# lRomul/sensorium

Hardware: AMD Instinct MI355X
Metric: training clips/sec/GPU (DwiseNeuro fwd+bwd, B=32 T=32 36x64) at 1/2/4/8 GPUs (higher is better)
Workload: dtype bf16

## Files before the change

### include/dwn.h

```cpp
#ifndef DWN_H_
#define DWN_H_
#include <stddef.h>
#include <stdint.h>

#ifdef __cplusplus
extern "C" {
#endif

#define DWN_ABI_VERSION 7
#define DWN_F32 0
#define DWN_BF16 1
#define DWN_F32_AUTO 0
#define DWN_F32_NATIVE 1
#define DWN_F32_SPLIT3 2
#define DWN_BN_EVAL 0
#define DWN_BN_TRAIN 1
#define DWN_BN_FROZEN 2
#define DWN_NREP 32

#define DWN_LD_PLAIN 0
#define DWN_LD_PE 1
#define DWN_LD_BNACT 2
#define DWN_LD_AFFINE2 3
#define DWN_LD_DY3 4
// ... 81 lines not shown
typedef struct dwn_dw_spatial_bwd_args {
    dwn_load_desc dy;
    dwn_load_desc y1;
    const float* w;
    void* dh1;
    float* dw;
    int planes, Hin, Win, Hout, Wout, C, stride, ks;
    double* stats;
    int rows_band;
    int impl;
    const void* a0; long long a0_ld; const void* w1; int Cin;
} dwn_dw_spatial_bwd_args;

typedef struct dwn_dw_temporal_fwd_args {
    dwn_load_desc in;
    const float* w;
    void* out;
    int B, T, HW, C, kt;
    double* stats;
    const float* z_scale; const float* z_shift; long long* pooled;
} dwn_dw_temporal_fwd_args;

typedef struct dwn_dw_temporal_bwd_args {
    dwn_load_desc dy; int dy_kind;
    dwn_load_desc y2;
    const float* w;
    void* dh2;
    float* dw;
    int B, T, HW, C, kt;
    double* stats;
} dwn_dw_temporal_bwd_args;

typedef struct dwn_bn {
    const float* gamma; const float* beta;
    float* running_mean; float* running_var; long long* num_batches_tracked;
    float* coef;
    float* dgamma; float* dbeta;
} dwn_bn;

typedef struct dwn_stem_args {
    int dtype, training, B, Cin, C0; long long S;
    float eps, momentum;
    const float* x;
    const float* w;
    dwn_bn bn;
    const float *pe_t, *pe_h, *pe_w;
    int T, H, W;
    void* y0;
    void* out;
    const void* dout;
    float* dw;
    void* ws; size_t ws_bytes;
    double* xmom;
} dwn_stem_args;

typedef struct dwn_stem_input_grad_args {
    int dtype, training, B, Cin, C0; long long S;
    const float* w;
    const float* coef;
    const void* dout;
    float* dx;
} dwn_stem_input_grad_args;

typedef struct dwn_block_args {
    int dtype, training;
    int B, T, Hin, Win, Hout, Wout, Cin, Cmid, Cout, stride, ks, kt, se_r;
    float eps, momentum;
    const void* x; void* out;
    void *y1, *y2, *y3, *y4;
    void* z3;
    int x_has_pe;
    void* a0;
    const float *pe_t, *pe_h, *pe_w;
    const float *out_pe_t, *out_pe_h, *out_pe_w;
    const float *w_pw, *w_dws, *w_dwt, *w_pwl, *se_wr, *se_br, *se_we, *se_be;
    dwn_bn bn1, bn2, bn3, bn4, bnsc;
    const float* drop_scale;
    const int *hsrc, *wsrc, *hinv, *winv;
    float *se_pmean, *se_hidpre, *se_gate;
    const void* dout; void* dx;
    void *buf_a, *buf_b;
    void *dy4, *da0;
    float *dw_pw, *dw_dws, *dw_dwt, *dw_pwl, *dse_wr, *dse_br, *dse_we, *dse_be;
    void* ws; size_t ws_bytes;
    int pwl_bwd;
    int f32_products;
    int y1_mode;
} dwn_block_args;

typedef struct dwn_pool_args {
    int dtype; long long BT; int HW, C;
    const void* x; void* out; const void* dout; void* dx;
} dwn_pool_args;

typedef struct dwn_cortex_args {
    int dtype, training, B, T, Cin, C, groups;
    float eps, momentum;
    const void* x; void* out; void* y;
    const float* w;
    dwn_bn bn, bnsc;
    const float* drop_scale;
    const void* dout; void* dx; float* dw;
    const float* dout_mask; int dout_mask_ld;
    void* ws; size_t ws_bytes;
    int f32_products;
} dwn_cortex_args;

typedef struct dwn_readout_args {
    int dtype, B, T, Cin, groups, n_out;
    float softplus_beta;
    const void* x;
    const float* w; const float* bias;
    const float* drop_mask;
    float* out;
    const float* dout; void* dx; float* dw; float* dbias;
    void* ws; size_t ws_bytes;
    void* wt;
    int f32_products;
    const float* beta_dev; float* dbeta;
} dwn_readout_args;

typedef struct dwn_tensor_entry {
    float* param; const float* grad; float* exp_avg; float* exp_avg_sq; float* ema;
    long long numel; int is_int64; int pad_;
} dwn_tensor_entry;

typedef struct dwn_guarded_entry {
    float* param; const float* grad; float* exp_avg; float* exp_avg_sq; float* ema;
    long long numel; int is_int64; int pad_;
    long long* step;
} dwn_guarded_entry;
typedef struct dwn_step_guard {
    double norm;
    float coef;
    int skip;
    long long nonfinite;
    long long good_steps, skipped_steps;
} dwn_step_guard;
#define DWN_GS_SEG 1024

// ... 11 lines not shown
typedef struct dwn_clip_desc {
    dwn_clip_src src, mix;
    int bbx1, bby1, bbx2, bby2;
    float one_minus_lam, lam;
    int mouse;
    int mix_mode;
} dwn_clip_desc;

enum {
    DWN_FAM_PW_FWD = 0, DWN_FAM_DWS_FWD, DWN_FAM_DWT_FWD, DWN_FAM_SE_POOL, DWN_FAM_PWL_FWD, DWN_FAM_RESID_FWD,
    DWN_FAM_RESID_BWD, DWN_FAM_PWL_DGRAD, DWN_FAM_PWL_WGRAD, DWN_FAM_BN3_REDUCE, DWN_FAM_DWT_BWD, DWN_FAM_DWS_BWD,
    DWN_FAM_PW_DGRAD, DWN_FAM_PW_WGRAD, DWN_FAM_CORTEX_FWD, DWN_FAM_CORTEX_BWD, DWN_FAM_READOUT_FWD, DWN_FAM_READOUT_BWD,
    DWN_FAM_COUNT
};
#define DWN_PROF_ROCTX (1ull << 63)
int dwn_profile_enable(unsigned long long family_mask, int device);
int dwn_profile_collect(int family, double* total_ms, long long* launches);

int dwn_abi_version(void);
const char* dwn_source_hash(void);
int dwn_sizeof(const char* struct_name);
const char* dwn_last_error(void);

int dwn_gemm_nn(const dwn_gemm_nn_args* a, int dtype, int device, void* stream);
int dwn_gemm_tn(const dwn_gemm_tn_args* a, int dtype, int device, void* stream);
int dwn_dw_spatial_fwd(const dwn_dw_spatial_fwd_args* a, int dtype, int device, void* stream);
int dwn_dw_spatial_bwd(const dwn_dw_spatial_bwd_args* a, int dtype, int device, void* stream);
int dwn_dw_spatial_fwd_rc_supported(const dwn_dw_spatial_fwd_args* a, int dtype);
int dwn_dw_spatial_bwd_rc_supported(const dwn_dw_spatial_bwd_args* a, int dtype);
int dwn_dw_temporal_fwd(const dwn_dw_temporal_fwd_args* a, int dtype, int device, void* stream);
int dwn_dw_temporal_bwd(const dwn_dw_temporal_bwd_args* a, int dtype, int device, void* stream);
int dwn_dw_temporal_wide_fwd(const dwn_dw_temporal_fwd_args* a, int dtype, int device, void* stream);
int dwn_dw_temporal_wide_bwd(const dwn_dw_temporal_bwd_args* a, int dtype, int device, void* stream);
int dwn_bn_finalize(const double* stats, int stat_c, double count, const dwn_bn* bn, int C, int training,
                    float momentum, float eps, int device, void* stream);
int dwn_bn_bwd_finalize(const double* stats, double count, const dwn_bn* bn, float* abc, int C, int device,
                        void* stream);
int dwn_pack_weight(const float* src, void* dst, int groups, int R, int C, int transpose, int Rd, int Cd,
                    int dtype, int device, void* stream);
size_t dwn_conv_pw_bn_stats_workspace_bytes(int Cin);
int dwn_conv_pw_bn_stats(const void* a0, long long a0_ld, long long M, const float* w_pw, int E, int Cin, const dwn_bn* bn,
                         float momentum, float eps, double* sc_stats, void* ws, size_t ws_bytes, int dtype, int device,
                         void* stream);

size_t dwn_stem_workspace_bytes(const dwn_stem_args* a);
int dwn_stem_forward(const dwn_stem_args* a, int device, void* stream);
int dwn_stem_backward(const dwn_stem_args* a, int device, void* stream);
int dwn_stem_input_grad(const dwn_stem_input_grad_args* a, int device, void* stream);
int dwn_stem_backward_input(const dwn_stem_args* a, float* dx, int device, void* stream);
size_t dwn_block_workspace_bytes(const dwn_block_args* a, int backward);
int dwn_block_forward(const dwn_block_args* a, int device, void* stream);
int dwn_block_backward(const dwn_block_args* a, int device, void* stream);
int dwn_block_forward_writes(const dwn_block_args* a);
int dwn_pool_forward(const dwn_pool_args* a, int device, void* stream);
int dwn_pool_backward(const dwn_pool_args* a, int device, void* stream);
size_t dwn_cortex_workspace_bytes(const dwn_cortex_args* a, int backward);
int dwn_cortex_forward(const dwn_cortex_args* a, int device, void* stream);
int dwn_cortex_backward(const dwn_cortex_args* a, int device, void* stream);
size_t dwn_readout_workspace_bytes(const dwn_readout_args* a, int backward);
size_t dwn_readout_wt_bytes(const dwn_readout_args* a);
int dwn_readout_forward(const dwn_readout_args* a, int device, void* stream);
int dwn_readout_backward(const dwn_readout_args* a, int device, void* stream);

int dwn_poisson_loss_forward(const float* pred, const float* target, const float* w, long long per_sample,
                             long long total, float eps, double* loss_acc, int device, void* stream);
int dwn_poisson_loss_backward(const float* pred, const float* target, const float* w, const float* gscale,
                              long long per_sample, long long total, float eps, float* dpred, int device,
                              void* stream);
int dwn_f64_to_f32(const double* src, float* dst, int n, int device, void* stream);

int dwn_adamw_ema_multi(const dwn_tensor_entry* list, int ntensors, int max_blocks, double lr, double beta1,
                        double beta2, double eps, double weight_decay, long long step, double ema_decay,
                        double grad_scale, int device, void* stream);
int dwn_ema_lerp_multi(const dwn_tensor_entry* list, int ntensors, int max_blocks, double decay, int device,
                       void* stream);

size_t dwn_grad_guard_workspace_bytes(int ntensors, int max_blocks);
int dwn_grad_sumsq_multi(const dwn_guarded_entry* list, int ntensors, int max_blocks, double grad_scale, void* ws,
                         size_t ws_bytes, double* pair, int device, void* stream);
int dwn_step_guard_finalize(const double* pair_a, const double* pair_b, double max_norm, int skip_nonfinite,
                            const dwn_guarded_entry* list, int ntensors, dwn_step_guard* guard, int device, void* stream);
int dwn_adamw_ema_multi_guarded(const dwn_guarded_entry* list, int ntensors, int max_blocks, double lr, double beta1,
                                double beta2, double eps, double weight_decay, double ema_decay, double grad_scale,
                                const dwn_step_guard* guard, int device, void* stream);


typedef struct dwn_pw_bwd_args {
    const void* dh1; const void* a0; const float* w_pw; const float* abc;
    void* da0; float* dw;
    long long M; int E; int Cin;
    void* ws; size_t ws_bytes;
    const void* res; const float* res_abc; int res_C;
    const int* res_hinv; const int* res_winv; int res_Hin, res_Win, res_Hout, res_Wout;
} dwn_pw_bwd_args;
int dwn_pw_bwd_fused_supported(int dtype, long long M, int E, int Cin);
size_t dwn_pw_backward_workspace_bytes(int E, int Cin, int dtype);
int dwn_pw_backward(const dwn_pw_bwd_args* a, int dtype, int device, void* stream);

typedef struct dwn_dw_spatial_rc_fwd_args {
    const void* a0; long long a0_ld;
    const void* blob;
    void* out;
    int planes, Hin, Win, Hout, Wout, Cin, E, stride;
    double* stats;
    int rows_band;
    int round_y1;
// ... 238 lines not shown
```

### sensorium_amd/_lib.py

```python
from __future__ import annotations

import ctypes as C
import os
from pathlib import Path

import torch

_HERE = Path(__file__).resolve().parent
DETERMINISTIC = os.environ.get("DWN_DETERMINISTIC", "0") == "1"
_LIB_NAME = "libdwiseneuro_hip_det.so" if DETERMINISTIC else "libdwiseneuro_hip.so"
LIB_PATH = Path(os.environ["DWN_LIB_PATH"]) if os.environ.get("DWN_LIB_PATH") else _HERE / "csrc" / _LIB_NAME

c_p = C.c_void_p
c_i = C.c_int
c_ll = C.c_longlong
c_f = C.c_float
c_d = C.c_double
c_sz = C.c_size_t

DWN_F32, DWN_BF16 = 0, 1
DWN_NREP = 32
LD_PLAIN, LD_PE, LD_BNACT, LD_AFFINE2, LD_DY3, LD_GATE, LD_CAT1 = 0, 1, 2, 3, 4, 5, 6
EPI_STORE, EPI_READOUT, EPI_DG, EPI_STORE_CAT, EPI_DH3 = 0, 1, 2, 3, 4
NN_AUTO, NN_XL128, NN_XL256, NN_TILE128, NN_KD = 0, 1, 2, 3, 4
# ... 12 lines not shown


class GemmNNArgs(C.Structure):
    _fields_ = [("a", LoadDesc), ("a_kind", c_i), ("b", c_p), ("ldb", c_ll), ("c", c_p), ("ldc", c_ll),
                ("M", c_i), ("N", c_i), ("K", c_i), ("groups", c_i), ("stats", c_p),
                ("f32_split", c_i), ("stat_nchan", c_i), ("epi", c_i), ("bias", c_p),
                ("sp_beta", c_f), ("out_nct", c_p), ("Tn", c_i), ("n_valid", c_i), ("y3", c_p), ("ldy3", c_ll),
                ("s3", c_p), ("t3", c_p), ("dg", c_p), ("dg_ld", c_i), ("rows_per_sample", c_i),
                ("a2", c_p), ("a2_ld", c_ll), ("K1", c_i), ("b_sample_stride", c_ll), ("b_rows_per_sample", c_i),
                ("gate3", c_p), ("dps3", c_p), ("coef3", c_p), ("coef3_ld", c_i), ("variant", c_i), ("sp_beta_dev", c_p)]


class GemmTNArgs(C.Structure):
    _fields_ = [("p", LoadDesc), ("p_kind", c_i), ("q", LoadDesc), ("q_kind", c_i), ("M", c_i), ("R", c_i),
                ("Cc", c_i), ("dw", c_p), ("lddw", c_ll), ("groups", c_i), ("rows_per_split", c_i),
                ("nsplit", c_i), ("R_load", c_i), ("rows_per_sample", c_i), ("splits_per_sample", c_i),
                ("dw_sample_stride", c_ll), ("overwrite", c_i), ("dw_f64", c_i)]


class DwSpatialFwdArgs(C.Structure):
    _fields_ = [("inp", LoadDesc), ("w", c_p), ("out", c_p), ("planes", c_i), ("Hin", c_i), ("Win", c_i),
                ("Hout", c_i), ("Wout", c_i), ("C", c_i), ("stride", c_i), ("ks", c_i), ("stats", c_p),
                ("rows_band", c_i), ("impl", c_i),
                ("a0", c_p), ("a0_ld", c_ll), ("w1", c_p), ("Cin", c_i)]


class DwSpatialBwdArgs(C.Structure):
    _fields_ = [("dy", LoadDesc), ("y1", LoadDesc), ("w", c_p), ("dh1", c_p), ("dw", c_p), ("planes", c_i),
                ("Hin", c_i), ("Win", c_i), ("Hout", c_i), ("Wout", c_i), ("C", c_i), ("stride", c_i),
                ("ks", c_i), ("stats", c_p), ("rows_band", c_i), ("impl", c_i),
                ("a0", c_p), ("a0_ld", c_ll), ("w1", c_p), ("Cin", c_i)]


class DwTemporalFwdArgs(C.Structure):
    _fields_ = [("inp", LoadDesc), ("w", c_p), ("out", c_p), ("B", c_i), ("T", c_i), ("HW", c_i), ("C", c_i),
                ("kt", c_i), ("stats", c_p), ("z_scale", c_p), ("z_shift", c_p), ("pooled", c_p)]


class DwTemporalBwdArgs(C.Structure):
    _fields_ = [("dy", LoadDesc), ("dy_kind", c_i), ("y2", LoadDesc), ("w", c_p), ("dh2", c_p), ("dw", c_p),
                ("B", c_i), ("T", c_i), ("HW", c_i), ("C", c_i), ("kt", c_i), ("stats", c_p)]


class BN(C.Structure):
    _fields_ = [("gamma", c_p), ("beta", c_p), ("running_mean", c_p), ("running_var", c_p),
                ("num_batches_tracked", c_p), ("coef", c_p), ("dgamma", c_p), ("dbeta", c_p)]


class StemArgs(C.Structure):
    _fields_ = [("dtype", c_i), ("training", c_i), ("B", c_i), ("Cin", c_i), ("C0", c_i), ("S", c_ll),
                ("eps", c_f), ("momentum", c_f), ("x", c_p), ("w", c_p), ("bn", BN),
                ("pe_t", c_p), ("pe_h", c_p), ("pe_w", c_p), ("T", c_i), ("H", c_i), ("W", c_i),
                ("y0", c_p), ("out", c_p),
                ("dout", c_p), ("dw", c_p), ("ws", c_p), ("ws_bytes", c_sz), ("xmom", c_p)]


class StemInputGradArgs(C.Structure):
    _fields_ = [("dtype", c_i), ("training", c_i), ("B", c_i), ("Cin", c_i), ("C0", c_i), ("S", c_ll),
                ("w", c_p), ("coef", c_p), ("dout", c_p), ("dx", c_p)]


class BlockArgs(C.Structure):
    _fields_ = [("dtype", c_i), ("training", c_i),
                ("B", c_i), ("T", c_i), ("Hin", c_i), ("Win", c_i), ("Hout", c_i), ("Wout", c_i), ("Cin", c_i),
                ("Cmid", c_i), ("Cout", c_i), ("stride", c_i), ("ks", c_i), ("kt", c_i), ("se_r", c_i),
                ("eps", c_f), ("momentum", c_f),
                ("x", c_p), ("out", c_p), ("y1", c_p), ("y2", c_p), ("y3", c_p), ("y4", c_p),
                ("z3", c_p), ("x_has_pe", c_i), ("a0", c_p),
                ("pe_t", c_p), ("pe_h", c_p), ("pe_w", c_p),
                ("out_pe_t", c_p), ("out_pe_h", c_p), ("out_pe_w", c_p),
                ("w_pw", c_p), ("w_dws", c_p), ("w_dwt", c_p), ("w_pwl", c_p), ("se_wr", c_p), ("se_br", c_p),
                ("se_we", c_p), ("se_be", c_p),
                ("bn1", BN), ("bn2", BN), ("bn3", BN), ("bn4", BN), ("bnsc", BN),
                ("drop_scale", c_p), ("hsrc", c_p), ("wsrc", c_p), ("hinv", c_p), ("winv", c_p),
                ("se_pmean", c_p), ("se_hidpre", c_p), ("se_gate", c_p),
                ("dout", c_p), ("dx", c_p), ("buf_a", c_p), ("buf_b", c_p), ("dy4", c_p), ("da0", c_p),
                ("dw_pw", c_p), ("dw_dws", c_p), ("dw_dwt", c_p), ("dw_pwl", c_p), ("dse_wr", c_p),
                ("dse_br", c_p), ("dse_we", c_p), ("dse_be", c_p),
                ("ws", c_p), ("ws_bytes", c_sz), ("pwl_bwd", c_i), ("f32_products", c_i), ("y1_mode", c_i)]


class PoolArgs(C.Structure):
    _fields_ = [("dtype", c_i), ("BT", c_ll), ("HW", c_i), ("C", c_i), ("x", c_p), ("out", c_p), ("dout", c_p),
                ("dx", c_p)]


class CortexArgs(C.Structure):
    _fields_ = [("dtype", c_i), ("training", c_i), ("B", c_i), ("T", c_i), ("Cin", c_i), ("C", c_i),
                ("groups", c_i), ("eps", c_f), ("momentum", c_f), ("x", c_p), ("out", c_p), ("y", c_p),
                ("w", c_p), ("bn", BN), ("bnsc", BN), ("drop_scale", c_p), ("dout", c_p), ("dx", c_p),
                ("dw", c_p), ("dout_mask", c_p), ("dout_mask_ld", c_i), ("ws", c_p), ("ws_bytes", c_sz), ("f32_products", c_i)]


class ReadoutArgs(C.Structure):
    _fields_ = [("dtype", c_i), ("B", c_i), ("T", c_i), ("Cin", c_i), ("groups", c_i), ("n_out", c_i),
                ("softplus_beta", c_f), ("x", c_p), ("w", c_p), ("bias", c_p), ("drop_mask", c_p), ("out", c_p),
                ("dout", c_p), ("dx", c_p), ("dw", c_p), ("dbias", c_p), ("ws", c_p), ("ws_bytes", c_sz), ("wt", c_p),
                ("f32_products", c_i), ("beta_dev", c_p), ("dbeta", c_p)]


class TensorEntry(C.Structure):
    _fields_ = [("param", c_p), ("grad", c_p), ("exp_avg", c_p), ("exp_avg_sq", c_p), ("ema", c_p),
                ("numel", c_ll), ("is_int64", c_i), ("pad_", c_i)]


class GuardedEntry(C.Structure):
    _fields_ = [("param", c_p), ("grad", c_p), ("exp_avg", c_p), ("exp_avg_sq", c_p), ("ema", c_p),
                ("numel", c_ll), ("is_int64", c_i), ("pad_", c_i), ("step", c_p)]


class StepGuard(C.Structure):
    _fields_ = [("norm", c_d), ("coef", c_f), ("skip", c_i), ("nonfinite", c_ll), ("good_steps", c_ll),
                ("skipped_steps", c_ll)]


class ClipSrc(C.Structure):
    _fields_ = [("video", c_p), ("behavior", c_p), ("pupil_center", c_p), ("responses", c_p), ("length", c_ll),
                ("video_dtype", c_i), ("frame_start", c_i), ("frame_step", c_i), ("valid", c_i)]


class ClipDesc(C.Structure):
    _fields_ = [("src", ClipSrc), ("mix", ClipSrc), ("bbx1", c_i), ("bby1", c_i), ("bbx2", c_i), ("bby2", c_i),
                ("one_minus_lam", c_f), ("lam", c_f), ("mouse", c_i), ("mix_mode", c_i)]


class PwBwdArgs(C.Structure):
    _fields_ = [("dh1", c_p), ("a0", c_p), ("w_pw", c_p), ("abc", c_p), ("da0", c_p), ("dw", c_p),
                ("M", c_ll), ("E", c_i), ("Cin", c_i), ("ws", c_p), ("ws_bytes", c_sz), ("res", c_p), ("res_abc", c_p),
                ("res_C", c_i), ("res_hinv", c_p), ("res_winv", c_p), ("res_Hin", c_i), ("res_Win", c_i), ("res_Hout", c_i),
                ("res_Wout", c_i)]


# ... 99 lines not shown
TRIAL_STATE_ROWS, TRIAL_SCORE_ROWS, TRIAL_SUMMARY, TRIAL_TILE = 17, 5, 8, 4
NOISE_BINARY, NOISE_SPARSE = 0, 1
STA_SUMMARY = 8
GAUSS_PARAMS, GAUSS_TABLE = 7, 16
MIX_BOX, MIX_BLEND = 0, 1
VID_U8, VID_F32 = 0, 1

_STRUCTS = {
    "dwn_load_desc": LoadDesc, "dwn_gemm_nn_args": GemmNNArgs, "dwn_gemm_tn_args": GemmTNArgs,
    "dwn_dw_spatial_fwd_args": DwSpatialFwdArgs, "dwn_dw_spatial_bwd_args": DwSpatialBwdArgs,
    "dwn_dw_temporal_fwd_args": DwTemporalFwdArgs, "dwn_dw_temporal_bwd_args": DwTemporalBwdArgs,
    "dwn_bn": BN, "dwn_stem_args": StemArgs, "dwn_block_args": BlockArgs, "dwn_pool_args": PoolArgs,
    "dwn_cortex_args": CortexArgs, "dwn_readout_args": ReadoutArgs, "dwn_tensor_entry": TensorEntry,
    "dwn_clip_src": ClipSrc, "dwn_clip_desc": ClipDesc, "dwn_pw_bwd_args": PwBwdArgs,
    "dwn_dw_spatial_rc_fwd_args": DwSpatialRcFwdArgs, "dwn_stem_input_grad_args": StemInputGradArgs,
    "dwn_guarded_entry": GuardedEntry, "dwn_step_guard": StepGuard, "dwn_gaze_args": GazeArgs,
    "dwn_corr_args": CorrArgs, "dwn_gabor_args": GaborArgs, "dwn_modulator_args": ModulatorArgs,
    "dwn_blur3d_args": Blur3dArgs, "dwn_clip_moments_args": ClipMomentsArgs, "dwn_mei_update_args": MeiUpdateArgs,
    "dwn_trial_desc": TrialDesc, "dwn_trial_group": TrialGroup, "dwn_trial_score_args": TrialScoreArgs,
    "dwn_spatial_gain_args": SpatialGainArgs, "dwn_noise_args": NoiseArgs, "dwn_sta_args": StaArgs,
    "dwn_gauss2d_args": Gauss2dArgs, "dwn_gauss2d_profile_args": Gauss2dProfileArgs,
}

_P = C.POINTER
SYMBOLS = {
    "dwn_abi_version": (c_i, []),
    "dwn_source_hash": (C.c_char_p, []),
    "dwn_sizeof": (c_i, [C.c_char_p]),
    "dwn_last_error": (C.c_char_p, []),
    "dwn_profile_enable": (c_i, [C.c_ulonglong, c_i]),
    "dwn_profile_collect": (c_i, [c_i, _P(c_d), _P(c_ll)]),
    "dwn_gemm_nn": (c_i, [_P(GemmNNArgs), c_i, c_i, c_p]),
    "dwn_gemm_tn": (c_i, [_P(GemmTNArgs), c_i, c_i, c_p]),
    "dwn_dw_spatial_fwd": (c_i, [_P(DwSpatialFwdArgs), c_i, c_i, c_p]),
    "dwn_dw_spatial_bwd": (c_i, [_P(DwSpatialBwdArgs), c_i, c_i, c_p]),
    "dwn_dw_spatial_bwd_rc_supported": (c_i, [_P(DwSpatialBwdArgs), c_i]),
    "dwn_dw_spatial_fwd_rc_supported": (c_i, [_P(DwSpatialFwdArgs), c_i]),
    "dwn_dw_temporal_fwd": (c_i, [_P(DwTemporalFwdArgs), c_i, c_i, c_p]),
    "dwn_dw_temporal_bwd": (c_i, [_P(DwTemporalBwdArgs), c_i, c_i, c_p]),
    "dwn_dw_temporal_wide_fwd": (c_i, [_P(DwTemporalFwdArgs), c_i, c_i, c_p]),
    "dwn_dw_temporal_wide_bwd": (c_i, [_P(DwTemporalBwdArgs), c_i, c_i, c_p]),
    "dwn_bn_finalize": (c_i, [c_p, c_i, c_d, _P(BN), c_i, c_i, c_f, c_f, c_i, c_p]),
    "dwn_bn_bwd_finalize": (c_i, [c_p, c_d, _P(BN), c_p, c_i, c_i, c_p]),
    "dwn_pack_weight": (c_i, [c_p, c_p, c_i, c_i, c_i, c_i, c_i, c_i, c_i, c_i, c_p]),
    "dwn_stem_workspace_bytes": (c_sz, [_P(StemArgs)]),
    "dwn_stem_forward": (c_i, [_P(StemArgs), c_i, c_p]),
    "dwn_stem_backward": (c_i, [_P(StemArgs), c_i, c_p]),
    "dwn_stem_input_grad": (c_i, [_P(StemInputGradArgs), c_i, c_p]),
    "dwn_stem_backward_input": (c_i, [_P(StemArgs), c_p, c_i, c_p]),
    "dwn_block_workspace_bytes": (c_sz, [_P(BlockArgs), c_i]),
    "dwn_block_forward": (c_i, [_P(BlockArgs), c_i, c_p]),
    "dwn_block_backward": (c_i, [_P(BlockArgs), c_i, c_p]),
    "dwn_block_forward_writes": (c_i, [_P(BlockArgs)]),
    "dwn_pool_forward": (c_i, [_P(PoolArgs), c_i, c_p]),
    "dwn_pool_backward": (c_i, [_P(PoolArgs), c_i, c_p]),
    "dwn_cortex_workspace_bytes": (c_sz, [_P(CortexArgs), c_i]),
    "dwn_cortex_forward": (c_i, [_P(CortexArgs), c_i, c_p]),
    "dwn_cortex_backward": (c_i, [_P(CortexArgs), c_i, c_p]),
    "dwn_readout_workspace_bytes": (c_sz, [_P(ReadoutArgs), c_i]),
    "dwn_readout_wt_bytes": (c_sz, [_P(ReadoutArgs)]),
    "dwn_readout_forward": (c_i, [_P(ReadoutArgs), c_i, c_p]),
    "dwn_readout_backward": (c_i, [_P(ReadoutArgs), c_i, c_p]),
    "dwn_poisson_loss_forward": (c_i, [c_p, c_p, c_p, c_ll, c_ll, c_f, c_p, c_i, c_p]),
    "dwn_poisson_loss_backward": (c_i, [c_p, c_p, c_p, c_p, c_ll, c_ll, c_f, c_p, c_i, c_p]),
    "dwn_f64_to_f32": (c_i, [c_p, c_p, c_i, c_i, c_p]),
    "dwn_adamw_ema_multi": (c_i, [c_p, c_i, c_i, c_d, c_d, c_d, c_d, c_d, c_ll, c_d, c_d, c_i, c_p]),
    "dwn_ema_lerp_multi": (c_i, [c_p, c_i, c_i, c_d, c_i, c_p]),
    "dwn_grad_guard_workspace_bytes": (c_sz, [c_i, c_i]),
    "dwn_grad_sumsq_multi": (c_i, [c_p, c_i, c_i, c_d, c_p, c_sz, c_p, c_i, c_p]),
    "dwn_step_guard_finalize": (c_i, [c_p, c_p, c_d, c_i, c_p, c_i, c_p, c_i, c_p]),
    "dwn_adamw_ema_multi_guarded": (c_i, [c_p, c_i, c_i, c_d, c_d, c_d, c_d, c_d, c_d, c_d, c_p, c_i, c_p]),
    "dwn_conv_pw_bn_stats_workspace_bytes": (c_sz, [c_i]),
    "dwn_conv_pw_bn_stats": (c_i, [c_p, c_ll, c_ll, c_p, c_i, c_i, _P(BN), c_f, c_f, c_p, c_p, c_sz, c_i, c_i, c_p]),
    "dwn_pw_bwd_fused_supported": (c_i, [c_i, c_ll, c_i, c_i]),
    "dwn_pw_backward_workspace_bytes": (c_sz, [c_i, c_i, c_i]),
    "dwn_pw_backward": (c_i, [_P(PwBwdArgs), c_i, c_i, c_p]),
    "dwn_dw_spatial_rc_blob_bytes": (c_sz, [c_i, c_i]),
    "dwn_dw_spatial_rc_prep": (c_i, [c_p, c_p, c_p, c_i, c_i, c_p, c_i, c_p]),
    "dwn_dw_spatial_rc_supported": (c_i, [c_i, c_i, c_i, c_i, c_i, c_i, c_i]),
    "dwn_dw_spatial_fwd_rc": (c_i, [_P(DwSpatialRcFwdArgs), c_i, c_p]),
    "dwn_assemble_inputs": (c_i, [c_p, c_i, c_i, c_i, c_i, c_i, c_i, c_f, c_p, c_i, c_p]),
    "dwn_assemble_targets": (c_i, [c_p, c_i, c_i, c_p, c_p, c_i, c_i, c_p, c_i, c_p]),
    "dwn_gaze_shift_forward": (c_i, [_P(GazeArgs), c_i, c_p]),
    "dwn_gaze_shift_backward": (c_i, [_P(GazeArgs), c_i, c_p]),
    "dwn_plane_mean": (c_i, [c_p, c_i, c_i, c_i, c_i, c_i, c_i, c_i, c_p, c_i, c_p]),
    "dwn_corr_ws_bytes": (c_sz, [_P(CorrArgs)]),
    "dwn_corr_moments": (c_i, [_P(CorrArgs), c_i, c_p]),
    "dwn_corr_loss_finalize": (c_i, [_P(CorrArgs), c_i, c_p]),
    "dwn_corr_loss_backward": (c_i, [_P(CorrArgs), c_i, c_p]),
    "dwn_gabor_workspace_bytes": (c_sz, [_P(GaborArgs)]),
    "dwn_gabor_forward": (c_i, [_P(GaborArgs), c_i, c_p]),
    "dwn_gabor_backward": (c_i, [_P(GaborArgs), c_i, c_p]),
    "dwn_modulator_ws_bytes": (c_sz, [_P(ModulatorArgs)]),
    "dwn_modulator_forward": (c_i, [_P(ModulatorArgs), c_i, c_p]),
    "dwn_modulator_backward": (c_i, [_P(ModulatorArgs), c_i, c_p]),
    "dwn_blur3d_ws_bytes": (c_sz, [_P(Blur3dArgs)]),
    "dwn_clip_moments_ws_bytes": (c_sz, [_P(ClipMomentsArgs)]),
    "dwn_blur3d": (c_i, [_P(Blur3dArgs), c_i, c_p]),
    "dwn_clip_moments": (c_i, [_P(ClipMomentsArgs), c_i, c_p]),
    "dwn_mei_update": (c_i, [_P(MeiUpdateArgs), c_i, c_p]),
    "dwn_trial_score_ws_bytes": (c_sz, [_P(TrialScoreArgs)]),
    "dwn_trial_moments": (c_i, [_P(TrialScoreArgs), c_i, c_p]),
    "dwn_trial_score_finalize": (c_i, [_P(TrialScoreArgs), c_i, c_p]),
    "dwn_spatial_gain_ws_bytes": (c_sz, [_P(SpatialGainArgs)]),
    "dwn_spatial_gain_forward": (c_i, [_P(SpatialGainArgs), c_i, c_p]),
    "dwn_spatial_gain_backward": (c_i, [_P(SpatialGainArgs), c_i, c_p]),
    "dwn_gauss2d_ws_bytes": (c_sz, [_P(Gauss2dArgs)]),
    "dwn_gauss2d_fit": (c_i, [_P(Gauss2dArgs), c_i, c_p]),
    "dwn_gauss2d_profile": (c_i, [_P(Gauss2dProfileArgs), c_i, c_p]),
    "dwn_noise_forward": (c_i, [_P(NoiseArgs), c_i, c_p]),
    "dwn_sta_state_bytes": (c_sz, [_P(StaArgs)]),
    "dwn_sta_ws_bytes": (c_sz, [_P(StaArgs)]),
    "dwn_sta_accumulate": (c_i, [_P(StaArgs), c_i, c_p]),
    "dwn_sta_finalize": (c_i, [_P(StaArgs), c_i, c_p]),
}


class DwnError(RuntimeError):
    pass


HASH_SRCS = ("dwn_api.hip", "dwn_gemm.hip", "dwn_gemm_nn_1.hip", "dwn_gemm_nn_2.hip", "dwn_gemm_nn_3.hip", "dwn_gemm_nn_4.hip", "dwn_gemm_nn_5.hip",
             "dwn_gemm_nn_6.hip", "dwn_gemm_tn.hip", "dwn_pw_bwd.hip", "dwn_gemm_xl.hip", "dwn_gemm_kd.hip", "dwn_dwconv.hip", "dwn_dwrc.hip",
             "dwn_dwbwd.hip", "dwn_dwfwd.hip", "dwn_elementwise.hip", "dwn_data.hip", "dwn_gaze.hip", "dwn_modulator.hip", "dwn_spatial.hip", "dwn_mei.hip", "dwn_rf_fit.hip", "dwn_trial_score.hip", "dwn_rf.hip", "dwn_corr.hip", "dwn_stim.hip", "dwn_common.h", "dwn_internal.h",
             "dwn_kernels.h", "dwn_launch.h", "dwn_gemm_nn.h", "dwn_gain.h",
             "../../include/dwn.h")


def source_hash() -> str:
    import hashlib
    h = hashlib.sha256()
    for name in HASH_SRCS:
        h.update((_HERE / "csrc" / name).read_bytes())
    return h.hexdigest()[:16]


def _load():
    if not LIB_PATH.exists():
        raise ImportError(
            f"{LIB_PATH} is missing: build it with `python -c 'import __graft_entry__ as g; g.build()'` "
            f"(or `make -C {LIB_PATH.parent}`).  sensorium_amd has no fallback path.")
    lib = C.CDLL(str(LIB_PATH), mode=getattr(os, "RTLD_NOW", 2))
    ab = bool(os.environ.get("DWN_LIB_PATH"))
    for name, (restype, argtypes) in SYMBOLS.items():
        if ab and name in ("dwn_stem_input_grad", "dwn_stem_backward_input", "dwn_grad_guard_workspace_bytes", "dwn_grad_sumsq_multi",
                           "dwn_step_guard_finalize", "dwn_adamw_ema_multi_guarded", "dwn_dw_temporal_wide_fwd",
                           "dwn_dw_temporal_wide_bwd", "dwn_gaze_shift_forward", "dwn_gaze_shift_backward",
                           "dwn_plane_mean", "dwn_corr_ws_bytes", "dwn_corr_moments", "dwn_corr_loss_finalize",
                           "dwn_corr_loss_backward", "dwn_gabor_workspace_bytes", "dwn_gabor_forward",
                           "dwn_gabor_backward", "dwn_modulator_ws_bytes", "dwn_modulator_forward",
                           "dwn_modulator_backward", "dwn_blur3d_ws_bytes", "dwn_clip_moments_ws_bytes", "dwn_blur3d",
                           "dwn_clip_moments", "dwn_mei_update", "dwn_trial_score_ws_bytes", "dwn_trial_moments",
                           "dwn_trial_score_finalize", "dwn_spatial_gain_ws_bytes", "dwn_spatial_gain_forward",
                           "dwn_spatial_gain_backward", "dwn_noise_forward", "dwn_sta_state_bytes", "dwn_sta_ws_bytes",
                           "dwn_sta_accumulate", "dwn_sta_finalize", "dwn_gauss2d_ws_bytes", "dwn_gauss2d_fit",
                           "dwn_gauss2d_profile") and not hasattr(lib, name):
            continue
        fn = getattr(lib, name)
        fn.restype = restype
        fn.argtypes = argtypes
    if lib.dwn_abi_version() != 7 and not (ab and lib.dwn_abi_version() == 6):
        raise ImportError("libdwiseneuro_hip.so ABI version mismatch")
    built, have = lib.dwn_source_hash().decode(), source_hash()
    if built != have and not os.environ.get("DWN_LIB_PATH"):
        raise ImportError(f"{LIB_PATH.name} was built from other sources (binary {built}, tree {have}): rebuild it with "
                          f"`make -C {LIB_PATH.parent}` — binaries are not in git, so what runs must be what is committed")
    for cname, struct in _STRUCTS.items():
        n = lib.dwn_sizeof(cname.encode())
        if n != C.sizeof(struct) and not (ab and (0 < n < C.sizeof(struct) or cname in ("dwn_stem_input_grad_args", "dwn_guarded_entry", "dwn_step_guard", "dwn_gaze_args", "dwn_corr_args", "dwn_gabor_args", "dwn_modulator_args", "dwn_blur3d_args", "dwn_clip_moments_args", "dwn_mei_update_args", "dwn_trial_desc", "dwn_trial_group", "dwn_trial_score_args", "dwn_spatial_gain_args", "dwn_noise_args", "dwn_sta_args", "dwn_gauss2d_args", "dwn_gauss2d_profile_args"))):
            raise ImportError(f"struct layout mismatch for {cname}: C {n} bytes vs ctypes {C.sizeof(struct)}")
    return lib


lib = _load()


def check(rc: int, what: str = ""):
    if rc != 0:
        msg = lib.dwn_last_error()
        raise DwnError(f"{what} failed (rc={rc}): {msg.decode() if msg else ''}")
```

### sensorium_amd/csrc/dwn_api.hip

```cpp
#include "dwn_internal.h"
#include "dwn_kernels.h"
#include <string.h>
#include <math.h>

static thread_local char g_err[512] = "";
#ifndef DWN_EVAL_CHAIN
#define DWN_EVAL_CHAIN 1
#endif

extern "C" size_t dwn_dw_spatial_rc_blob_bytes(int E, int Cin);
extern "C" int dwn_dw_spatial_rc_supported(int dtype, int Cin, int E, int ks, int stride, int Hin, int Win);
extern "C" int dwn_dw_spatial_rc_prep(const float* w_pw, const float* w_dws, const float* bn1_coef, int E, int Cin, void* blob,
                                      int device, void* stream);
extern "C" int dwn_dw_spatial_fwd_rc(const dwn_dw_spatial_rc_fwd_args* a, int device, void* stream);
bool dw_spatial_bwd_rc_supported(const DwSpatialBwd& a, int dtype);
bool dw_spatial_fwd_rc_walk_supported(const DwSpatialFwd& a, int dtype);

int dwn_set_error(int code, const char* msg) {
    snprintf(g_err, sizeof(g_err), "dwn error %d: %s", code, msg ? msg : "");
    return code;
}

#define TRY(x) do { int rc__ = (x); if (rc__ != 0) return rc__; } while (0)

// ... 325 lines not shown
int dwn_dw_temporal_wide_bwd(const dwn_dw_temporal_bwd_args* a, int dtype, int device, void* stream) {
    g_err[0] = 0;
    if (int rc = dw_temporal_wide_check(a->kt, a->C, a->dy_kind)) return rc;
    ENTER(device);
    return launch_dw_temporal_wide_bwd(*a, dtype, (hipStream_t)stream);
}
int dwn_bn_finalize(const double* stats, int stat_c, double count, const dwn_bn* bn, int C, int training,
                    float momentum, float eps, int device, void* stream) {
    ENTER(device);
    return bn_finalize(stats, stat_c, count, *bn, C, training, momentum, eps, (hipStream_t)stream);
}
int dwn_bn_bwd_finalize(const double* stats, double count, const dwn_bn* bn, float* abc, int C, int device,
                        void* stream) {
    ENTER(device);
    return k_bn_bwd_finalize(bwd_job(stats, count, *bn, abc, C, false), BnBwdJob{}, (hipStream_t)stream);
}
size_t dwn_conv_pw_bn_stats_workspace_bytes(int Cin) { return (size_t)(Cin + 8) * Cin * sizeof(double) + 256; }
int dwn_conv_pw_bn_stats(const void* a0, long long a0_ld, long long M, const float* w_pw, int E, int Cin, const dwn_bn* bn,
                         float momentum, float eps, double* sc_stats, void* ws, size_t ws_bytes, int dtype, int device, void* stream) {
    ENTER(device);
    hipStream_t s = (hipStream_t)stream;
    if (!a0 || !w_pw || !bn || !bn->coef || !ws) return dwn_set_error(-1, "conv_pw_bn_stats: null pointer");
    if (Cin % 8 || E <= 0 || M <= 0 || M >= (1ll << 31)) return dwn_set_error(-2, "conv_pw_bn_stats: Cin % 8 == 0, 0 < M < 2^31");
    if (ws_bytes < dwn_conv_pw_bn_stats_workspace_bytes(Cin)) return dwn_set_error(-6, "conv_pw_bn_stats: workspace too small");
    double* gram = reinterpret_cast<double*>(((size_t)ws + 255) & ~(size_t)255);
    TRY(k_zero(gram, (size_t)(Cin + 8) * Cin * sizeof(double), s));
    LoadDesc cat = ld_plain(a0, a0_ld);
    cat.cat_c1 = Cin; cat.cat_c2 = 0;
    GemmTN g = tn_base(cat, LD_CAT1, ld_plain(a0, a0_ld), LD_PLAIN, (int)M, Cin + 8, Cin, reinterpret_cast<float*>(gram), Cin, 1);
    g.dw_f64 = 1;
    TRY(launch_gemm_tn(g, dtype, s));
    return k_bn1_gram_finalize(gram, w_pw, E, Cin, (double)M, bn->gamma, bn->beta, bn->running_mean, bn->running_var,
                               bn->num_batches_tracked, momentum, eps, bn->coef, sc_stats, dtype, s);
}
int dwn_pack_weight(const float* src, void* dst, int groups, int R, int C, int transpose, int Rd, int Cd, int dtype,
                    int device, void* stream) {
    ENTER(device);
    return k_pack_weight(src, dst, groups, R, C, transpose, Rd, Cd, dtype, (hipStream_t)stream);
}

size_t dwn_stem_workspace_bytes(const dwn_stem_args* a) {
    return ((size_t)DWN_NREP * stem_moment_count() * sizeof(double) + 256 +
            (size_t)DWN_NREP * a->C0 * stem_acc_stride() * sizeof(double) + 1024);
}
int dwn_stem_forward(const dwn_stem_args* a, int device, void* stream) {
    ENTER(device);
    hipStream_t s = (hipStream_t)stream;
    if (a->C0 % 8) return dwn_set_error(-2, "stem: C0 must be a multiple of 8");
    if (a->pe_t && (i64)a->T * a->H * a->W != a->S) return dwn_set_error(-2, "stem: T*H*W != S");
    Carver c(a->ws, a->ws_bytes);
    double* mom = c.take<double>((size_t)DWN_NREP * stem_moment_count());
    if (!c.ok()) return dwn_set_error(-6, "stem: workspace too small");
    const i64 M = (i64)a->B * a->S;
    if (a->training == DWN_BN_TRAIN) {
        if (!a->xmom) return dwn_set_error(-1, "stem_forward: xmom buffer required in training mode");
        TRY(k_zero(mom, (size_t)DWN_NREP * stem_moment_count() * sizeof(double), s));
        TRY(k_stem_xmom(a->x, a->B, a->Cin, a->S, mom, s));
        TRY(k_stem_bn_finalize(mom, (double)M, a->w, a->bn.gamma, a->bn.beta, a->bn.running_mean, a->bn.running_var,
                               a->bn.num_batches_tracked, a->momentum, a->eps, a->bn.coef, a->xmom, a->C0, a->Cin, s));
    } else {
        TRY(bn_finalize(nullptr, a->C0, (double)M, a->bn, a->C0, 0, a->momentum, a->eps, s));
    }
    return k_stem_out(a->x, a->w, a->bn.coef, a->pe_t, a->pe_h, a->pe_w, a->T, a->H, a->W, a->B, a->Cin, a->S, a->C0, a->out,
                      a->dtype, s);
}
int dwn_stem_backward(const dwn_stem_args* a, int device, void* stream) {
    ENTER(device);
    hipStream_t s = (hipStream_t)stream;
    const bool frozen = a->training == DWN_BN_FROZEN;
    if (!frozen && !a->xmom) return dwn_set_error(-1, "stem_backward: xmom (saved by the forward) required");
    Carver c(a->ws, a->ws_bytes);
    double* mom = c.take<double>((size_t)DWN_NREP * stem_moment_count());
    double* acc = c.take<double>((size_t)DWN_NREP * a->C0 * stem_acc_stride());
    if (!c.ok()) return dwn_set_error(-6, "stem: workspace too small");
    const i64 M = (i64)a->B * a->S;
    if (frozen) {
        TRY(k_zero(mom, (size_t)((char*)(acc + (size_t)DWN_NREP * a->C0 * stem_acc_stride()) - (char*)mom), s));
        TRY(k_stem_bwd_acc(a->dout, a->x, mom, (double)M, a->B, a->Cin, a->S, a->C0, acc, a->dtype, s));
        return k_stem_bwd_finalize_frozen(acc, a->w, a->bn.coef, a->bn.dgamma, a->bn.dbeta, a->dw, a->C0, a->Cin, s);
    }
    TRY(k_zero(acc, (size_t)DWN_NREP * a->C0 * stem_acc_stride() * sizeof(double), s));
    TRY(k_stem_bwd_acc(a->dout, a->x, a->xmom, (double)M, a->B, a->Cin, a->S, a->C0, acc, a->dtype, s));
    return k_stem_bwd_finalize(acc, a->xmom, a->w, a->bn.coef, (double)M, a->bn.dgamma, a->bn.dbeta, a->dw, a->C0, a->Cin, s);
}

int dwn_stem_backward_input(const dwn_stem_args* a, float* dx, int device, void* stream) {
    g_err[0] = 0;
    if (!a || !dx) return dwn_set_error(-1, "stem_backward_input: null pointer (args, dx)");
    if (a->training != DWN_BN_TRAIN)
        return dwn_set_error(-7, "stem_backward_input: built for batch statistics (DWN_BN_TRAIN) only; the frozen-statistics input "
                                 "gradient is dwn_stem_backward + dwn_stem_input_grad");
    if (!a->x || !a->w || !a->bn.coef || !a->dout || !a->dw || !a->xmom || !a->ws)
        return dwn_set_error(-1, "stem_backward_input: null pointer (x, w, bn.coef, dout, dw, xmom, ws)");
    if (a->C0 <= 0 || a->C0 % 8 || a->Cin <= 0 || a->B <= 0 || a->S <= 0)
        return dwn_set_error(-2, "stem_backward_input: C0 must be a positive multiple of 8; B, Cin, S positive");
    if (a->dtype != DWN_F32 && a->dtype != DWN_BF16) return dwn_set_error(-2, "stem_backward_input: dtype");
    if (a->C0 > (a->dtype == DWN_BF16 ? 128 : 64) || a->Cin > 8)
        return dwn_set_error(-4, "stem_backward_input: more than 128 (bf16) / 64 (fp32) stem channels or 8 input channels not built");
    ENTER(device);
    hipStream_t s = (hipStream_t)stream;
    Carver c(a->ws, a->ws_bytes);
    double* mom = c.take<double>((size_t)DWN_NREP * stem_moment_count());
    double* acc = c.take<double>((size_t)DWN_NREP * a->C0 * stem_acc_stride());
    if (!c.ok()) return dwn_set_error(-6, "stem: workspace too small");
    float* qx = reinterpret_cast<float*>(mom);
    const i64 M = (i64)a->B * a->S;
    TRY(k_zero(acc, (size_t)DWN_NREP * a->C0 * stem_acc_stride() * sizeof(double), s));
    TRY(k_stem_bwd_acc(a->dout, a->x, a->xmom, (double)M, a->B, a->Cin, a->S, a->C0, acc, a->dtype, s));
    TRY(k_stem_bwd_finalize(acc, a->xmom, a->w, a->bn.coef, (double)M, a->bn.dgamma, a->bn.dbeta, a->dw, a->C0, a->Cin, s));
    TRY(k_stem_bwd_finalize_dx(acc, a->xmom, a->w, a->bn.coef, (double)M, qx, a->C0, a->Cin, s));
    return k_stem_input_grad_train(a->dout, a->w, a->bn.coef, a->x, qx, a->B, a->Cin, a->S, a->C0, dx, a->dtype, s);
}

int dwn_stem_input_grad(const dwn_stem_input_grad_args* a, int device, void* stream) {
    g_err[0] = 0;
    if (!a || !a->w || !a->coef || !a->dout || !a->dx) return dwn_set_error(-1, "stem_input_grad: null pointer");
    if (a->C0 <= 0 || a->C0 % 8 || a->Cin <= 0 || a->B <= 0 || a->S <= 0)
        return dwn_set_error(-2, "stem_input_grad: C0 must be a positive multiple of 8; B, Cin, S positive");
    if (a->dtype != DWN_F32 && a->dtype != DWN_BF16) return dwn_set_error(-2, "stem_input_grad: dtype");
    if (a->training != DWN_BN_FROZEN)
        return dwn_set_error(-7, "stem_input_grad: this entry is the frozen-statistics (DWN_BN_FROZEN) input gradient; through batch "
                                 "statistics (DWN_BN_TRAIN) it is dwn_stem_backward_input");
    ENTER(device);
    return k_stem_input_grad(a->dout, a->w, a->coef, a->B, a->Cin, a->S, a->C0, a->dx, a->dtype, (hipStream_t)stream);
}

size_t dwn_block_workspace_bytes(const dwn_block_args* a, int backward) {
    return carve_block(*a, backward, nullptr, 0).bytes;
}

int dwn_block_forward(const dwn_block_args* ap, int device, void* stream) {
    ENTER(device);
    const dwn_block_args& a = *ap;
    hipStream_t s = (hipStream_t)stream;
    TRY(check_block(a));
    BlockWs w = carve_block(a, 0, a.ws, a.ws_bytes);
    if (w.bytes > a.ws_bytes) return dwn_set_error(-6, "block_forward: workspace too small");
    const int dt = a.dtype, tr = a.training != DWN_BN_EVAL;
    const bool bs = a.training == DWN_BN_TRAIN;
    const i64 Min = (i64)a.B * a.T * a.Hin * a.Win, Mout = (i64)a.B * a.T * a.Hout * a.Wout;
    const int S_out = a.T * a.Hout * a.Wout;
    {
        PrepArgs pa;
        bool ok = pa.zero(w.zero_beg, ((size_t)(w.zero_end - w.zero_beg) + 15) & ~(size_t)15);
        ok = ok && pa.packw(a.w_pw, w.wpw, 1, a.Cmid, a.Cin, 0, a.Cmid, a.Cin);
        ok = ok && pa.packw(a.w_pwl, w.wpwl, 1, a.Cout, a.Cmid, 0, a.Cout, a.Cmid);
        ok = ok && pa.packdw(a.w_dws, w.wdws, a.Cmid, a.ks * a.ks);
        ok = ok && pa.packdw(a.w_dwt, w.wdwt, a.Cmid, a.kt);
        if (!bs) {
            ok = ok && pa.bneval(a.bn1, a.Cmid, a.eps) && pa.bneval(a.bn2, a.Cmid, a.eps) && pa.bneval(a.bn3, a.Cmid, a.eps);
            ok = ok && pa.bneval(a.bn4, a.Cout, a.eps) && pa.bneval(a.bnsc, a.Cout, a.eps);
        }
        if (!ok) return dwn_set_error(-2, "block_forward: workspace arena must be 16-byte aligned");
        TRY(k_prep(pa, dt, s));
    }

    const void* a0 = a.x;
    if (!a.x_has_pe) {
        if (!a.a0) return dwn_set_error(-2, "block_forward: a0 buffer required when x_has_pe == 0");
        TRY(k_ew_apply(ld_pe(a.x, a.Cin, a.pe_t, a.pe_h, a.pe_w, a.T, a.Hin, a.Win), LD_PE, a.a0, a.Cin, Min, a.Cin, dt, s));
        a0 = a.a0;
    }
    LoadDesc xin = ld_plain(a0, a.Cin);
    const bool identity_sc = a.stride == 1 && a.Hin == a.Hout && a.Win == a.Wout;
    const bool y1_free = tr && block_y1_free(a);
    bool eval_chain = false;
    if (DWN_EVAL_CHAIN && !tr && dt == DWN_BF16) {
        DwSpatialFwd f; memset(&f, 0, sizeof(f));
        f.planes = a.B * a.T; f.Hin = a.Hin; f.Win = a.Win; f.Hout = a.Hout; f.Wout = a.Wout; f.C = a.Cmid; f.stride = a.stride; f.ks = a.ks;
        f.in.ld = a.Cmid; f.a0_ld = a.Cin; f.Cin = a.Cin;
        eval_chain = dw_spatial_fwd_rc_walk_supported(f, dt);
    }
    if (eval_chain) {
        DwSpatialFwd d; memset(&d, 0, sizeof(d));
        d.in = ld_bnact(nullptr, a.Cmid, a.bn1.coef, a.Cmid, 1, nullptr, 0, 1);
        d.a0 = a0; d.a0_ld = a.Cin; d.w1 = w.wpw; d.Cin = a.Cin;
        d.w = w.wdws; d.out = a.y2; d.planes = a.B * a.T; d.Hin = a.Hin; d.Win = a.Win; d.Hout = a.Hout;
        d.Wout = a.Wout; d.C = a.Cmid; d.stride = a.stride; d.ks = a.ks; d.stats = nullptr;
        PROF(DWN_FAM_DWS_FWD, launch_dw_spatial_fwd(d, dt, s));
    } else if (y1_free) {
        LoadDesc cat = ld_plain(a0, a.Cin);
        cat.cat_c1 = a.Cin; cat.cat_c2 = 0;
        if (bs) {
        GemmTN g = tn_base(cat, LD_CAT1, ld_plain(a0, a.Cin), LD_PLAIN, (int)Min, a.Cin + 8, a.Cin, reinterpret_cast<float*>(w.gram), a.Cin, 1);
        g.dw_f64 = 1;
        PROF(DWN_FAM_PW_FWD, launch_gemm_tn(g, dt, s));
        PROF(DWN_FAM_PW_FWD, k_bn1_gram_finalize(w.gram, a.w_pw, a.Cmid, a.Cin, (double)Min, a.bn1.gamma, a.bn1.beta, a.bn1.running_mean,
                                                 a.bn1.running_var, a.bn1.num_batches_tracked, a.momentum, a.eps, a.bn1.coef,
                                                 identity_sc ? w.stsc : nullptr, dt, s));
        }
        DwSpatialFwd d; memset(&d, 0, sizeof(d));
        d.in = ld_bnact(nullptr, a.Cmid, a.bn1.coef, a.Cmid, 1, nullptr, 0, 1);
        d.a0 = a0; d.a0_ld = a.Cin; d.w1 = w.wpw; d.Cin = a.Cin;
        d.w = w.wdws; d.out = a.y2; d.planes = a.B * a.T; d.Hin = a.Hin; d.Win = a.Win; d.Hout = a.Hout;
        d.Wout = a.Wout; d.C = a.Cmid; d.stride = a.stride; d.ks = a.ks; d.stats = w.st2;
        PROF(DWN_FAM_DWS_FWD, launch_dw_spatial_fwd(d, dt, s));
    } else if (block_fwd_rc(a)) {
        TRY(dwn_dw_spatial_rc_prep(a.w_pw, w.wdws, a.bn1.coef, a.Cmid, a.Cin, w.rcblob, device, stream));
        dwn_dw_spatial_rc_fwd_args r; memset(&r, 0, sizeof(r));
        r.a0 = a0; r.a0_ld = a.Cin; r.blob = w.rcblob; r.out = a.y2; r.planes = a.B * a.T; r.Hin = a.Hin; r.Win = a.Win;
        r.Hout = a.Hout; r.Wout = a.Wout; r.Cin = a.Cin; r.E = a.Cmid; r.stride = a.stride; r.stats = nullptr;
        r.rows_band = 0; r.round_y1 = 1;
        PROF(DWN_FAM_DWS_FWD, dwn_dw_spatial_fwd_rc(&r, device, stream));
    } else {
    {
        GemmNN g = nn_base(xin, LD_PLAIN, w.wpw, a.Cin, a.y1, a.Cmid, (int)Min, a.Cmid, a.Cin, 1);
        g.f32_split = f32_split_of(a.f32_products, !tr);
        g.stats = tr ? w.st1 : nullptr; g.stat_nchan = a.Cmid;
        PROF(DWN_FAM_PW_FWD, launch_gemm_nn(g, dt, s));
    }
    if (bs) TRY(bn_finalize(w.st1, a.Cmid, (double)Min, a.bn1, a.Cmid, 1, a.momentum, a.eps, s));
    {
        DwSpatialFwd d; memset(&d, 0, sizeof(d));
        d.in = ld_bnact(a.y1, a.Cmid, a.bn1.coef, a.Cmid, 1, nullptr, 0, 1);
        d.w = w.wdws; d.out = a.y2; d.planes = a.B * a.T; d.Hin = a.Hin; d.Win = a.Win; d.Hout = a.Hout;
        d.Wout = a.Wout; d.C = a.Cmid; d.stride = a.stride; d.ks = a.ks; d.stats = tr ? w.st2 : nullptr;
        PROF(DWN_FAM_DWS_FWD, launch_dw_spatial_fwd(d, dt, s));
    }
    }
    if (bs) TRY(bn_finalize(w.st2, a.Cmid, (double)Mout, a.bn2, a.Cmid, 1, a.momentum, a.eps, s));
    const bool eval_z3 = !tr;
    {
        DwTemporalFwd d; memset(&d, 0, sizeof(d));
        d.in = ld_bnact(a.y2, a.Cmid, a.bn2.coef, a.Cmid, 1, nullptr, 0, 1);
        d.w = w.wdwt; d.out = a.y3; d.B = a.B; d.T = a.T; d.HW = a.Hout * a.Wout; d.C = a.Cmid; d.kt = a.kt;
        d.stats = tr ? w.st3 : nullptr;
        if (eval_z3) {
            d.out = a.z3; d.z_scale = a.bn3.coef; d.z_shift = a.bn3.coef + a.Cmid; d.pooled = w.pooled;
        }
        PROF(DWN_FAM_DWT_FWD, launch_dw_temporal_fwd(d, dt, s));
    }
    if (bs) TRY(bn_finalize(w.st3, a.Cmid, (double)Mout, a.bn3, a.Cmid, 1, a.momentum, a.eps, s));
    if (!eval_z3) {
        LoadDesc z3 = ld_bnact(a.y3, a.Cmid, a.bn3.coef, a.Cmid, 1, nullptr, 0, S_out);
        PROF(DWN_FAM_SE_POOL, k_se_pool(z3, a.B, a.Cmid, S_out, w.pooled, a.z3, dt, s));
    }
    int gate_folded = 0;
    TRY(k_se_mlp_fwd(w.pooled, 1.0f / (float)S_out, a.se_wr, a.se_br, a.se_we, a.se_be, a.B, a.Cmid, a.se_r,
                     a.se_pmean, a.se_hidpre, a.se_gate, pwl_gated_weights(a) ? a.w_pwl : nullptr, w.wgated, a.Cout, dt, &gate_folded, s));
    if (pwl_gated_weights(a)) {
        if (!gate_folded) TRY(k_gate_weights(a.w_pwl, a.se_gate, w.wgated, a.B, a.Cout, a.Cmid, dt, s));
        GemmNN g = nn_base(ld_plain(a.z3, a.Cmid), LD_PLAIN, w.wgated, a.Cmid, a.y4, a.Cout, (int)Mout, a.Cout, a.Cmid, 1);
        g.b_sample_stride = (i64)a.Cout * a.Cmid; g.b_rows_per_sample = S_out;
        g.stats = tr ? w.st4 : nullptr; g.stat_nchan = a.Cout; g.f32_split = f32_split_of(a.f32_products, !tr);
        PROF(DWN_FAM_PWL_FWD, launch_gemm_nn(g, dt, s));
    } else {
        LoadDesc u = ld_plain(a.z3, a.Cmid);
        u.gate = a.se_gate; u.gate_ld = a.Cmid; u.rows_per_sample = S_out;
        GemmNN g = nn_base(u, LD_GATE, w.wpwl, a.Cmid, a.y4, a.Cout, (int)Mout, a.Cout, a.Cmid, 1);
        g.stats = tr ? w.st4 : nullptr; g.stat_nchan = a.Cout; g.f32_split = f32_split_of(a.f32_products, !tr);
        PROF(DWN_FAM_PWL_FWD, launch_gemm_nn(g, dt, s));
    }
    ResGeom gm = geom_of(a);
    if (bs) {
        if (!(y1_free && identity_sc)) PROF(DWN_FAM_RESID_FWD, k_shortcut_stats(xin, gm, w.stsc, dt, s));
        TRY(k_bn_finalize_train(fin_job(w.st4, a.Cout, (double)Mout, a.bn4, a.Cout),
                                 fin_job(w.stsc, a.Cin, (double)Mout, a.bnsc, a.Cout), a.momentum, a.eps, s));
    }
    PROF(DWN_FAM_RESID_FWD, k_residual_fwd(xin, a.y4, a.bn4.coef, a.bnsc.coef, a.drop_scale, gm, a.out_pe_t, a.out_pe_h,
                                           a.out_pe_w, a.out, dt, s));
    return 0;
}

static int pw_backward(int dt, const void* dh1, const void* a0, const float* w_pw, const float* abc, int E, int Cin, i64 M,
                       void* bp, float* gacc, float* r3, float* tacc, void* da0, float* dw, const void* res,
                       const float* res_abc, int res_C, const ResGeom* rg, hipStream_t s) {
    const int res_n = res ? res_C / Cin : 0;
    const bool gathered = res && rg && rg->hinv;
    if (res && (!res_abc || res_C % Cin || res_n < 1 || res_n > 2))
        return dwn_set_error(-2, "pw_backward: the shortcut term needs res_abc and res_C in {Cin, 2 Cin}");
    if (res && !pw_bwd_fused_supported(dt, M, E, Cin))
        return dwn_set_error(-3, "pw_backward: the shortcut term is built into the one-pass kernel only (dwn_pw_bwd_fused_supported)");
    TRY(k_pw_bwd_prep(w_pw, abc, E, Cin, bp, gacc, r3, dt, (res && !gathered) ? res_abc : nullptr, res_C, s));
    if (pw_bwd_fused_supported(dt, M, E, Cin)) {
        PROF(DWN_FAM_PW_DGRAD, launch_pw_bwd_fused(dh1, a0, bp, r3, da0, tacc, M, E, Cin, dt, res, res_abc, res_n,
                                                   gathered ? rg->hinv : nullptr, gathered ? rg->winv : nullptr, gathered ? rg->Hin : 0,
                                                   gathered ? rg->Win : 0, gathered ? rg->Hout : 0, gathered ? rg->Wout : 0, s));
    } else {
        {
            GemmNN g = nn_base(ld_plain(dh1, E), LD_PLAIN, bp, (i64)E + Cin, da0, Cin, (int)M, Cin, E + Cin, 1);
            g.epi = EPI_STORE_CAT; g.a2 = a0; g.a2_ld = Cin; g.K1 = E; g.bias = r3;
            PROF(DWN_FAM_PW_DGRAD, launch_gemm_nn(g, dt, s));
        }
        {
            LoadDesc cat = ld_plain(dh1, E);
            cat.q = a0; cat.ld2 = Cin; cat.cat_c1 = E; cat.cat_c2 = Cin;
            GemmTN g = tn_base(cat, LD_CAT1, ld_plain(a0, Cin), LD_PLAIN, (int)M, E + Cin + 8, Cin, tacc, Cin, 1);
            PROF(DWN_FAM_PW_WGRAD, launch_gemm_tn(g, dt, s));
        }
    }
    return k_pw_wgrad_fold(tacc, abc, w_pw, E, Cin, dw, dt, s);
}

int dwn_block_backward(const dwn_block_args* ap, int device, void* stream) {
    const dwn_block_args& a = *ap;
    hipStream_t s = (hipStream_t)stream;
    g_err[0] = 0;
    TRY(check_block(a));
    if (a.training == DWN_BN_EVAL)
        return dwn_set_error(-7, "block_backward: only training-mode (batch-statistics) and frozen-statistics backward are built");
    ENTER(device);
    const bool frozen = a.training == DWN_BN_FROZEN;
    BlockWs w = carve_block(a, 1, a.ws, a.ws_bytes);
    if (w.bytes > a.ws_bytes) return dwn_set_error(-6, "block_backward: workspace too small");
    const int dt = a.dtype;
    const i64 Min = (i64)a.B * a.T * a.Hin * a.Win, Mout = (i64)a.B * a.T * a.Hout * a.Wout;
    const int S_out = a.T * a.Hout * a.Wout;
    float* dg = reinterpret_cast<float*>(w.pooled);
    const bool y1_free = block_y1_free(a);
    {
        PrepArgs pa;
        bool ok = pa.zero(w.zero_beg, ((size_t)(w.zero_end - w.zero_beg) + 15) & ~(size_t)15);
        ok = ok && pa.packw(a.w_pwl, w.wpwl, 1, a.Cout, a.Cmid, 1, a.Cmid, a.Cout);
// ... 49 lines not shown
    }
    TRY(k_se_mlp_bwd(dg, a.se_gate, a.se_hidpre, a.se_pmean, a.se_wr, a.se_we, a.B, a.Cmid, a.se_r,
                     1.0f / (float)S_out, w.dgp, w.dhp, w.dps, a.dse_wr, a.dse_br, a.dse_we, a.dse_be, s));
    LoadDesc d3; memset(&d3, 0, sizeof(d3));
    d3.p = du; d3.q = a.y3; d3.ld = a.Cmid; d3.v1 = w.ident3; d3.v2 = w.ident3 + a.Cmid; d3.v3 = w.ident3 + 2 * a.Cmid;
    d3.v4 = a.bn3.coef; d3.v5 = a.bn3.coef + a.Cmid; d3.gate = a.se_gate; d3.gate2 = w.dps; d3.gate_ld = a.Cmid;
    d3.rows_per_sample = S_out;
    PROF(DWN_FAM_BN3_REDUCE, k_bn3_bwd_reduce(d3, a.bn3.coef, Mout, a.Cmid, w.st3, du, dt, s));
    }
    TRY(k_bn_bwd_finalize(bwd_job(w.st3, (double)Mout, a.bn3, w.abc3, a.Cmid, frozen), BnBwdJob{}, s));
    {
        DwTemporalBwd d; memset(&d, 0, sizeof(d));
        d.dy = ld_affine2(du, a.y3, a.Cmid, w.abc3, a.Cmid);
        d.dy_kind = LD_PLAIN;
        d.y2 = ld_ycoef(a.y2, a.Cmid, a.bn2.coef, a.Cmid);
        d.w = w.wdwt; d.dh2 = a.buf_b; d.dw = a.dw_dwt; d.B = a.B; d.T = a.T; d.HW = a.Hout * a.Wout; d.C = a.Cmid;
        d.kt = a.kt; d.stats = w.st2;
        PROF(DWN_FAM_DWT_BWD, launch_dw_temporal_bwd(d, dt, s));
    }
    TRY(k_bn_bwd_finalize(bwd_job(w.st2, (double)Mout, a.bn2, w.abc2, a.Cmid, frozen), BnBwdJob{}, s));
    void* dh1 = a.buf_a;
    {
        DwSpatialBwd d; memset(&d, 0, sizeof(d));
        d.dy = ld_affine2(a.buf_b, a.y2, a.Cmid, w.abc2, a.Cmid);
        d.y1 = ld_ycoef(y1_free ? nullptr : a.y1, a.Cmid, a.bn1.coef, a.Cmid);
        if (y1_free) { d.a0 = xin.p; d.a0_ld = a.Cin; d.w1 = w.wpw; d.Cin = a.Cin; }
        d.w = w.wdws; d.dh1 = dh1; d.dw = a.dw_dws; d.planes = a.B * a.T; d.Hin = a.Hin; d.Win = a.Win;
        d.Hout = a.Hout; d.Wout = a.Wout; d.C = a.Cmid; d.stride = a.stride; d.ks = a.ks; d.stats = w.st1;
        PROF(DWN_FAM_DWS_BWD, launch_dw_spatial_bwd(d, dt, s));
    }
    TRY(k_bn_bwd_finalize(bwd_job(w.st1, (double)Min, a.bn1, w.abc1, a.Cmid, frozen), BnBwdJob{}, s));
    const bool identity_sc = a.stride == 1 && a.Hin == a.Hout && a.Win == a.Wout;
    const bool dx_folded = a.Cout % a.Cin == 0 && a.Cout / a.Cin <= 2 && dwn_pw_bwd_fused_supported(dt, Min, a.Cmid, a.Cin) &&
                           (identity_sc || (gm.hinv && gm.winv && a.Hin + a.Win <= 512));
    TRY(pw_backward(dt, dh1, xin.p, a.w_pw, w.abc1, a.Cmid, a.Cin, Min, w.bp, w.gacc, w.r3, w.tacc, dx_folded ? a.dx : a.da0, a.dw_pw,
                    dx_folded ? a.dout : nullptr, w.abcsc, a.Cout, (dx_folded && !identity_sc) ? &gm : nullptr, s));
    if (dx_folded) return 0;
    PROF(DWN_FAM_RESID_BWD, k_residual_bwd_dx(xin, a.da0, a.dout, w.abcsc, gm, a.dx, dt, s));
    return 0;
}

int dwn_block_forward_writes(const dwn_block_args* ap) {
    const dwn_block_args& a = *ap;
    if (a.training) return block_y1_free(a) ? 2 : 3;
    if (block_fwd_rc(a)) return 0;
    if (DWN_EVAL_CHAIN && a.dtype == DWN_BF16) {
        DwSpatialFwd f; memset(&f, 0, sizeof(f));
        f.planes = a.B * a.T; f.Hin = a.Hin; f.Win = a.Win; f.Hout = a.Hout; f.Wout = a.Wout; f.C = a.Cmid; f.stride = a.stride; f.ks = a.ks;
        f.in.ld = a.Cmid; f.a0_ld = a.Cin; f.Cin = a.Cin;
        if (dw_spatial_fwd_rc_walk_supported(f, a.dtype)) return 0;
    }
    return 1;
}

int dwn_pool_forward(const dwn_pool_args* a, int device, void* stream) {
    ENTER(device);
    if (a->C % 8) return dwn_set_error(-2, "pool: C must be a multiple of 8");
    return k_pool_fwd(a->x, a->out, a->BT, a->HW, a->C, a->dtype, (hipStream_t)stream);
}
int dwn_pool_backward(const dwn_pool_args* a, int device, void* stream) {
    ENTER(device);
    if (a->C % 8) return dwn_set_error(-2, "pool: C must be a multiple of 8");
    return k_pool_bwd(a->dout, a->dx, a->BT, a->HW, a->C, a->dtype, (hipStream_t)stream);
}

namespace {
struct CortexWs { void* wp; double *st, *stsc; float *abc, *abcsc; void *dy, *dxmain; char *zb, *ze; size_t bytes; };
CortexWs carve_cortex(const dwn_cortex_args& a, int backward, void* base, size_t cap) {
    CortexWs w; memset(&w, 0, sizeof(w));
    Carver c(base, cap);
    const size_t ts = tsize(a.dtype);
    const i64 M = (i64)a.B * a.T;
    w.wp = c.take<char>((size_t)a.C * (a.Cin / a.groups) * ts);
    c.take<char>(0);
    size_t z0 = (c.off + 255) & ~(size_t)255;
    w.st = c.take<double>(nstat(a.C));
    w.stsc = c.take<double>(nstat(backward ? a.C : a.Cin));
    size_t z1 = c.off;
    if (backward) {
        w.abc = c.take<float>(3 * (size_t)a.C);
        w.abcsc = c.take<float>(3 * (size_t)a.C);
        w.dy = c.take<char>((size_t)M * a.C * ts);
        w.dxmain = c.take<char>((size_t)M * a.Cin * ts);
    }
    w.bytes = c.off + 256;
    if (base) { w.zb = (char*)base + z0; w.ze = (char*)base + z1; }
    return w;
}
}

size_t dwn_cortex_workspace_bytes(const dwn_cortex_args* a, int backward) {
    return carve_cortex(*a, backward, nullptr, 0).bytes;
}
int dwn_cortex_forward(const dwn_cortex_args* ap, int device, void* stream) {
    ENTER(device);
    const dwn_cortex_args& a = *ap;
    hipStream_t s = (hipStream_t)stream;
    if (a.Cin % (8 * a.groups) || a.C % (8 * a.groups)) return dwn_set_error(-2, "cortex: channels per group must be multiples of 8");
    CortexWs w = carve_cortex(a, 0, a.ws, a.ws_bytes);
    if (w.bytes > a.ws_bytes) return dwn_set_error(-6, "cortex_forward: workspace too small");
    const int M = a.B * a.T, Kg = a.Cin / a.groups, Ng = a.C / a.groups, dt = a.dtype, tr = a.training != DWN_BN_EVAL;
    const bool bs = a.training == DWN_BN_TRAIN;
    {
        PrepArgs pa;
        bool ok = pa.zero(w.zb, ((size_t)(w.ze - w.zb) + 15) & ~(size_t)15);
        ok = ok && pa.packw(a.w, w.wp, 1, a.C, Kg, 0, a.C, Kg);
// ... 661 lines not shown
```

### sensorium_amd/csrc/dwn_elementwise.hip

```cpp
#include "dwn_internal.h"
#include "dwn_kernels.h"
#include "dwn_launch.h"

#define NCV 8
#define DISPATCH_T(dtype, CALL_BF, CALL_F) do { if ((dtype) == DWN_BF16) { CALL_BF; } else { CALL_F; } } while (0)

#define SLICE_SETUP(Cval)                                   \
    constexpr int KC = TT<T>::KC;                           \
    const int tid = threadIdx.x;                            \
    const int cv = tid % NCV, pl = tid / NCV;               \
    const int c0 = blockIdx.y * NCV * KC;                   \
    const int chan = c0 + cv * KC;                          \
    const bool chan_ok = chan < (Cval);                     \
    (void)pl; (void)chan_ok;

template <int KC>
__device__ __forceinline__ void slice_stats_flush(float* lstat, const float* s0, const float* s1, int cv,
                                                 int c0, int C, double* stats, int rep) {
    static_assert(NCV == 8, "wave pre-reduction below assumes 8 channel vectors per slice");
    const int tid = threadIdx.x;
    DET_WAVES_BEGIN
#pragma unroll
    for (int i = 0; i < KC; ++i) {
        float a = s0[i], b = s1[i];
#pragma unroll
        for (int o = 8; o < 64; o <<= 1) { a += __shfl_xor(a, o); b += __shfl_xor(b, o); }
        if ((tid & 63) < NCV) {
            atomicAdd(&lstat[cv * KC + i], a);
            atomicAdd(&lstat[NCV * KC + cv * KC + i], b);
        }
    }
    DET_WAVES_END
    __syncthreads();
    DET_ENTER();
    if (tid < 2 * NCV * KC) {
        int which = tid / (NCV * KC), c = c0 + tid % (NCV * KC);
        if (c < C) stat_add(stats, rep, C, which, c, lstat[tid]);
    }
}

template <typename K>
static dim3 resident_slice_grid(K kernel, i64 rows, int C, int KC, int max_bpc = 1 << 20) {
    int slices = (C + NCV * KC - 1) / (NCV * KC);
    int bpc = resident_bpc(kernel, 256, 0, 4);
    if (bpc > max_bpc) bpc = max_bpc;
    return dim3((unsigned)resident_grid_x(bpc, slices, (rows + 31) / 32), (unsigned)slices);
}

static inline dim3 slice_grid(i64 rows, int C, int KC, int cap = 2048) {
    int slices = (C + NCV * KC - 1) / (NCV * KC);
    i64 bx = (rows + 31) / 32;
    int capx = (cap + slices - 1) / slices;
    if (bx > capx) bx = capx;
    if (bx < 1) bx = 1;
    return dim3((unsigned)bx, (unsigned)slices);
}

static inline dim3 fat_slice_grid(i64 rows, int C, int KC) {
    int slices = (C + NCV * KC - 1) / (NCV * KC);
    i64 bx = 256 / slices;
    i64 need = (rows + (1024 / NCV) - 1) / (1024 / NCV);
    if (bx > need) bx = need;
    if (bx < 1) bx = 1;
    return dim3((unsigned)bx, (unsigned)slices);
}

static_assert(DWN_NREP == 32, "replica reduce below assumes 32 replicas");
__device__ __forceinline__ void rep_reduce(const double* stats, int stat_c, int sc, int r, bool ok, double& s, double& ss) {
    s = ok ? stats[((i64)r * 2 + 0) * stat_c + sc] : 0.0;
    ss = ok ? stats[((i64)r * 2 + 1) * stat_c + sc] : 0.0;
#pragma unroll
    for (int o = 16; o > 0; o >>= 1) { s += __shfl_xor(s, o); ss += __shfl_xor(ss, o); }
}

__device__ __forceinline__ void bn_finalize_train_body(const int blk, const double* stats, int stat_c, double count,
                                                       const float* gamma, const float* beta, float* running_mean,
                                                       float* running_var, long long* nbt, float momentum, float eps,
                                                       float* coef, int C) {
    const int r = threadIdx.x & 31;
    const int c = blk * 8 + (threadIdx.x >> 5);
    if (c == 0 && r == 0 && nbt) *nbt += 1;
    const bool ok = c < C;
    const int sc = ok ? c % stat_c : 0;
    double s, ss;
    rep_reduce(stats, stat_c, sc, r, ok, s, ss);
    if (!ok || r != 0) return;
    double mean = s / count;
    double var = ss / count - mean * mean;
    if (var < 0) var = 0;
    float invstd = (float)(1.0 / sqrt(var + (double)eps));
    float scale = gamma[c] * invstd;
    coef[c] = scale;
    coef[C + c] = beta[c] - (float)mean * scale;
    coef[2 * C + c] = (float)mean;
    coef[3 * C + c] = invstd;
    if (running_mean) {
        double unbiased = count > 1 ? var * count / (count - 1) : var;
        running_mean[c] = (1.f - momentum) * running_mean[c] + momentum * (float)mean;
        running_var[c] = (1.f - momentum) * running_var[c] + momentum * (float)unbiased;
    }
}
__global__ __launch_bounds__(256) void bn_finalize_train_kernel(BnFinJob j0, BnFinJob j1, float momentum, float eps) {
    const bool first = (int)blockIdx.x < j0.nblocks;
    const BnFinJob& j = first ? j0 : j1;
    bn_finalize_train_body(first ? blockIdx.x : blockIdx.x - j0.nblocks, j.stats, j.stat_c, j.count, j.gamma, j.beta,
                           j.running_mean, j.running_var, j.nbt, momentum, eps, j.coef, j.C);
}

__global__ void bn_finalize_eval_kernel(const float* gamma, const float* beta, const float* running_mean,
                                        const float* running_var, float eps, float* coef, int C) {
    int c = blockIdx.x * blockDim.x + threadIdx.x;
    if (c >= C) return;
    float invstd = 1.0f / sqrtf(running_var[c] + eps);
    float scale = gamma[c] * invstd;
    coef[c] = scale;
    coef[C + c] = beta[c] - running_mean[c] * scale;
    coef[2 * C + c] = running_mean[c];
    coef[3 * C + c] = invstd;
// ... 184 lines not shown
    DET_WAVES_END
    __syncthreads();
    DET_ENTER();
    if (tid < STEM_NM) {
        const double v = lsum[tid];
        if (v != 0.0) atomicAdd(mom + (i64)(blockIdx.x % DWN_NREP) * STEM_NM + tid, v);
    }
    DET_EXIT();
}

__global__ __launch_bounds__(256) void stem_bn_finalize_kernel(const double* mom, double count, const float* w, const float* gamma,
                                                               const float* beta, float* running_mean, float* running_var,
                                                               long long* nbt, float momentum, float eps, float* coef,
                                                               double* xmom, int C0, int Cin) {
    __shared__ double lm[STEM_NM];
    const int tid = threadIdx.x;
    if (tid < STEM_NM) {
        double v = 0.0;
        for (int r = 0; r < DWN_NREP; ++r) v += mom[(i64)r * STEM_NM + tid];
        lm[tid] = v;
    }
    __syncthreads();
    if (tid < STEM_NM) {
        const int a_ = tid < STEM_MAXCIN ? 0 : (tid - STEM_MAXCIN) / STEM_MAXCIN, b_ = tid < STEM_MAXCIN ? 0 : (tid - STEM_MAXCIN) % STEM_MAXCIN;
        double v = lm[tid];
        if (tid >= STEM_MAXCIN && b_ < a_) v = lm[STEM_MAXCIN + b_ * STEM_MAXCIN + a_];
        xmom[tid] = v;
    }
    if (tid == 0 && nbt) *nbt += 1;
    for (int c = tid; c < C0; c += blockDim.x) {
        double mean = 0.0, var = 0.0;
        for (int a_ = 0; a_ < Cin; ++a_) mean += (double)w[c * Cin + a_] * (lm[a_] / count);
        for (int a_ = 0; a_ < Cin; ++a_)
            for (int b_ = 0; b_ < Cin; ++b_) {
                const double sxx = a_ <= b_ ? lm[STEM_MAXCIN + a_ * STEM_MAXCIN + b_] : lm[STEM_MAXCIN + b_ * STEM_MAXCIN + a_];
                const double cov = sxx / count - (lm[a_] / count) * (lm[b_] / count);
                var += (double)w[c * Cin + a_] * (double)w[c * Cin + b_] * cov;
            }
        if (var < 0) var = 0;
        const float invstd = (float)(1.0 / sqrt(var + (double)eps));
        const float scale = gamma[c] * invstd;
        coef[c] = scale;
        coef[C0 + c] = beta[c] - (float)mean * scale;
        coef[2 * C0 + c] = (float)mean;
        coef[3 * C0 + c] = invstd;
        if (running_mean) {
            const double unbiased = count > 1 ? var * count / (count - 1) : var;
            running_mean[c] = (1.f - momentum) * running_mean[c] + momentum * (float)mean;
            running_var[c] = (1.f - momentum) * running_var[c] + momentum * (float)unbiased;
        }
    }
}

template <typename T, int CINT>
__global__ __launch_bounds__(256) void stem_out_kernel(const float* x, const float* w, const float* coef, const float* pe_t,
                                                       const float* pe_h, const float* pe_w, int Tn, int H, int W, int B,
                                                       int Cin, i64 S, int C0, T* out) {
    SLICE_SETUP(C0)
    constexpr int STEM_MAXCIN = CINT;
    const int chs_ = chan_ok ? chan : 0;
    float wr[STEM_MAXCIN][KC], sc[KC], sh[KC];
#pragma unroll
    for (int c = 0; c < STEM_MAXCIN; ++c)
#pragma unroll
        for (int i = 0; i < KC; ++i) wr[c][i] = (c < Cin && chan_ok) ? w[(chan + i) * Cin + c] : 0.f;
    ld_coef<KC>(coef + chs_, sc);
    ld_coef<KC>(coef + C0 + chs_, sh);
    const RasterIdx ro(H, W);
    const UDiv32 dT((unsigned)Tn), dS((unsigned)S);
    constexpr int RU = 2;
    const unsigned nrows = (unsigned)((i64)B * S), stride = gridDim.x * 32u;
    for (unsigned row0 = blockIdx.x * 32u + pl; row0 < nrows; row0 += RU * stride) {
        float xm[RU], xv[RU][STEM_MAXCIN];
#pragma unroll
        for (int u = 0; u < RU; ++u) {
            const unsigned row = row0 + u * stride < nrows ? row0 + u * stride : row0;
            const unsigned b = dS.div(row), sp = row - b * (unsigned)S;
            xm[u] = cv < Cin ? x[((i64)b * Cin + cv) * S + sp] : 0.f;
        }
#pragma unroll
        for (int u = 0; u < RU; ++u)
#pragma unroll
            for (int c = 0; c < STEM_MAXCIN; ++c) xv[u][c] = __shfl(xm[u], (tid & 56) | c);
#pragma unroll
        for (int u = 0; u < RU; ++u) {
            const unsigned row = row0 + u * stride;
            if (row >= nrows || !chan_ok) break;
            float v[KC];
#pragma unroll
            for (int i = 0; i < KC; ++i) v[i] = 0.f;
#pragma unroll
            for (int c = 0; c < STEM_MAXCIN; ++c)
#pragma unroll
                for (int i = 0; i < KC; ++i) v[i] = fmaf(wr[c][i], xv[u][c], v[i]);
#pragma unroll
            for (int i = 0; i < KC; ++i) v[i] = fmaf(v[i], sc[i], sh[i]);
            if (pe_t) {
                unsigned f; int h, wq;
                ro.decode(row, f, h, wq);
                const unsigned t = f - dT.div(f) * (unsigned)Tn;
                float pa[KC], pb[KC], pc[KC];
                ld_coef<KC>(pe_t + (i64)t * C0 + chan, pa);
                ld_coef<KC>(pe_h + (i64)h * C0 + chan, pb);
                ld_coef<KC>(pe_w + (i64)wq * C0 + chan, pc);
#pragma unroll
                for (int i = 0; i < KC; ++i) v[i] = round_t<T>(v[i]) + ((pa[i] + pb[i]) + pc[i]);
            }
            st_vec<T>(out + (i64)row * C0 + chan, v);
        }
    }
}

template <typename T, int CINT>
__global__ __launch_bounds__(256) void stem_bwd_acc_kernel(const T* dout, const float* x, const double* xmom, double count,
                                                           int B, int Cin, i64 S, int C0, double* acc) {
    SLICE_SETUP(C0)
    constexpr int NVG = ::STEM_MAXCIN + 1;
    constexpr int STEM_MAXCIN = CINT;
    constexpr int NV = STEM_MAXCIN + 1;
    __shared__ float lacc[NV * NCV * KC];
    for (int i = tid; i < NV * NCV * KC; i += 256) lacc[i] = 0.f;
    __syncthreads();
    float a_[NV][KC];
#pragma unroll
    for (int c = 0; c < NV; ++c)
#pragma unroll
        for (int i = 0; i < KC; ++i) a_[c][i] = 0.f;
    const float xbar_mine = cv < Cin ? (float)(xmom[cv] / count) : 0.f;
    const unsigned rows = (unsigned)((i64)B * S);
    const UDiv32 dS((unsigned)S);
    const int chs_ = chan_ok ? chan : 0;
    {
        constexpr int RU = 4;
        const unsigned stride = gridDim.x * 32u;
        for (unsigned row0 = blockIdx.x * 32u + pl; row0 < rows; row0 += RU * stride) {
            float g[RU][KC], xm[RU], xv[RU][STEM_MAXCIN];
#pragma unroll
            for (int u = 0; u < RU; ++u) {
                const unsigned row = row0 + u * stride < rows ? row0 + u * stride : row0;
                const unsigned b = dS.div(row), sp = row - b * (unsigned)S;
                ld_vec<T>(dout + (i64)row * C0 + chs_, g[u]);
                xm[u] = cv < Cin ? x[((i64)b * Cin + cv) * S + sp] - xbar_mine : 0.f;
            }
#pragma unroll
            for (int u = 0; u < RU; ++u)
#pragma unroll
                for (int c = 0; c < STEM_MAXCIN; ++c) xv[u][c] = __shfl(xm[u], (tid & 56) | c);
#pragma unroll
            for (int u = 0; u < RU; ++u) {
                if (row0 + u * stride >= rows || !chan_ok) break;
#pragma unroll
                for (int c = 0; c < STEM_MAXCIN; ++c)
#pragma unroll
                    for (int i = 0; i < KC; ++i) a_[c][i] = fmaf(g[u][i], xv[u][c], a_[c][i]);
#pragma unroll
                for (int i = 0; i < KC; ++i) a_[STEM_MAXCIN][i] += g[u][i];
            }
        }
    }
    DET_WAVES_BEGIN
#pragma unroll
    for (int c = 0; c < NV; ++c) {
        if (c < STEM_MAXCIN && c >= Cin) continue;
// ... 23 lines not shown
    const int part = threadIdx.x & 3;
    for (int cb = 0; cb < C0; cb += blockDim.x / 4) {
        const int c = cb + (threadIdx.x >> 2);
        const bool ok = c < C0;
        double dx[STEM_MAXCIN], s1 = 0.0;
        for (int k = 0; k < STEM_MAXCIN; ++k) dx[k] = 0.0;
        for (int r = part * (DWN_NREP / 4); r < (part + 1) * (DWN_NREP / 4); ++r) {
            const double* p = acc + ((i64)r * C0 + (ok ? c : 0)) * NV;
            for (int k = 0; k < Cin; ++k) dx[k] += p[k];
            s1 += p[STEM_MAXCIN];
        }
        for (int o = 1; o < 4; o <<= 1) {
            for (int k = 0; k < STEM_MAXCIN; ++k) dx[k] += __shfl_xor(dx[k], o);
            s1 += __shfl_xor(s1, o);
        }
        if (!ok || part != 0) continue;
        const double scale = coef[c], invstd = coef[3 * C0 + c];
        double dyc = 0.0;
        for (int k = 0; k < Cin; ++k) dyc += (double)w[c * Cin + k] * dx[k];
        const double s2 = invstd * dyc;
        if (dgamma) dgamma[c] = (float)s2;
        if (dbeta) dbeta[c] = (float)s1;
        const double a2 = -scale * invstd * (s2 / count);
        for (int k = 0; k < Cin; ++k) {
            double cw = 0.0;
            for (int l = 0; l < Cin; ++l)
                cw += (double)w[c * Cin + l] * (xmom[STEM_MAXCIN + l * STEM_MAXCIN + k] - xmom[l] * xmom[k] / count);
            dw[c * Cin + k] = (float)(scale * dx[k] + a2 * cw);
        }
    }
}

int k_stem_xmom(const float* x, int B, int Cin, i64 S, double* mom, hipStream_t s) {
    if (Cin > STEM_MAXCIN) return dwn_set_error(-4, "stem: in_channels > 8 not built");
    i64 bx = ((i64)B * S + 255) / 256;
    if (bx > 1024) bx = 1024;
    hipLaunchKernelGGL(stem_xmom_kernel, dim3((unsigned)bx), dim3(256), 0, s, x, B, Cin, S, mom);
    DWN_CHECK_LAUNCH();
    return 0;
}
int k_stem_bn_finalize(const double* mom, double count, const float* w, const float* gamma, const float* beta, float* rm,
                       float* rv, long long* nbt, float momentum, float eps, float* coef, double* xmom, int C0, int Cin,
                       hipStream_t s) {
    hipLaunchKernelGGL(stem_bn_finalize_kernel, dim3(1), dim3(256), 0, s, mom, count, w, gamma, beta, rm, rv, nbt, momentum, eps,
                       coef, xmom, C0, Cin);
    DWN_CHECK_LAUNCH();
    return 0;
}
template <typename T, int CINT>
static void stem_out_launch(const float* x, const float* w, const float* coef, const float* pe_t, const float* pe_h, const float* pe_w,
                            int Tn, int H, int W, int B, int Cin, i64 S, int C0, void* out, hipStream_t s) {
    auto kern = stem_out_kernel<T, CINT>;
    hipLaunchKernelGGL(kern, resident_slice_grid(kern, (i64)B * S, C0, TT<T>::KC), dim3(256), 0, s, x, w, coef, pe_t, pe_h, pe_w, Tn, H, W,
                       B, Cin, S, C0, (T*)out);
}
int k_stem_out(const float* x, const float* w, const float* coef, const float* pe_t, const float* pe_h, const float* pe_w,
               int Tn, int H, int W, int B, int Cin, i64 S, int C0, void* out, int dtype, hipStream_t s) {
    if (Cin > STEM_MAXCIN) return dwn_set_error(-4, "stem: in_channels > 8 not built");
    if ((i64)B * S >= (1ll << 31)) return dwn_set_error(-4, "stem: more than 2^31 rows");
    if (Cin <= 5) {
        DISPATCH_T(dtype, (stem_out_launch<bf16_t, 5>(x, w, coef, pe_t, pe_h, pe_w, Tn, H, W, B, Cin, S, C0, out, s)),
                   (stem_out_launch<float, 5>(x, w, coef, pe_t, pe_h, pe_w, Tn, H, W, B, Cin, S, C0, out, s)));
    } else {
        DISPATCH_T(dtype, (stem_out_launch<bf16_t, 8>(x, w, coef, pe_t, pe_h, pe_w, Tn, H, W, B, Cin, S, C0, out, s)),
                   (stem_out_launch<float, 8>(x, w, coef, pe_t, pe_h, pe_w, Tn, H, W, B, Cin, S, C0, out, s)));
    }
    DWN_CHECK_LAUNCH();
    return 0;
}
template <typename T, int CINT>
static void stem_bwd_acc_launch(const void* dout, const float* x, const double* xmom, double count, int B, int Cin, i64 S, int C0,
                                double* acc, hipStream_t s) {
    auto kern = stem_bwd_acc_kernel<T, CINT>;
    hipLaunchKernelGGL(kern, resident_slice_grid(kern, (i64)B * S, C0, TT<T>::KC), dim3(256), 0, s, (const T*)dout, x, xmom, count, B, Cin,
                       S, C0, acc);
}
int k_stem_bwd_acc(const void* dout, const float* x, const double* xmom, double count, int B, int Cin, i64 S, int C0,
                   double* acc, int dtype, hipStream_t s) {
    if (Cin > STEM_MAXCIN) return dwn_set_error(-4, "stem: in_channels > 8 not built");
    if ((i64)B * S >= (1ll << 31)) return dwn_set_error(-4, "stem: more than 2^31 rows");
    if (Cin <= 5) {
        DISPATCH_T(dtype, (stem_bwd_acc_launch<bf16_t, 5>(dout, x, xmom, count, B, Cin, S, C0, acc, s)),
                   (stem_bwd_acc_launch<float, 5>(dout, x, xmom, count, B, Cin, S, C0, acc, s)));
    } else {
        DISPATCH_T(dtype, (stem_bwd_acc_launch<bf16_t, 8>(dout, x, xmom, count, B, Cin, S, C0, acc, s)),
                   (stem_bwd_acc_launch<float, 8>(dout, x, xmom, count, B, Cin, S, C0, acc, s)));
    }
    DWN_CHECK_LAUNCH();
    return 0;
}
int k_stem_bwd_finalize(const double* acc, const double* xmom, const float* w, const float* coef, double count, float* dgamma,
                        float* dbeta, float* dw, int C0, int Cin, hipStream_t s) {
    hipLaunchKernelGGL(stem_bwd_finalize_kernel, dim3(1), dim3(256), 0, s, acc, xmom, w, coef, count, dgamma, dbeta, dw, C0, Cin);
    DWN_CHECK_LAUNCH();
    return 0;
}
constexpr int STEM_DX_MAXC0 = 128;
__global__ __launch_bounds__(256) void stem_bwd_finalize_dx_kernel(const double* acc, const double* xmom, const float* w,
                                                                   const float* coef, double count, float* qx, int C0, int Cin) {
    constexpr int NV = STEM_MAXCIN + 1;
    __shared__ double la2[STEM_DX_MAXC0], lb[STEM_DX_MAXC0];
    const int part = threadIdx.x & 3;
    for (int cb = 0; cb < C0; cb += blockDim.x / 4) {
        const int c = cb + (threadIdx.x >> 2);
        const bool ok = c < C0;
        double dx[STEM_MAXCIN], s1 = 0.0;
        for (int k = 0; k < STEM_MAXCIN; ++k) dx[k] = 0.0;
        for (int r = part * (DWN_NREP / 4); r < (part + 1) * (DWN_NREP / 4); ++r) {
            const double* p = acc + ((i64)r * C0 + (ok ? c : 0)) * NV;
            for (int k = 0; k < Cin; ++k) dx[k] += p[k];
            s1 += p[STEM_MAXCIN];
        }
// ... 226 lines not shown
#define RES_RU 2
#define RES_TAB 256
#define RES_STAGE_TABLES(hptr, hn, wptr, wn)                                             \
    __shared__ int s_ht[RES_TAB], s_wt[RES_TAB];                                         \
    const bool tab_lds = (hn) <= RES_TAB && (wn) <= RES_TAB;                             \
    if (tab_lds) {                                                                       \
        for (int i_ = threadIdx.x; i_ < (hn); i_ += blockDim.x) s_ht[i_] = (hptr)[i_];          \
        for (int i_ = threadIdx.x; i_ < (wn); i_ += blockDim.x) s_wt[i_] = (wptr)[i_];          \
    }                                                                                    \
    __syncthreads();                                                                     \
    const int* const ht_ = tab_lds ? s_ht : (hptr);                                      \
    const int* const wt_ = tab_lds ? s_wt : (wptr);
#define SC_RU 4
#define STAT_NT 1024
template <typename T>
__global__ __launch_bounds__(STAT_NT) void shortcut_stats_kernel(LoadDesc xin, ResGeom gm, double* stats) {
    SLICE_SETUP(gm.Cin)
    __shared__ float lstat[2 * NCV * KC];
    if (tid < 2 * NCV * KC) lstat[tid] = 0.f;
    __syncthreads();
    float s0[KC], s1[KC];
#pragma unroll
    for (int i = 0; i < KC; ++i) { s0[i] = 0.f; s1[i] = 0.f; }
    const unsigned rows = (unsigned)gm.BT * gm.Hout * gm.Wout;
    const RasterIdx ro(gm.Hout, gm.Wout);
    const T* xp = reinterpret_cast<const T*>(xin.p);
    RES_STAGE_TABLES(gm.hsrc, gm.Hout, gm.wsrc, gm.Wout)
    if (chan_ok) {
        const unsigned stride = gridDim.x * (unsigned)(STAT_NT / NCV);
        for (unsigned row0 = blockIdx.x * (unsigned)(STAT_NT / NCV) + pl; row0 < rows; row0 += SC_RU * stride) {
            uint4 raw[SC_RU];
#pragma unroll
            for (int u = 0; u < SC_RU; ++u) {
                const unsigned row = row0 + u * stride < rows ? row0 + u * stride : row0;
                unsigned bt; int ho, wo;
                ro.decode(row, bt, ho, wo);
                const i64 rin = ((i64)bt * gm.Hin + ht_[ho]) * gm.Win + wt_[wo];
                raw[u] = *reinterpret_cast<const uint4*>(xp + rin * xin.ld + chan);
            }
#pragma unroll
            for (int u = 0; u < SC_RU; ++u) {
                if (row0 + u * stride >= rows) break;
                float v[KC];
                unpack16<T>(raw[u], v);
#pragma unroll
                for (int i = 0; i < KC; ++i) { s0[i] += v[i]; s1[i] += v[i] * v[i]; }
            }
        }
    }
    slice_stats_flush<KC>(lstat, s0, s1, cv, c0, gm.Cin, stats, blockIdx.x % DWN_NREP);
    DET_EXIT();
}

template <typename T>
__global__ __launch_bounds__(256) void residual_fwd_kernel(LoadDesc xin, const T* y4, const float* coef4,
                                                           const float* coefsc, const float* dscale, ResGeom gm,
                                                           const float* ope_t, const float* ope_h, const float* ope_w,
                                                           T* out) {
    SLICE_SETUP(gm.Cout)
    RES_STAGE_TABLES(gm.hsrc, gm.Hout, gm.wsrc, gm.Wout)
    if (!chan_ok) return;
    float s4[KC], t4[KC], ss[KC], ts[KC];
    ld_coef<KC>(coef4 + chan, s4); ld_coef<KC>(coef4 + gm.Cout + chan, t4);
    ld_coef<KC>(coefsc + chan, ss); ld_coef<KC>(coefsc + gm.Cout + chan, ts);
    const int csrc = chan % gm.Cin;
    const unsigned rows = (unsigned)gm.BT * gm.Hout * gm.Wout;
    const RasterIdx ro(gm.Hout, gm.Wout);
    const UDiv32 dT((unsigned)gm.T);
    const T* xp = reinterpret_cast<const T*>(xin.p);
    const unsigned stride = gridDim.x * 32u;
    for (unsigned row0 = blockIdx.x * 32u + pl; row0 < rows; row0 += RES_RU * stride) {
        uint4 rs[RES_RU], ry[RES_RU];
        unsigned btv[RES_RU]; int hov[RES_RU], wov[RES_RU];
#pragma unroll
        for (int u = 0; u < RES_RU; ++u) {
            const unsigned row = row0 + u * stride < rows ? row0 + u * stride : row0;
            ro.decode(row, btv[u], hov[u], wov[u]);
            const i64 rin = ((i64)btv[u] * gm.Hin + ht_[hov[u]]) * gm.Win + wt_[wov[u]];
            rs[u] = *reinterpret_cast<const uint4*>(xp + rin * xin.ld + csrc);
            ry[u] = *reinterpret_cast<const uint4*>(y4 + (i64)row * gm.Cout + chan);
        }
#pragma unroll
        for (int u = 0; u < RES_RU; ++u) {
            const unsigned row = row0 + u * stride;
            if (row >= rows) break;
            float sv[KC], yv[KC], o[KC];
            unpack16<T>(rs[u], sv);
            unpack16<T>(ry[u], yv);
            const unsigned b = dT.div(btv[u]);
            const float d = dscale ? dscale[b] : 1.0f;
#pragma unroll
            for (int i = 0; i < KC; ++i) o[i] = d * fmaf(yv[i], s4[i], t4[i]) + fmaf(sv[i], ss[i], ts[i]);
            if (ope_t) {
                float pa[KC], pb[KC], pc[KC];
                ld_coef<KC>(ope_t + (i64)(btv[u] - b * (unsigned)gm.T) * gm.Cout + chan, pa);
                ld_coef<KC>(ope_h + (i64)hov[u] * gm.Cout + chan, pb);
                ld_coef<KC>(ope_w + (i64)wov[u] * gm.Cout + chan, pc);
#pragma unroll
                for (int i = 0; i < KC; ++i) o[i] = round_t<T>(o[i]) + ((pa[i] + pb[i]) + pc[i]);
            }
            st_vec<T>(out + (i64)row * gm.Cout + chan, o);
        }
    }
}

#define RR_RU 2
template <typename T>
__global__ __launch_bounds__(STAT_NT) void residual_bwd_reduce_kernel(LoadDesc xin, const T* y4, const T* dout,
                                                                  const float* coef4, const float* coefsc,
                                                                  const float* dscale, ResGeom gm, double* stats4,
                                                                  double* statssc) {
    SLICE_SETUP(gm.Cout)
    __shared__ float lstat[2 * NCV * KC];
    __shared__ float lstat2[2 * NCV * KC];
    if (tid < 2 * NCV * KC) { lstat[tid] = 0.f; lstat2[tid] = 0.f; }
    RES_STAGE_TABLES(gm.hsrc, gm.Hout, gm.wsrc, gm.Wout)
    float a0[KC], a1[KC], b0[KC], b1[KC];
#pragma unroll
    for (int i = 0; i < KC; ++i) { a0[i] = a1[i] = b0[i] = b1[i] = 0.f; }
    if (chan_ok) {
        float m4[KC], i4[KC], ms[KC], is[KC];
        ld_coef<KC>(coef4 + 2 * gm.Cout + chan, m4); ld_coef<KC>(coef4 + 3 * gm.Cout + chan, i4);
        ld_coef<KC>(coefsc + 2 * gm.Cout + chan, ms); ld_coef<KC>(coefsc + 3 * gm.Cout + chan, is);
        const int csrc = chan % gm.Cin;
        const unsigned rows = (unsigned)gm.BT * gm.Hout * gm.Wout;
        const RasterIdx ro(gm.Hout, gm.Wout);
        const UDiv32 dT((unsigned)gm.T);
        const T* xp = reinterpret_cast<const T*>(xin.p);
        const unsigned stride = gridDim.x * (unsigned)(STAT_NT / NCV);
        for (unsigned row0 = blockIdx.x * (unsigned)(STAT_NT / NCV) + pl; row0 < rows; row0 += RR_RU * stride) {
            uint4 rs[RR_RU], ry[RR_RU], rg[RR_RU];
            unsigned btv[RR_RU];
#pragma unroll
            for (int u = 0; u < RR_RU; ++u) {
                const unsigned row = row0 + u * stride < rows ? row0 + u * stride : row0;
                int ho, wo;
                ro.decode(row, btv[u], ho, wo);
                const i64 rin = ((i64)btv[u] * gm.Hin + ht_[ho]) * gm.Win + wt_[wo];
                rs[u] = *reinterpret_cast<const uint4*>(xp + rin * xin.ld + csrc);
                ry[u] = *reinterpret_cast<const uint4*>(y4 + (i64)row * gm.Cout + chan);
                rg[u] = *reinterpret_cast<const uint4*>(dout + (i64)row * gm.Cout + chan);
            }
#pragma unroll
            for (int u = 0; u < RR_RU; ++u) {
                if (row0 + u * stride >= rows) break;
                float sv[KC], yv[KC], g[KC];
                unpack16<T>(rs[u], sv);
                unpack16<T>(ry[u], yv);
                unpack16<T>(rg[u], g);
                const float d = dscale ? dscale[dT.div(btv[u])] : 1.0f;
#pragma unroll
                for (int i = 0; i < KC; ++i) {
                    float gd = g[i] * d;
                    a0[i] += gd;
                    a1[i] += gd * (yv[i] - m4[i]) * i4[i];
                    b0[i] += g[i];
// ... 49 lines not shown
    if (!chan_ok) return;
    const unsigned rows = (unsigned)gm.BT * gm.Hin * gm.Win;
    const RasterIdx ri(gm.Hin, gm.Win);
    const T* xp = reinterpret_cast<const T*>(xin.p);
    const unsigned stride = gridDim.x * 32u;
    for (unsigned row0 = blockIdx.x * 32u + pl; row0 < rows; row0 += RES_RU * stride) {
        uint4 ra[RES_RU], rx[RES_RU];
        i64 routv[RES_RU];
#pragma unroll
        for (int u = 0; u < RES_RU; ++u) {
            const unsigned row = row0 + u * stride < rows ? row0 + u * stride : row0;
            unsigned bt; int hi, wi;
            ri.decode(row, bt, hi, wi);
            const int ho = ht_[hi], wo = wt_[wi];
            routv[u] = (ho >= 0 && wo >= 0) ? ((i64)bt * gm.Hout + ho) * gm.Wout + wo : -1;
            ra[u] = *reinterpret_cast<const uint4*>(da0 + (i64)row * gm.Cin + chan);
            rx[u] = make_uint4(0, 0, 0, 0);
            if (routv[u] >= 0) rx[u] = *reinterpret_cast<const uint4*>(xp + (i64)row * xin.ld + chan);
        }
#pragma unroll
        for (int u = 0; u < RES_RU; ++u) {
            const unsigned row = row0 + u * stride;
            if (row >= rows) break;
            float o[KC];
            unpack16<T>(ra[u], o);
            if (routv[u] >= 0) {
                float sv[KC];
                unpack16<T>(rx[u], sv);
                for (int cc = chan; cc < gm.Cout; cc += gm.Cin) {
                    float g[KC], a1[KC], a2[KC], a3[KC];
                    ld_vec<T>(dout + routv[u] * gm.Cout + cc, g);
                    ld_coef<KC>(abcsc + cc, a1); ld_coef<KC>(abcsc + gm.Cout + cc, a2);
                    ld_coef<KC>(abcsc + 2 * gm.Cout + cc, a3);
#pragma unroll
                    for (int i = 0; i < KC; ++i) o[i] += fmaf(a1[i], g[i], fmaf(a2[i], sv[i], a3[i]));
                }
            }
            st_vec<T>(dx + (i64)row * gm.Cin + chan, o);
        }
    }
}


int k_shortcut_stats(const LoadDesc& xin, const ResGeom& gm, double* stats, int dtype, hipStream_t s) {
    i64 rows = (i64)gm.BT * gm.Hout * gm.Wout;
    DISPATCH_T(dtype,
        hipLaunchKernelGGL((shortcut_stats_kernel<bf16_t>), fat_slice_grid(rows, gm.Cin, 8), dim3(STAT_NT), 0, s, xin, gm, stats),
        hipLaunchKernelGGL((shortcut_stats_kernel<float>), fat_slice_grid(rows, gm.Cin, 4), dim3(STAT_NT), 0, s, xin, gm, stats));
    DWN_CHECK_LAUNCH();
    return 0;
}
int k_residual_fwd(const LoadDesc& xin, const void* y4, const float* coef4, const float* coefsc, const float* dscale,
                   const ResGeom& gm, const float* ope_t, const float* ope_h, const float* ope_w, void* out, int dtype,
                   hipStream_t s) {
    i64 rows = (i64)gm.BT * gm.Hout * gm.Wout;
    DISPATCH_T(dtype,
        hipLaunchKernelGGL((residual_fwd_kernel<bf16_t>), slice_grid(rows, gm.Cout, 8), dim3(256), 0, s, xin, (const bf16_t*)y4, coef4, coefsc, dscale, gm, ope_t, ope_h, ope_w, (bf16_t*)out),
        hipLaunchKernelGGL((residual_fwd_kernel<float>), slice_grid(rows, gm.Cout, 4), dim3(256), 0, s, xin, (const float*)y4, coef4, coefsc, dscale, gm, ope_t, ope_h, ope_w, (float*)out));
    DWN_CHECK_LAUNCH();
    return 0;
}
int k_residual_bwd_reduce(const LoadDesc& xin, const void* y4, const void* dout, const float* coef4,
                          const float* coefsc, const float* dscale, const ResGeom& gm, double* stats4,
                          double* statssc, int dtype, hipStream_t s) {
    i64 rows = (i64)gm.BT * gm.Hout * gm.Wout;
    DISPATCH_T(dtype,
        hipLaunchKernelGGL((residual_bwd_reduce_kernel<bf16_t>), fat_slice_grid(rows, gm.Cout, 8), dim3(STAT_NT), 0, s, xin, (const bf16_t*)y4, (const bf16_t*)dout, coef4, coefsc, dscale, gm, stats4, statssc),
        hipLaunchKernelGGL((residual_bwd_reduce_kernel<float>), fat_slice_grid(rows, gm.Cout, 4), dim3(STAT_NT), 0, s, xin, (const float*)y4, (const float*)dout, coef4, coefsc, dscale, gm, stats4, statssc));
    DWN_CHECK_LAUNCH();
    return 0;
}
int k_residual_bwd_dy4(const void* y4, const void* dout, const float* abc4, const float* dscale, const ResGeom& gm,
                       void* dy4, int dtype, hipStream_t s) {
    i64 rows = (i64)gm.BT * gm.Hout * gm.Wout;
    DISPATCH_T(dtype,
        hipLaunchKernelGGL((residual_bwd_dy4_kernel<bf16_t>), slice_grid(rows, gm.Cout, 8), dim3(256), 0, s, (const bf16_t*)y4, (const bf16_t*)dout, abc4, dscale, gm, (bf16_t*)dy4),
        hipLaunchKernelGGL((residual_bwd_dy4_kernel<float>), slice_grid(rows, gm.Cout, 4), dim3(256), 0, s, (const float*)y4, (const float*)dout, abc4, dscale, gm, (float*)dy4));
    DWN_CHECK_LAUNCH();
    return 0;
}
int k_residual_bwd_dx(const LoadDesc& xin, const void* da0, const void* dout, const float* abcsc, const ResGeom& gm,
                      void* dx, int dtype, hipStream_t s) {
    i64 rows = (i64)gm.BT * gm.Hin * gm.Win;
    DISPATCH_T(dtype,
        hipLaunchKernelGGL((residual_bwd_dx_kernel<bf16_t>), slice_grid(rows, gm.Cin, 8), dim3(256), 0, s, xin, (const bf16_t*)da0, (const bf16_t*)dout, abcsc, gm, (bf16_t*)dx),
        hipLaunchKernelGGL((residual_bwd_dx_kernel<float>), slice_grid(rows, gm.Cin, 4), dim3(256), 0, s, xin, (const float*)da0, (const float*)dout, abcsc, gm, (float*)dx));
    DWN_CHECK_LAUNCH();
    return 0;
}

template <typename T>
__global__ __launch_bounds__(256) void se_pool_kernel(LoadDesc z3, int C, int rows_per_sample, int chunks,
                                                      long long* pooled, T* z3out) {
    SLICE_SETUP(C)
    __shared__ unsigned long long lacc[NCV * KC];
    if (tid < NCV * KC) lacc[tid] = 0ull;
    __syncthreads();
    const int b = blockIdx.x / chunks, chunk = blockIdx.x % chunks;
    const int per = (rows_per_sample + chunks - 1) / chunks;
    const int r_beg = chunk * per;
    const int r_end = (r_beg + per < rows_per_sample) ? r_beg + per : rows_per_sample;
    float acc[KC];
#pragma unroll
    for (int i = 0; i < KC; ++i) acc[i] = 0.f;
    if (chan_ok) {
        float sc[KC], sh[KC];
        ld_coef<KC>(z3.v1 + chan, sc);
        ld_coef<KC>(z3.v2 + chan, sh);
        const T* yp = reinterpret_cast<const T*>(z3.p);
        for (int r0 = r_beg + pl; r0 < r_end; r0 += 4 * 32) {
            uint4 raw[4];
// ... 1551 lines not shown
```

### sensorium_amd/csrc/dwn_kernels.h

```cpp
#pragma once
#include "dwn_internal.h"

struct ResGeom {
    int BT, T, Hin, Win, Hout, Wout, Cin, Cout;
    const int* hsrc; const int* wsrc;
    const int* hinv; const int* winv;
};

typedef dwn_tensor_entry TensorListEntry;

struct BnFinJob {
    const double* stats; int stat_c; double count; const float* gamma; const float* beta;
    float* running_mean; float* running_var; long long* nbt; float* coef; int C; int nblocks;
};
struct BnBwdJob { const double* stats; double count; const float* coef; float* dgamma; float* dbeta; float* abc; int C; int nblocks; int frozen; };
int k_bn_finalize_train(BnFinJob j0, BnFinJob j1, float momentum, float eps, hipStream_t s);
int k_bn_bwd_finalize(BnBwdJob j0, BnBwdJob j1, hipStream_t s);
int k_bn_finalize_eval(const float* gamma, const float* beta, const float* rm, const float* rv, float eps,
                       float* coef, int C, hipStream_t s);
int k_bn1_gram_finalize(const double* gram, const float* w1, int E, int Cin, double count, const float* gamma, const float* beta,
                        float* rm, float* rv, long long* nbt, float momentum, float eps, float* coef, double* sc_stats, int dtype,
                        hipStream_t s);
int k_ew_apply(const LoadDesc& d, int kind, void* out, i64 ldo, i64 rows, int C, int dtype, hipStream_t s);
int k_stem_xmom(const float* x, int B, int Cin, i64 S, double* mom, hipStream_t s);
int k_stem_bn_finalize(const double* mom, double count, const float* w, const float* gamma, const float* beta, float* rm,
                       float* rv, long long* nbt, float momentum, float eps, float* coef, double* xmom, int C0, int Cin,
                       hipStream_t s);
int k_stem_out(const float* x, const float* w, const float* coef, const float* pe_t, const float* pe_h, const float* pe_w,
               int Tn, int H, int W, int B, int Cin, i64 S, int C0, void* out, int dtype, hipStream_t s);
int k_stem_bwd_acc(const void* dout, const float* x, const double* xmom, double count, int B, int Cin, i64 S, int C0,
                   double* acc, int dtype, hipStream_t s);
int k_stem_bwd_finalize(const double* acc, const double* xmom, const float* w, const float* coef, double count, float* dgamma,
                        float* dbeta, float* dw, int C0, int Cin, hipStream_t s);
int k_stem_bwd_finalize_frozen(const double* acc, const float* w, const float* coef, float* dgamma, float* dbeta, float* dw,
                               int C0, int Cin, hipStream_t s);
int k_stem_input_grad(const void* dout, const float* w, const float* coef, int B, int Cin, i64 S, int C0, float* dx, int dtype,
                      hipStream_t s);
int k_stem_bwd_finalize_dx(const double* acc, const double* xmom, const float* w, const float* coef, double count, float* qx,
                           int C0, int Cin, hipStream_t s);
int k_stem_input_grad_train(const void* dout, const float* w, const float* coef, const float* x, const float* qx, int B, int Cin,
                            i64 S, int C0, float* dx, int dtype, hipStream_t s);
int stem_moment_count();
int stem_acc_stride();
int k_shortcut_stats(const LoadDesc& xin, const ResGeom& gm, double* stats, int dtype, hipStream_t s);
int k_residual_fwd(const LoadDesc& xin, const void* y4, const float* coef4, const float* coefsc, const float* dscale,
                   const ResGeom& gm, const float* ope_t, const float* ope_h, const float* ope_w, void* out, int dtype,
                   hipStream_t s);
int k_residual_bwd_reduce(const LoadDesc& xin, const void* y4, const void* dout, const float* coef4,
                          const float* coefsc, const float* dscale, const ResGeom& gm, double* stats4,
                          double* statssc, int dtype, hipStream_t s);
int k_residual_bwd_dy4(const void* y4, const void* dout, const float* abc4, const float* dscale, const ResGeom& gm,
                       void* dy4, int dtype, hipStream_t s);
int k_residual_bwd_dx(const LoadDesc& xin, const void* da0, const void* dout, const float* abcsc, const ResGeom& gm,
                      void* dx, int dtype, hipStream_t s);
int k_se_pool(const LoadDesc& z3, int B, int C, int rows_per_sample, long long* pooled, void* z3out, int dtype, hipStream_t s);
int k_se_mlp_fwd(const long long* pooled_sum, float inv_s, const float* wr, const float* br, const float* we,
                 const float* be, int B, int C, int R, float* pmean, float* hid_pre, float* gate, const float* w2, void* wg, int N2,
                 int dtype, int* folded, hipStream_t s);
int k_se_mlp_bwd(const float* dg, const float* gate, const float* hid_pre, const float* pmean, const float* wr,
                 const float* we, int B, int C, int R, float inv_s, float* dgp, float* dhp, float* dps, float* dwr,
                 float* dbr, float* dwe, float* dbe, hipStream_t s);
int k_bn3_bwd_reduce(const LoadDesc& d, const float* coef3, i64 rows, int C, double* stats, void* dh_out, int dtype, hipStream_t s);
int k_pool_fwd(const void* x, void* out, i64 BT, int HW, int C, int dtype, hipStream_t s);
int k_pool_bwd(const void* dpool, void* dx, i64 BT, int HW, int C, int dtype, hipStream_t s);
int k_cortex_residual_fwd(const void* y, const void* x, const float* coef, const float* coefsc, const float* dscale,
                          int M, int Tn, int Cin, int C, int groups, void* out, int dtype, hipStream_t s);
int k_cortex_stats(const void* y, const void* x, int M, int Cin, int C, double* stats, double* statssc, int dtype, hipStream_t s);
int k_cortex_bwd_reduce(const void* y, const void* x, const void* dout, const float* gmask, int gmask_ld,
                        const float* coef, const float* coefsc, const float* dscale, int M, int Tn, int Cin, int C,
                        int groups, double* stats, double* statssc, int dtype, hipStream_t s);
int k_cortex_bwd_dy(const void* y, const void* dout, const float* gmask, int gmask_ld, const float* coef,
                    const float* abc, const float* dscale, int M, int Tn, int C, int groups, void* dy, int dtype,
                    hipStream_t s);
int k_cortex_bwd_dx(const void* dxmain, const void* x, const void* dout, const float* gmask, int gmask_ld,
                    const float* abcsc, int M, int Tn, int Cin, int C, void* dx, int dtype, hipStream_t s);
int k_pack_weight(const float* src, void* dst, int groups, int R, int C, int transpose, int Rd, int Cd, int dtype,
                  hipStream_t s);
int k_gate_weights(const float* w, const float* gate, void* dst, int B, int N, int K, int dtype, hipStream_t s);
size_t k_readout_dbeta_parts(int B, int Rp, int groups);
int k_readout_dz(const float* dout, const float* out, float beta, const float* beta_dev, double* part, float* dbeta, int B, int Tn, int n_valid, int Rg, int Rp,
                 int groups, void* dz, float* db, int dtype, hipStream_t s);
int k_poisson_fwd(const float* pred, const float* target, const float* w, i64 per_sample, i64 total, float eps,
                  double* loss, hipStream_t s);
int k_poisson_bwd(const float* pred, const float* target, const float* w, const float* gscale, i64 per_sample,
                  i64 total, float eps, float* dpred, hipStream_t s);
int k_f64_to_f32(const double* src, float* dst, int n, hipStream_t s);
int k_adamw_ema(const TensorListEntry* list, int ntensors, int max_blocks, float decay_w, float omb1, float beta2,
                float omb2, float eps, float step_size, float bc2_sqrt, float ema_decay, float ema_omd,
                float grad_scale, hipStream_t s);
int k_ema_lerp(const TensorListEntry* list, int ntensors, int max_blocks, float decay, float omd, hipStream_t s);
int k_grad_sumsq(const dwn_guarded_entry* list, int ntensors, int max_blocks, double grad_scale, void* ws, double* pair,
                 hipStream_t s);
int k_step_guard_finalize(const double* pair_a, const double* pair_b, double max_norm, int skip_nonfinite,
                          const dwn_guarded_entry* list, int ntensors, dwn_step_guard* guard, hipStream_t s);
int k_adamw_ema_guarded(const dwn_guarded_entry* list, int ntensors, int max_blocks, double lr, double beta1, double beta2,
                        double eps, double weight_decay, double ema_decay, double grad_scale, const dwn_step_guard* guard,
                        hipStream_t s);
int k_fill_f32(float* p, float v, int n, hipStream_t s);
int k_pack_weight_dual(const float* src, void* plain, void* tr, int groups, int R, int C, int Rp, int ldp, int ldt, int dtype,
                       hipStream_t s);
// ... 94 lines not shown
```

### sensorium_amd/dwiseneuro.py

```python
from __future__ import annotations

import math
from typing import Optional, Sequence

import torch
from torch import nn

from . import ops


def _select_dtype(explicit: Optional[torch.dtype]) -> torch.dtype:
    if explicit is not None:
        return explicit
    if torch.is_autocast_enabled():
        return torch.bfloat16
    return torch.float32


class BatchNormAct(nn.Module):

    def __init__(self, num_features: int, bn_layer=nn.BatchNorm3d, apply_act: bool = True):
        super().__init__()
        self.bn = bn_layer(num_features)
        self.apply_act = apply_act
# ... 71 lines not shown
        self.temp_covn_dw = nn.Sequential(
            nn.Conv3d(mid, mid, (temporal_kernel, 1, 1), stride=(1, 1, 1), padding=(tp, 0, 0), groups=mid,
                      bias=False),
            BatchNormAct(mid))
        self.se = SqueezeExcite3d(mid, reduce_ratio=se_reduce_ratio)
        self.conv_pwl = nn.Sequential(nn.Conv3d(mid, out_features, (1, 1, 1), bias=False),
                                      BatchNormAct(out_features, apply_act=False))
        self.drop_path = DropPath(drop_prob=drop_path_rate)
        self.bn_sc = BatchNormAct(out_features, apply_act=False)
        self._geom_cache: dict = {}

    def __deepcopy__(self, memo):
        cache, self._geom_cache = self._geom_cache, {}
        try:
            cls = self.__class__
            new = cls.__new__(cls)
            memo[id(self)] = new
            import copy
            for k, v in self.__dict__.items():
                setattr(new, k, copy.deepcopy(v, memo))
            return new
        finally:
            self._geom_cache = cache

    def bn_modules(self):
        return [self.conv_pw[1].bn, self.spat_covn_dw[1].bn, self.temp_covn_dw[1].bn, self.conv_pwl[1].bn,
                self.bn_sc.bn]

    def parameters_in_kernel_order(self):
        bn = self.bn_modules()
        return (self.conv_pw[0].weight, bn[0].weight, bn[0].bias,
                self.spat_covn_dw[0].weight, bn[1].weight, bn[1].bias,
                self.temp_covn_dw[0].weight, bn[2].weight, bn[2].bias,
                self.se.conv_reduce.weight, self.se.conv_reduce.bias,
                self.se.conv_expand.weight, self.se.conv_expand.bias,
                self.conv_pwl[0].weight, bn[3].weight, bn[3].bias, bn[4].weight, bn[4].bias)

    def geometry(self, pe: PositionalEncoding3d, t: int, h: int, w: int, device):
        key = (t, h, w, str(device))
        geom = self._geom_cache.get(key)
        if geom is None:
            pt, ph, pw = ops.pe_axis_tables(self.in_features, pe.inv_freq, t, h, w)
            s = self.spatial_stride
            ho, wo = (h - 1) // s + 1, (w - 1) // s + 1
            hsrc = ops.nearest_src_index(ho, h)
            wsrc = ops.nearest_src_index(wo, w)
            to = lambda a: torch.as_tensor(a).to(device)
            geom = (pt.to(device), ph.to(device), pw.to(device), to(hsrc), to(wsrc),
                    to(ops.inverse_index(hsrc, h)), to(ops.inverse_index(wsrc, w)))
            self._geom_cache = {key: geom}
        return geom

    def forward(self, x: torch.Tensor, pe: PositionalEncoding3d, dtype: torch.dtype, x_has_pe: bool = False,
                out_pe=None) -> torch.Tensor:
        b, t, h, w, _ = x.shape
        geom = self.geometry(pe, t, h, w, x.device)
        drop = self.drop_path.sample(b, x.device)
        mode = ops.bn_mode(self.conv_pw[1].bn.training, x)
        return ops.BlockFn.apply(x, drop, self, geom, dtype, x_has_pe, out_pe, mode, *self.parameters_in_kernel_order())


class ShuffleLayer(nn.Module):

    def __init__(self, in_features: int, out_features: int, groups: int = 1, drop_path_rate: float = 0.0):
        super().__init__()
        self.in_features = in_features
        self.out_features = out_features
        self.groups = groups
        self.conv = nn.Conv1d(in_features, out_features, (1,), groups=groups, bias=False)
        self.bn = BatchNormAct(out_features, bn_layer=nn.BatchNorm1d)
        self.drop_path = DropPath(drop_prob=drop_path_rate)
        self.bn_sc = BatchNormAct(out_features, bn_layer=nn.BatchNorm1d, apply_act=False)

    def forward(self, x: torch.Tensor, dtype: torch.dtype) -> torch.Tensor:
        drop = self.drop_path.sample(x.shape[0], x.device)
        mode = ops.bn_mode(self.bn.bn.training, x)
        return ops.CortexFn.apply(x, drop, self, dtype, mode, self.conv.weight, self.bn.bn.weight, self.bn.bn.bias,
                                  self.bn_sc.bn.weight, self.bn_sc.bn.bias)


class Cortex(nn.Module):

    def __init__(self, in_features: int, features: Sequence[int], groups: int = 1, drop_path_rate: float = 0.0):
        super().__init__()
        self.layers = nn.Sequential()
        prev = in_features
        for num_features in features:
            self.layers.append(ShuffleLayer(prev, num_features, groups=groups, drop_path_rate=drop_path_rate))
            prev = num_features

    def forward(self, x: torch.Tensor, dtype: torch.dtype) -> torch.Tensor:
        for layer in self.layers:
            x = layer(x, dtype)
        return x


class SoftplusGate(nn.Module):

    def __init__(self, softplus_beta: float, param: str = "beta"):
        super().__init__()
        if param not in ("beta", "log"):
            raise ValueError("softplus_param: 'beta' or 'log'")
        if not float(softplus_beta) > 0.0:
            raise ValueError("a learnable Softplus beta must start positive")
        self.param = param
        if param == "beta":
            self.beta = nn.Parameter(torch.tensor(float(softplus_beta), dtype=torch.float32))
        else:
            self.log_beta = nn.Parameter(torch.tensor(math.log(float(softplus_beta)), dtype=torch.float32))

    def value(self) -> torch.Tensor:
        return self.beta if self.param == "beta" else self.log_beta.float().exp()
# ... 22 lines not shown

    def beta(self) -> torch.Tensor:
        if self.learnable_softplus:
            return self.gate.value().detach()
        return torch.tensor(self.softplus_beta, dtype=torch.float32, device=self.layer[1].weight.device)

    def forward(self, x: torch.Tensor) -> torch.Tensor:
        mask = None
        if self.training and self.drop_rate > 0.0:
            keep = 1.0 - self.drop_rate
            mask = torch.empty(x.shape[0], x.shape[2], dtype=torch.float32, device=x.device).bernoulli_(keep)
            mask.div_(keep)
        conv = self.layer[1]
        if self.learnable_softplus:
            return ops.ReadoutFn.apply(x, mask, self, conv.weight, conv.bias, self.gate.value())
        return ops.ReadoutFn.apply(x, mask, self, conv.weight, conv.bias)


class DepthwiseCore(nn.Module):

    def __init__(self, in_channels: int = 1, features: Sequence[int] = (64, 128, 256, 512),
                 spatial_strides: Sequence[int] = (2, 2, 2, 2), spatial_kernel: int = 3, temporal_kernel: int = 3,
                 expansion_ratio: int = 3, se_reduce_ratio: int = 16, drop_path_rate: float = 0.0):
        super().__init__()
        num_blocks = len(features)
        assert num_blocks and num_blocks == len(spatial_strides)
        self.stem = nn.Sequential(nn.Conv3d(in_channels, features[0], (1, 1, 1), bias=False),
                                  BatchNormAct(features[0], apply_act=False))
        blocks = []
        nxt = features[0]
        for i in range(num_blocks):
            if i < num_blocks - 1:
                nxt = features[i + 1]
            blocks += [
                PositionalEncoding3d(features[i]),
                InvertedResidual3d(features[i], nxt, spatial_kernel=spatial_kernel, temporal_kernel=temporal_kernel,
                                   spatial_stride=spatial_strides[i], expansion_ratio=expansion_ratio,
                                   se_reduce_ratio=se_reduce_ratio,
                                   drop_path_rate=drop_path_rate * i / num_blocks, bias=False),
            ]
        self.blocks = nn.Sequential(*blocks)

    def forward(self, x: torch.Tensor, dtype: torch.dtype) -> torch.Tensor:
        bn = self.stem[1].bn
        mods = list(self.blocks)
        pes, blks = mods[0::2], mods[1::2]
        _, _, t, h, w = x.shape
        sizes = []
        for blk in blks:
            sizes.append((h, w))
            s = blk.spatial_stride
            h, w = (h - 1) // s + 1, (w - 1) // s + 1
        tables = [blk.geometry(pe, t, hw[0], hw[1], x.device)[:3] for pe, blk, hw in zip(pes, blks, sizes)]
        x = ops.StemFn.apply(x, self.stem[0].weight, bn.weight, bn.bias, self, dtype, tables[0], ops.bn_mode(bn.training, x))
        for i, (pe, blk) in enumerate(zip(pes, blks)):
            x = blk(x, pe, dtype, True, tables[i + 1] if i + 1 < len(blks) else None)
        return x


class DwiseNeuro(nn.Module):

    def __init__(self,
                 readout_outputs: Sequence[int],
                 in_channels: int = 5,
                 core_features: Sequence[int] = (64, 64, 64, 64, 128, 128, 128, 256, 256),
                 spatial_strides: Sequence[int] = (2, 1, 1, 1, 2, 1, 1, 2, 1),
                 spatial_kernel: int = 3,
                 temporal_kernel: int = 5,
                 expansion_ratio: int = 6,
                 se_reduce_ratio: int = 32,
                 cortex_features: Sequence[int] = (1024, 2048, 4096),
                 groups: int = 2,
                 softplus_beta: float = 0.07,
                 drop_rate: float = 0.4,
                 drop_path_rate: float = 0.1,
                 compute_dtype: Optional[torch.dtype] = None,
                 learnable_softplus: bool = False,
                 softplus_param: str = "beta"):
        super().__init__()
        self.compute_dtype = compute_dtype
        self.fp32_eval_products = "bf16x3"
        self.bn_frozen_finetune = False
        self.core = DepthwiseCore(in_channels=in_channels, features=core_features, spatial_strides=spatial_strides,
                                  spatial_kernel=spatial_kernel, temporal_kernel=temporal_kernel,
                                  expansion_ratio=expansion_ratio, se_reduce_ratio=se_reduce_ratio,
                                  drop_path_rate=drop_path_rate)
        self.pool = nn.AdaptiveAvgPool3d((None, 1, 1))
        self.cortex = Cortex(in_features=core_features[-1], features=cortex_features, groups=groups,
                             drop_path_rate=drop_path_rate)
        self.readouts = nn.ModuleList()
        for n in readout_outputs:
            self.readouts.append(Readout(in_features=cortex_features[-1], out_features=n, groups=groups,
                                         softplus_beta=softplus_beta, drop_rate=drop_rate,
                                         learnable_softplus=learnable_softplus, softplus_param=softplus_param))

    def softplus_parameters(self):
        return [p for r in self.readouts if r.learnable_softplus for p in r.gate.parameters()]

    def set_fp32_eval_products(self, mode: str = "bf16x3") -> "DwiseNeuro":
        if mode not in ("bf16x3", "native"):
            raise ValueError("fp32 eval products: 'bf16x3' or 'native'")
        self.fp32_eval_products = mode
        for m in self.modules():
            if isinstance(m, (InvertedResidual3d, ShuffleLayer, Readout)):
                m._dwn_fp32_native = mode == "native"
        return self

    def freeze_batchnorm(self, flag: bool = True) -> "DwiseNeuro":
        self.bn_frozen_finetune = bool(flag)
# ... 44 lines not shown
```

### sensorium_amd/ops.py

```python
from __future__ import annotations

import ctypes as C
import math
import os
import threading
from typing import Optional

import numpy as np
import torch
from torch.autograd.function import once_differentiable

from . import _lib as L

_DT = {torch.float32: L.DWN_F32, torch.bfloat16: L.DWN_BF16}


def _ptr(t: Optional[torch.Tensor]):
    return None if t is None else t.data_ptr()


def _stream(device: torch.device):
    return torch.cuda.current_stream(device).cuda_stream


# ... 33 lines not shown

class _BnModeState(threading.local):
    override: Optional[int] = None


_BN_MODE = _BnModeState()


class bn_mode_scope:

    def __init__(self, mode: Optional[int]):
        self.mode = mode

    def __enter__(self):
        self.prev, _BN_MODE.override = _BN_MODE.override, self.mode
        return self

    def __exit__(self, *exc):
        _BN_MODE.override = self.prev
        return False


def wants_frozen(x: torch.Tensor, switch: bool = False) -> bool:
    return torch.is_grad_enabled() and (bool(x.requires_grad) or switch)


def bn_mode(training: bool, x: torch.Tensor) -> int:
    if training:
        return L.BN_TRAIN
    if _BN_MODE.override is not None:
        return _BN_MODE.override
    return L.BN_FROZEN if wants_frozen(x) else L.BN_EVAL


def _ddp_flush() -> None:
    from . import ddp
    if ddp._LIVE:
        ddp.flush_ready_all()


def _ws(nbytes: int, device) -> torch.Tensor:
    return torch.empty(int(nbytes), dtype=torch.uint8, device=device)


def _env_choice(name: str, table: dict) -> int:
    v = os.environ.get(name, "")
    if v not in table:
        raise ValueError(f"{name}={v!r}: expected one of {sorted(k for k in table if k)} (or unset)")
    return table[v]


_PWL_BWD = _env_choice("DWN_PWL_BWD", {"": 0, "new": 1, "old": 2})
_Y1_MODE = _env_choice("DWN_Y1", {"": 0, "free": 0, "materialise": 1, "all": 2})


def grad_out(param: torch.Tensor, zero: bool = False) -> torch.Tensor:
    slot = getattr(param, "_dwn_grad_slot", None)
    if slot is not None and param.grad is None and not getattr(param, "_dwn_slot_out", False):
        param._dwn_slot_out = True
        flat, off = slot
        g = flat[off:off + param.numel()].view(param.shape)
        return g.zero_() if zero else g
    if zero:
        return torch.zeros_like(param, dtype=torch.float32)
    return torch.empty_like(param, dtype=torch.float32)


def nearest_src_index(out_size: int, in_size: int) -> np.ndarray:
    scale = np.float32(in_size) / np.float32(out_size)
    src = np.floor(np.arange(out_size, dtype=np.float32) * scale).astype(np.int64)
    return np.minimum(src, in_size - 1).astype(np.int32)


def inverse_index(src: np.ndarray, in_size: int) -> np.ndarray:
    inv = np.full(in_size, -1, dtype=np.int32)
    inv[src] = np.arange(len(src), dtype=np.int32)
    if len(np.unique(src)) != len(src):
        raise RuntimeError("nearest-neighbour shortcut map is not injective (stride < 1?)")
    return inv


def pe_axis_tables(channels: int, inv_freq: torch.Tensor, t: int, h: int, w: int):
    ch = int(math.ceil(channels / 6) * 2)
    if ch % 2:
        ch += 1
    inv = inv_freq.detach().float().cpu()
    tabs = []
    for axis, size in enumerate((t, h, w)):
        arg = inv[:, None] * torch.arange(size).float()[None, :]
        emb = torch.cat([arg.sin(), arg.cos()], dim=0)
        tab = torch.zeros(size, channels, dtype=torch.float32)
        lo = axis * ch
        n = max(0, min(ch, channels - lo))
        if n > 0:
            tab[:, lo:lo + n] = emb[:n].t()
        tabs.append(tab.contiguous())
    return tabs


class StemFn(torch.autograd.Function):

    @staticmethod
    def forward(ctx, x, weight, gamma, beta, mod, dtype, pe=None, mode=None):
        _require_gpu(x, "StemFn")
        conv, bn = mod.stem[0], mod.stem[1].bn
        _check_bn(bn)
        if mode is None:
            mode = int(bn.training)
        x = x.contiguous().float()
        B, Cin, T, H, W = x.shape
        C0 = weight.shape[0]
        dev = x.device
        out = torch.empty(B, T, H, W, C0, dtype=dtype, device=dev)
        coef = torch.empty(4 * C0, dtype=torch.float32, device=dev)
        xmom = torch.empty(72, dtype=torch.float64, device=dev)
        a = L.StemArgs()
        a.dtype = _DT[dtype]; a.training = mode; a.B = B; a.Cin = Cin; a.C0 = C0; a.S = T * H * W
        a.eps = bn.eps; a.momentum = bn.momentum
        a.x = x.data_ptr(); a.w = weight.data_ptr(); a.bn = _bn_struct(bn, coef)
        a.out = out.data_ptr(); a.xmom = xmom.data_ptr()
        if pe is not None:
            a.pe_t, a.pe_h, a.pe_w = (t.data_ptr() for t in pe)
        a.T, a.H, a.W = T, H, W
        ws = _ws(L.lib.dwn_stem_workspace_bytes(C.byref(a)), dev)
        a.ws = ws.data_ptr(); a.ws_bytes = ws.numel()
        L.check(L.lib.dwn_stem_forward(C.byref(a), dev.index, _stream(dev)), "dwn_stem_forward")
        ctx.mod = mod; ctx.dtype = dtype; ctx.mode = mode
        ctx.save_for_backward(x, weight, xmom, coef)
        return out

    @staticmethod
    def backward(ctx, dout):
        x, weight, xmom, coef = ctx.saved_tensors
        if ctx.mode == L.BN_EVAL:
            raise RuntimeError(_EVAL_BACKWARD_ERROR)
        bn = ctx.mod.stem[1].bn
        dev = x.device
        B, Cin, T, H, W = x.shape
        C0 = weight.shape[0]
        dout = dout.contiguous()
        dx = None
        if ctx.needs_input_grad[0] and ctx.mode == L.BN_FROZEN:
            dx = torch.empty_like(x)
            g = L.StemInputGradArgs()
            g.dtype = _DT[ctx.dtype]; g.training = ctx.mode; g.B = B; g.Cin = Cin; g.C0 = C0; g.S = T * H * W
            g.w = weight.data_ptr(); g.coef = coef.data_ptr(); g.dout = dout.data_ptr(); g.dx = dx.data_ptr()
            L.check(L.lib.dwn_stem_input_grad(C.byref(g), dev.index, _stream(dev)), "dwn_stem_input_grad")
            if not any(ctx.needs_input_grad[1:4]):
                return dx, None, None, None, None, None, None, None
        dw = grad_out(ctx.mod.stem[0].weight)
        dgamma = grad_out(bn.weight)
        dbeta = grad_out(bn.bias)
        a = L.StemArgs()
        a.dtype = _DT[ctx.dtype]; a.training = ctx.mode; a.B = B; a.Cin = Cin; a.C0 = C0; a.S = T * H * W
        a.eps = bn.eps; a.momentum = bn.momentum
        a.x = x.data_ptr(); a.w = weight.data_ptr(); a.bn = _bn_struct(bn, coef, dgamma, dbeta)
        a.xmom = xmom.data_ptr(); a.dout = dout.data_ptr(); a.dw = dw.data_ptr()
        ws = _ws(L.lib.dwn_stem_workspace_bytes(C.byref(a)), dev)
        a.ws = ws.data_ptr(); a.ws_bytes = ws.numel()
        if ctx.needs_input_grad[0] and ctx.mode == L.BN_TRAIN:
            dx = torch.empty_like(x)
            L.check(L.lib.dwn_stem_backward_input(C.byref(a), dx.data_ptr(), dev.index, _stream(dev)), "dwn_stem_backward_input")
        else:
            L.check(L.lib.dwn_stem_backward(C.byref(a), dev.index, _stream(dev)), "dwn_stem_backward")
        return dx, dw, dgamma, dbeta, None, None, None, None


_BLOCK_PARAMS = ("w_pw", "g1", "b1", "w_dws", "g2", "b2", "w_dwt", "g3", "b3", "se_wr", "se_br", "se_we", "se_be",
                 "w_pwl", "g4", "b4", "gsc", "bsc")


def _block_args(blk, geom, x, dtype, training, coefs, saved, drop_scale, x_has_pe, a0):
    B, T, Hin, Win, Cin = x.shape
    a = L.BlockArgs()
    a.dtype = _DT[dtype]; a.training = int(training)
    a.B = B; a.T = T; a.Hin = Hin; a.Win = Win
    a.Hout = (Hin - 1) // blk.spatial_stride + 1
    a.Wout = (Win - 1) // blk.spatial_stride + 1
    a.Cin = Cin; a.Cmid = blk.mid_features; a.Cout = blk.out_features
    a.stride = blk.spatial_stride; a.ks = blk.spatial_kernel; a.kt = blk.temporal_kernel
    a.se_r = blk.se.conv_reduce.out_channels
    bn1 = blk.conv_pw[1].bn
    a.eps = bn1.eps; a.momentum = bn1.momentum
    a.x = x.data_ptr()
    a.x_has_pe = int(x_has_pe)
    a.a0 = _ptr(a0)
    pe_t, pe_h, pe_w, hsrc, wsrc, hinv, winv = geom
    a.pe_t = pe_t.data_ptr(); a.pe_h = pe_h.data_ptr(); a.pe_w = pe_w.data_ptr()
    a.hsrc = hsrc.data_ptr(); a.wsrc = wsrc.data_ptr(); a.hinv = hinv.data_ptr(); a.winv = winv.data_ptr()
    a.w_pw = blk.conv_pw[0].weight.data_ptr()
    a.w_dws = blk.spat_covn_dw[0].weight.data_ptr()
    a.w_dwt = blk.temp_covn_dw[0].weight.data_ptr()
    a.w_pwl = blk.conv_pwl[0].weight.data_ptr()
    a.se_wr = blk.se.conv_reduce.weight.data_ptr(); a.se_br = blk.se.conv_reduce.bias.data_ptr()
    a.se_we = blk.se.conv_expand.weight.data_ptr(); a.se_be = blk.se.conv_expand.bias.data_ptr()
    a.drop_scale = _ptr(drop_scale)
    a.se_pmean = saved["pmean"].data_ptr(); a.se_hidpre = saved["hidpre"].data_ptr()
    a.se_gate = saved["gate"].data_ptr()
    a.f32_products = _f32_products(blk)
    a.y1_mode = getattr(blk, "_dwn_y1_mode", _Y1_MODE)
    return a


class BlockFn(torch.autograd.Function):

    @staticmethod
    def forward(ctx, x, drop_scale, blk, geom, dtype, x_has_pe, out_pe, mode, *params):
        _require_gpu(x, "BlockFn")
        x = x.contiguous()
        dev = x.device
        B, T, Hin, Win, Cin = x.shape
        s = blk.spatial_stride
        Hout, Wout = (Hin - 1) // s + 1, (Win - 1) // s + 1
        Cmid, Cout = blk.mid_features, blk.out_features
        bns = blk.bn_modules()
        for bn in bns:
            _check_bn(bn)
        training = mode
        f32 = dict(dtype=torch.float32, device=dev)
        y2 = torch.empty(B, T, Hout, Wout, Cmid, dtype=dtype, device=dev)
        z3 = torch.empty_like(y2)
        a0 = None if x_has_pe else torch.empty_like(x)
        y4 = torch.empty(B, T, Hout, Wout, Cout, dtype=dtype, device=dev)
        out = torch.empty_like(y4)
        coefs = [torch.empty(4 * c, **f32) for c in (Cmid, Cmid, Cmid, Cout, Cout)]
        R = blk.se.conv_reduce.out_channels
        saved = dict(pmean=torch.empty(B, Cmid, **f32), hidpre=torch.empty(B, R, **f32),
                     gate=torch.empty(B, Cmid, **f32))
        a = _block_args(blk, geom, x, dtype, training, coefs, saved, drop_scale, x_has_pe, a0)
        a.out = out.data_ptr()
        writes = L.lib.dwn_block_forward_writes(C.byref(a))
        y1 = torch.empty(B, T, Hin, Win, Cmid, dtype=dtype, device=dev) if writes & 1 else None
        y3 = torch.empty_like(y2) if writes & 2 else None
        a.y1 = _ptr(y1); a.y2 = y2.data_ptr(); a.y3 = _ptr(y3); a.y4 = y4.data_ptr()
        a.z3 = z3.data_ptr()
        if out_pe is not None:
            a.out_pe_t, a.out_pe_h, a.out_pe_w = (t.data_ptr() for t in out_pe)
        a.bn1, a.bn2, a.bn3, a.bn4, a.bnsc = (_bn_struct(bn, cf) for bn, cf in zip(bns, coefs))
        ws = _ws(L.lib.dwn_block_workspace_bytes(C.byref(a), 0), dev)
        a.ws = ws.data_ptr(); a.ws_bytes = ws.numel()
        L.check(L.lib.dwn_block_forward(C.byref(a), dev.index, _stream(dev)), "dwn_block_forward")
        ctx.blk = blk; ctx.geom = geom; ctx.dtype = dtype; ctx.mode = mode
        if getattr(blk, "_capture", False):
            blk._captured = dict(y1=y1, y2=y2, y3=y3, y4=y4, z3=z3, coefs=coefs, **saved)
        ctx.has_drop = drop_scale is not None
        if mode == L.BN_EVAL:
            return out
        tensors = [x if x_has_pe else a0, y1, y2, y3, y4, *coefs, saved["pmean"], saved["hidpre"], saved["gate"], z3]
        if drop_scale is not None:
            tensors.append(drop_scale)
        ctx.save_for_backward(*tensors)
        return out

    @staticmethod
    def backward(ctx, dout):
        if ctx.mode == L.BN_EVAL:
            raise RuntimeError(_EVAL_BACKWARD_ERROR)
        blk, dtype = ctx.blk, ctx.dtype
        t = ctx.saved_tensors
        x, y1, y2, y3, y4 = t[:5]
        coefs = list(t[5:10])
        saved = dict(pmean=t[10], hidpre=t[11], gate=t[12])
        z3 = t[13]
        drop_scale = t[14] if ctx.has_drop else None
        dev = x.device
        dout = dout.contiguous()
        B, T, Hin, Win, Cin = x.shape
        Hout, Wout = y2.shape[2], y2.shape[3]
        Cmid, Cout = blk.mid_features, blk.out_features
        f32 = dict(dtype=torch.float32, device=dev)
        a = _block_args(blk, ctx.geom, x, dtype, ctx.mode, coefs, saved, drop_scale, True, None)
        a.y1 = _ptr(y1); a.y2 = y2.data_ptr(); a.y3 = y3.data_ptr(); a.y4 = y4.data_ptr()
        a.z3 = z3.data_ptr()
        bns = blk.bn_modules()
        dg = [grad_out(bn.weight) for bn in bns]
        db = [grad_out(bn.bias) for bn in bns]
        a.bn1, a.bn2, a.bn3, a.bn4, a.bnsc = (_bn_struct(bn, cf, g_, b_) for bn, cf, g_, b_ in zip(bns, coefs, dg, db))
        m_in, m_out = B * T * Hin * Win, B * T * Hout * Wout
        buf_a = torch.empty(max(m_in, m_out) * Cmid, dtype=dtype, device=dev)
        buf_b = torch.empty(m_out * Cmid, dtype=dtype, device=dev)
        dy4 = torch.empty(m_out * Cout, dtype=dtype, device=dev)
        da0 = torch.empty(m_in * Cin, dtype=dtype, device=dev)
        dx = torch.empty_like(x)
        R = blk.se.conv_reduce.out_channels
        dw_pw = grad_out(blk.conv_pw[0].weight)
        dw_dws = grad_out(blk.spat_covn_dw[0].weight)
        dw_dwt = grad_out(blk.temp_covn_dw[0].weight)
        dw_pwl = grad_out(blk.conv_pwl[0].weight)
        dse_wr = grad_out(blk.se.conv_reduce.weight); dse_br = grad_out(blk.se.conv_reduce.bias)
        dse_we = grad_out(blk.se.conv_expand.weight); dse_be = grad_out(blk.se.conv_expand.bias)
        a.dout = dout.data_ptr(); a.dx = dx.data_ptr()
        a.buf_a = buf_a.data_ptr(); a.buf_b = buf_b.data_ptr(); a.dy4 = dy4.data_ptr(); a.da0 = da0.data_ptr()
        a.dw_pw = dw_pw.data_ptr(); a.dw_dws = dw_dws.data_ptr(); a.dw_dwt = dw_dwt.data_ptr()
        a.dw_pwl = dw_pwl.data_ptr()
        a.dse_wr = dse_wr.data_ptr(); a.dse_br = dse_br.data_ptr(); a.dse_we = dse_we.data_ptr()
        a.dse_be = dse_be.data_ptr()
        a.pwl_bwd = _PWL_BWD
        ws = _ws(L.lib.dwn_block_workspace_bytes(C.byref(a), 1), dev)
        a.ws = ws.data_ptr(); a.ws_bytes = ws.numel()
        L.check(L.lib.dwn_block_backward(C.byref(a), dev.index, _stream(dev)), "dwn_block_backward")
        _ddp_flush()
        grads = (dw_pw, dg[0], db[0], dw_dws, dg[1], db[1], dw_dwt, dg[2], db[2], dse_wr, dse_br, dse_we, dse_be,
                 dw_pwl, dg[3], db[3], dg[4], db[4])
        return (dx, None, None, None, None, None, None, None) + grads


class PoolFn(torch.autograd.Function):

    @staticmethod
    def forward(ctx, x):
        _require_gpu(x, "PoolFn")
        x = x.contiguous()
        B, T, H, W, Cc = x.shape
        out = torch.empty(B, T, Cc, dtype=x.dtype, device=x.device)
        a = L.PoolArgs()
        a.dtype = _DT[x.dtype]; a.BT = B * T; a.HW = H * W; a.C = Cc; a.x = x.data_ptr(); a.out = out.data_ptr()
        L.check(L.lib.dwn_pool_forward(C.byref(a), x.device.index, _stream(x.device)), "dwn_pool_forward")
        ctx.shape = (B, T, H, W, Cc)
        return out

    @staticmethod
    def backward(ctx, dout):
        B, T, H, W, Cc = ctx.shape
        dout = dout.contiguous()
        dx = torch.empty(B, T, H, W, Cc, dtype=dout.dtype, device=dout.device)
        a = L.PoolArgs()
        a.dtype = _DT[dout.dtype]; a.BT = B * T; a.HW = H * W; a.C = Cc; a.dout = dout.data_ptr(); a.dx = dx.data_ptr()
        L.check(L.lib.dwn_pool_backward(C.byref(a), dout.device.index, _stream(dout.device)), "dwn_pool_backward")
        return dx


class CortexFn(torch.autograd.Function):

    @staticmethod
    def forward(ctx, x, drop_scale, layer, dtype, mode, weight, g, b, gsc, bsc):
        _require_gpu(x, "CortexFn")
        x = x.contiguous()
        dev = x.device
        B, T, Cin = x.shape
        Cc = layer.out_features
        bn, bnsc = layer.bn.bn, layer.bn_sc.bn
        _check_bn(bn); _check_bn(bnsc)
        y = torch.empty(B, T, Cc, dtype=dtype, device=dev)
        out = torch.empty_like(y)
        coef = torch.empty(4 * Cc, dtype=torch.float32, device=dev)
        coefsc = torch.empty(4 * Cc, dtype=torch.float32, device=dev)
        a = L.CortexArgs()
        a.dtype = _DT[dtype]; a.training = mode; a.B = B; a.T = T; a.Cin = Cin; a.C = Cc
        a.groups = layer.groups; a.eps = bn.eps; a.momentum = bn.momentum
        a.x = x.data_ptr(); a.out = out.data_ptr(); a.y = y.data_ptr(); a.w = weight.data_ptr()
        a.bn = _bn_struct(bn, coef); a.bnsc = _bn_struct(bnsc, coefsc); a.drop_scale = _ptr(drop_scale)
        a.f32_products = _f32_products(layer)
        ws = _ws(L.lib.dwn_cortex_workspace_bytes(C.byref(a), 0), dev)
        a.ws = ws.data_ptr(); a.ws_bytes = ws.numel()
        L.check(L.lib.dwn_cortex_forward(C.byref(a), dev.index, _stream(dev)), "dwn_cortex_forward")
        ctx.layer = layer; ctx.dtype = dtype; ctx.mode = mode; ctx.has_drop = drop_scale is not None
        tensors = [x, y, coef, coefsc, weight]
# ... 825 lines not shown
```

Before: 1477.

## Fuse next block's BN1 Gram matrix into producer output kernels

The stem output kernel and the block residual-forward kernel now, when given a gram_out buffer, also accumulate the 64x64 Gram matrix (plus a column-sum row) of the tile they just wrote. They do this with bf16 MFMA on LDS-staged tiles and flush to global with f64 atomics. The next block then takes that matrix as gram_in and skips its own TN GEMM pass over the input that it used to compute BatchNorm-1 statistics. This removes one full read of each block's input activations. The cost is extra LDS, MFMA work, atomics and a changed launch config in the producer kernels, plus reduced determinism and tighter constraints (bf16, 64 channels, training mode only).

```diff
diff --git a/include/dwn.h b/include/dwn.h
--- a/include/dwn.h
+++ b/include/dwn.h
@@ -157,6 +157,7 @@
     float* dw;
     void* ws; size_t ws_bytes;
     double* xmom;
+    double* gram_out;
 } dwn_stem_args;
 
 typedef struct dwn_stem_input_grad_args {
@@ -191,6 +192,8 @@
     int pwl_bwd;
     int f32_products;
     int y1_mode;
+    double* gram_out;
+    const double* gram_in;
 } dwn_block_args;
 
 typedef struct dwn_pool_args {
@@ -308,6 +311,9 @@
 int dwn_block_forward(const dwn_block_args* a, int device, void* stream);
 int dwn_block_backward(const dwn_block_args* a, int device, void* stream);
 int dwn_block_forward_writes(const dwn_block_args* a);
+int dwn_block_takes_gram(const dwn_block_args* a);
+int dwn_stem_output_pass(const dwn_stem_args* a, int device, void* stream);
+int dwn_block_residual_pass(const dwn_block_args* a, int device, void* stream);
 int dwn_pool_forward(const dwn_pool_args* a, int device, void* stream);
 int dwn_pool_backward(const dwn_pool_args* a, int device, void* stream);
 size_t dwn_cortex_workspace_bytes(const dwn_cortex_args* a, int backward);
diff --git a/sensorium_amd/_lib.py b/sensorium_amd/_lib.py
--- a/sensorium_amd/_lib.py
+++ b/sensorium_amd/_lib.py
@@ -88,7 +88,8 @@
                 ("eps", c_f), ("momentum", c_f), ("x", c_p), ("w", c_p), ("bn", BN),
                 ("pe_t", c_p), ("pe_h", c_p), ("pe_w", c_p), ("T", c_i), ("H", c_i), ("W", c_i),
                 ("y0", c_p), ("out", c_p),
-                ("dout", c_p), ("dw", c_p), ("ws", c_p), ("ws_bytes", c_sz), ("xmom", c_p)]
+                ("dout", c_p), ("dw", c_p), ("ws", c_p), ("ws_bytes", c_sz), ("xmom", c_p),
+                ("gram_out", c_p)]
 
 
 class StemInputGradArgs(C.Structure):
@@ -113,7 +114,8 @@
                 ("dout", c_p), ("dx", c_p), ("buf_a", c_p), ("buf_b", c_p), ("dy4", c_p), ("da0", c_p),
                 ("dw_pw", c_p), ("dw_dws", c_p), ("dw_dwt", c_p), ("dw_pwl", c_p), ("dse_wr", c_p),
                 ("dse_br", c_p), ("dse_we", c_p), ("dse_be", c_p),
-                ("ws", c_p), ("ws_bytes", c_sz), ("pwl_bwd", c_i), ("f32_products", c_i), ("y1_mode", c_i)]
+                ("ws", c_p), ("ws_bytes", c_sz), ("pwl_bwd", c_i), ("f32_products", c_i), ("y1_mode", c_i),
+                ("gram_out", c_p), ("gram_in", c_p)]
 
 
 class PoolArgs(C.Structure):
@@ -319,6 +321,9 @@
     "dwn_block_forward": (c_i, [_P(BlockArgs), c_i, c_p]),
     "dwn_block_backward": (c_i, [_P(BlockArgs), c_i, c_p]),
     "dwn_block_forward_writes": (c_i, [_P(BlockArgs)]),
+    "dwn_block_takes_gram": (c_i, [_P(BlockArgs)]),
+    "dwn_stem_output_pass": (c_i, [_P(StemArgs), c_i, c_p]),
+    "dwn_block_residual_pass": (c_i, [_P(BlockArgs), c_i, c_p]),
     "dwn_pool_forward": (c_i, [_P(PoolArgs), c_i, c_p]),
     "dwn_pool_backward": (c_i, [_P(PoolArgs), c_i, c_p]),
     "dwn_cortex_workspace_bytes": (c_sz, [_P(CortexArgs), c_i]),
@@ -421,7 +426,7 @@
                            "dwn_trial_score_finalize", "dwn_spatial_gain_ws_bytes", "dwn_spatial_gain_forward",
                            "dwn_spatial_gain_backward", "dwn_noise_forward", "dwn_sta_state_bytes", "dwn_sta_ws_bytes",
                            "dwn_sta_accumulate", "dwn_sta_finalize", "dwn_gauss2d_ws_bytes", "dwn_gauss2d_fit",
-                           "dwn_gauss2d_profile") and not hasattr(lib, name):
+                           "dwn_gauss2d_profile", "dwn_block_takes_gram", "dwn_stem_output_pass", "dwn_block_residual_pass") and not hasattr(lib, name):
             continue
         fn = getattr(lib, name)
         fn.restype = restype
diff --git a/sensorium_amd/csrc/dwn_api.hip b/sensorium_amd/csrc/dwn_api.hip
--- a/sensorium_amd/csrc/dwn_api.hip
+++ b/sensorium_amd/csrc/dwn_api.hip
@@ -401,8 +401,20 @@
     double* mom = c.take<double>((size_t)DWN_NREP * stem_moment_count());
     if (!c.ok()) return dwn_set_error(-6, "stem: workspace too small");
     const i64 M = (i64)a->B * a->S;
+    if (a->gram_out) {
+        if (a->training != DWN_BN_TRAIN) return dwn_set_error(-2, "stem_forward: gram_out is for batch statistics (DWN_BN_TRAIN) only");
+        if (a->dtype != DWN_BF16 || a->C0 != 64) return dwn_set_error(-4, "stem_forward: gram_out is built for bf16 and 64 stem channels");
+        if ((size_t)a->gram_out & 15) return dwn_set_error(-2, "stem_forward: gram_out must be 16-byte aligned");
+    }
     if (a->training == DWN_BN_TRAIN) {
         if (!a->xmom) return dwn_set_error(-1, "stem_forward: xmom buffer required in training mode");
+        if (a->gram_out) {
+            PrepArgs pa;
+            if (!pa.zero(mom, (size_t)DWN_NREP * stem_moment_count() * sizeof(double)) ||
+                !pa.zero(a->gram_out, (size_t)(a->C0 + 8) * a->C0 * sizeof(double)))
+                return dwn_set_error(-2, "stem_forward: workspace must be 16-byte aligned");
+            TRY(k_prep(pa, a->dtype, s));
+        } else
         TRY(k_zero(mom, (size_t)DWN_NREP * stem_moment_count() * sizeof(double), s));
         TRY(k_stem_xmom(a->x, a->B, a->Cin, a->S, mom, s));
         TRY(k_stem_bn_finalize(mom, (double)M, a->w, a->bn.gamma, a->bn.beta, a->bn.running_mean, a->bn.running_var,
@@ -411,7 +423,7 @@
         TRY(bn_finalize(nullptr, a->C0, (double)M, a->bn, a->C0, 0, a->momentum, a->eps, s));
     }
     return k_stem_out(a->x, a->w, a->bn.coef, a->pe_t, a->pe_h, a->pe_w, a->T, a->H, a->W, a->B, a->Cin, a->S, a->C0, a->out,
-                      a->dtype, s);
+                      a->dtype, a->gram_out, s);
 }
 int dwn_stem_backward(const dwn_stem_args* a, int device, void* stream) {
     ENTER(device);
@@ -483,6 +495,13 @@
     const dwn_block_args& a = *ap;
     hipStream_t s = (hipStream_t)stream;
     TRY(check_block(a));
+    if (a.gram_out) {
+        if (a.training != DWN_BN_TRAIN) return dwn_set_error(-2, "block_forward: gram_out is for batch statistics (DWN_BN_TRAIN) only");
+        if (a.dtype != DWN_BF16 || a.Cout != 64) return dwn_set_error(-4, "block_forward: gram_out is built for bf16 and 64 output channels");
+        if ((size_t)a.gram_out & 15) return dwn_set_error(-2, "block_forward: gram_out must be 16-byte aligned");
+    }
+    if (a.gram_in && !dwn_block_takes_gram(ap))
+        return dwn_set_error(-2, "block_forward: gram_in only where BatchNorm-1's statistics come from the Gram matrix (dwn_block_takes_gram)");
     BlockWs w = carve_block(a, 0, a.ws, a.ws_bytes);
     if (w.bytes > a.ws_bytes) return dwn_set_error(-6, "block_forward: workspace too small");
     const int dt = a.dtype, tr = a.training != DWN_BN_EVAL;
@@ -492,6 +511,7 @@
     {
         PrepArgs pa;
         bool ok = pa.zero(w.zero_beg, ((size_t)(w.zero_end - w.zero_beg) + 15) & ~(size_t)15);
+        if (a.gram_out) ok = ok && pa.zero(a.gram_out, (size_t)(a.Cout + 8) * a.Cout * sizeof(double));
         ok = ok && pa.packw(a.w_pw, w.wpw, 1, a.Cmid, a.Cin, 0, a.Cmid, a.Cin);
         ok = ok && pa.packw(a.w_pwl, w.wpwl, 1, a.Cout, a.Cmid, 0, a.Cout, a.Cmid);
         ok = ok && pa.packdw(a.w_dws, w.wdws, a.Cmid, a.ks * a.ks);
@@ -531,10 +551,12 @@
         LoadDesc cat = ld_plain(a0, a.Cin);
         cat.cat_c1 = a.Cin; cat.cat_c2 = 0;
         if (bs) {
+        if (!a.gram_in) {
         GemmTN g = tn_base(cat, LD_CAT1, ld_plain(a0, a.Cin), LD_PLAIN, (int)Min, a.Cin + 8, a.Cin, reinterpret_cast<float*>(w.gram), a.Cin, 1);
         g.dw_f64 = 1;
         PROF(DWN_FAM_PW_FWD, launch_gemm_tn(g, dt, s));
-        PROF(DWN_FAM_PW_FWD, k_bn1_gram_finalize(w.gram, a.w_pw, a.Cmid, a.Cin, (double)Min, a.bn1.gamma, a.bn1.beta, a.bn1.running_mean,
+        }
+        PROF(DWN_FAM_PW_FWD, k_bn1_gram_finalize(a.gram_in ? a.gram_in : w.gram, a.w_pw, a.Cmid, a.Cin, (double)Min, a.bn1.gamma, a.bn1.beta, a.bn1.running_mean,
                                                  a.bn1.running_var, a.bn1.num_batches_tracked, a.momentum, a.eps, a.bn1.coef,
                                                  identity_sc ? w.stsc : nullptr, dt, s));
         }
@@ -607,7 +629,7 @@
                                  fin_job(w.stsc, a.Cin, (double)Mout, a.bnsc, a.Cout), a.momentum, a.eps, s));
     }
     PROF(DWN_FAM_RESID_FWD, k_residual_fwd(xin, a.y4, a.bn4.coef, a.bnsc.coef, a.drop_scale, gm, a.out_pe_t, a.out_pe_h,
-                                           a.out_pe_w, a.out, dt, s));
+                                           a.out_pe_w, a.out, dt, a.gram_out, s));
     return 0;
 }
 
@@ -763,6 +785,41 @@
     }
     return 1;
 }
+int dwn_block_takes_gram(const dwn_block_args* ap) { return ap->training == DWN_BN_TRAIN && block_y1_free(*ap) ? 1 : 0; }
+
+static int gram_out_check(const double* gram, int dtype, int C, const char* who) {
+    if (!gram) return 0;
+    if (dtype != DWN_BF16 || C != 64) { snprintf(g_err, sizeof(g_err), "%s: gram_out is built for bf16 and 64 output channels", who); return -4; }
+    if ((size_t)gram & 15) { snprintf(g_err, sizeof(g_err), "%s: gram_out must be 16-byte aligned", who); return -2; }
+    return 0;
+}
+int dwn_stem_output_pass(const dwn_stem_args* a, int device, void* stream) {
+    g_err[0] = 0;
+    if (!a || !a->x || !a->w || !a->bn.coef || !a->out) return dwn_set_error(-1, "stem_output_pass: null pointer (x, w, bn.coef, out)");
+    if (a->C0 <= 0 || a->C0 % 8 || a->Cin <= 0 || a->B <= 0 || a->S <= 0) return dwn_set_error(-2, "stem_output_pass: C0 a positive multiple of 8; B, Cin, S positive");
+    if (a->pe_t && (i64)a->T * a->H * a->W != a->S) return dwn_set_error(-2, "stem_output_pass: T*H*W != S");
+    if (int rc = gram_out_check(a->gram_out, a->dtype, a->C0, "stem_output_pass")) return rc;
+    if (a->gram_out && a->Cin > 5) return dwn_set_error(-4, "stem_output_pass: gram_out is built for at most 5 input channels");
+    ENTER(device);
+    hipStream_t s = (hipStream_t)stream;
+    if (a->gram_out) TRY(k_zero(a->gram_out, (size_t)(a->C0 + 8) * a->C0 * sizeof(double), s));
+    return k_stem_out(a->x, a->w, a->bn.coef, a->pe_t, a->pe_h, a->pe_w, a->T, a->H, a->W, a->B, a->Cin, a->S, a->C0, a->out,
+                      a->dtype, a->gram_out, s);
+}
+int dwn_block_residual_pass(const dwn_block_args* ap, int device, void* stream) {
+    g_err[0] = 0;
+    if (!ap) return dwn_set_error(-1, "block_residual_pass: null pointer");
+    const dwn_block_args& a = *ap;
+    if (!a.x || !a.y4 || !a.bn4.coef || !a.bnsc.coef || !a.out || !a.hsrc || !a.wsrc)
+        return dwn_set_error(-1, "block_residual_pass: null pointer (x, y4, bn4.coef, bnsc.coef, out, hsrc, wsrc)");
+    if (int rc = check_block(a)) return rc;
+    if (int rc = gram_out_check(a.gram_out, a.dtype, a.Cout, "block_residual_pass")) return rc;
+    ENTER(device);
+    hipStream_t s = (hipStream_t)stream;
+    if (a.gram_out) TRY(k_zero(a.gram_out, (size_t)(a.Cout + 8) * a.Cout * sizeof(double), s));
+    return k_residual_fwd(ld_plain(a.x, a.Cin), a.y4, a.bn4.coef, a.bnsc.coef, a.drop_scale, geom_of(a), a.out_pe_t, a.out_pe_h, a.out_pe_w,
+                          a.out, a.dtype, a.gram_out, s);
+}
 
 int dwn_pool_forward(const dwn_pool_args* a, int device, void* stream) {
     ENTER(device);
diff --git a/sensorium_amd/csrc/dwn_elementwise.hip b/sensorium_amd/csrc/dwn_elementwise.hip
--- a/sensorium_amd/csrc/dwn_elementwise.hip
+++ b/sensorium_amd/csrc/dwn_elementwise.hip
@@ -64,6 +64,91 @@
     if (bx < 1) bx = 1;
     return dim3((unsigned)bx, (unsigned)slices);
 }
+
+typedef __attribute__((ext_vector_type(8))) short pg_bf16x8_t;
+typedef __attribute__((ext_vector_type(4))) short pg_s16x4_t;
+typedef __attribute__((ext_vector_type(4))) float pg_f32x4_t;
+constexpr int PG_NT = 512;
+constexpr int PG_C = 64;
+constexpr int PG_RPI = PG_NT / NCV;
+constexpr int PG_RS = PG_C * 2;
+constexpr int PG_MAXWG = 512;
+static inline dim3 pgram_grid(i64 rows) {
+    i64 bx = (rows + 511) / 512;
+    return dim3((unsigned)(bx > PG_MAXWG ? PG_MAXWG : bx < 1 ? 1 : bx), 1u);
+}
+__device__ __forceinline__ void pg_lds_barrier() {
+    asm volatile("s_waitcnt lgkmcnt(0)" ::: "memory");
+    __builtin_amdgcn_s_barrier();
+}
+struct PGItems { int a0, b0, a1, b1, n; };
+__device__ __forceinline__ PGItems pg_items(int wave) {
+    switch (wave) {
+        case 0: return {0, 0, 0, 1, 2};
+        case 1: return {0, 2, 0, 3, 2};
+        case 2: return {1, 1, 1, 2, 2};
+        case 3: return {1, 3, 3, 3, 2};
+        case 4: return {2, 2, 2, 3, 2};
+        case 5: return {4, 0, 4, 1, 2};
+        case 6: return {4, 2, 4, 3, 2};
+        default: return {3, 3, 3, 3, 0};
+    }
+}
+template <int NROWS>
+struct PGram {
+    static constexpr int BYTES = NROWS * PG_RS;
+    static_assert(NROWS % 32 == 0, "whole 32-row k-steps");
+    static_assert(PG_NT == 512, "pg_items deals the tiles to 8 waves");
+    pg_f32x4_t acc[2];
+    __device__ __forceinline__ PGram() { acc[0] = acc[1] = pg_f32x4_t{0.f, 0.f, 0.f, 0.f}; }
+    static __device__ __forceinline__ void put(unsigned char* tile, int r, int cv, const uint4& v) {
+        *reinterpret_cast<uint4*>(tile + r * PG_RS + (((cv >> 1) ^ ((r >> 1) & 3)) * 32) + (cv & 1) * 16) = v;
+    }
+    static __device__ __forceinline__ pg_bf16x8_t frag(const unsigned char* lane_ptr, int kb) {
+        auto lo = __builtin_amdgcn_ds_read_tr16_b64_v4i16((__attribute__((address_space(3))) pg_s16x4_t*)(lane_ptr + kb * 32 * PG_RS));
+        auto hi = __builtin_amdgcn_ds_read_tr16_b64_v4i16((__attribute__((address_space(3))) pg_s16x4_t*)(lane_ptr + (kb * 32 + 8) * PG_RS));
+        return pg_bf16x8_t{lo[0], lo[1], lo[2], lo[3], hi[0], hi[1], hi[2], hi[3]};
+    }
+    __device__ __forceinline__ void mma(const unsigned char* tile) {
+        const int lane = threadIdx.x & 63;
+        const PGItems it = pg_items(__builtin_amdgcn_readfirstlane((int)(threadIdx.x >> 6)));
+        const int lr = lane & 15, lg = lane >> 4, q = lr >> 2, p = lr & 3;
+        const int rsub = 16 * (lg >> 1) + 4 * (lg & 1) + q;
+        const int sw = (rsub >> 1) & 3;
+        const unsigned char* row = tile + rsub * PG_RS + p * 8;
+        const unsigned char* pa0 = row + (((it.a0 & 3) ^ sw) * 32);
+        const unsigned char* pb0 = row + ((it.b0 ^ sw) * 32);
+        const unsigned char* pa1 = row + (((it.a1 & 3) ^ sw) * 32);
+        const unsigned char* pb1 = row + ((it.b1 ^ sw) * 32);
+        const pg_bf16x8_t ones = {(short)0x3F80, (short)0x3F80, (short)0x3F80, (short)0x3F80, (short)0x3F80, (short)0x3F80, (short)0x3F80, (short)0x3F80};
+#pragma unroll 1
+        for (int kb = 0; kb < NROWS / 32; ++kb) {
+            pg_bf16x8_t a0 = frag(pa0, kb), a1 = frag(pa1, kb);
+            const pg_bf16x8_t b0 = frag(pb0, kb), b1 = frag(pb1, kb);
+            if (it.a0 == 4) { a0 = ones; a1 = ones; }
+            acc[0] = __builtin_amdgcn_mfma_f32_16x16x32_bf16(a0, b0, acc[0], 0, 0, 0);
+            acc[1] = __builtin_amdgcn_mfma_f32_16x16x32_bf16(a1, b1, acc[1], 0, 0, 0);
+        }
+    }
+    __device__ __forceinline__ void flush(double* gram) const {
+        const int lane = threadIdx.x & 63;
+        const PGItems it = pg_items(__builtin_amdgcn_readfirstlane((int)(threadIdx.x >> 6)));
+        const int lr = lane & 15, lg = lane >> 4;
+        DET_ENTER();
+#pragma unroll
+        for (int j = 0; j < 2; ++j) {
+            const int a = j ? it.a1 : it.a0, b = j ? it.b1 : it.b0;
+            if (j >= it.n) continue;
+#pragma unroll
+            for (int r = 0; r < 4; ++r) {
+                const int rr = a * 16 + lg * 4 + r, cc = b * 16 + lr;
+                if (rr < PG_C + 8) atomicAdd(gram + (i64)rr * PG_C + cc, (double)acc[j][r]);
+                if (a < 4 && a != b) atomicAdd(gram + (i64)cc * PG_C + rr, (double)acc[j][r]);
+            }
+        }
+        DET_EXIT();
+    }
+};
 
 static_assert(DWN_NREP == 32, "replica reduce below assumes 32 replicas");
 __device__ __forceinline__ void rep_reduce(const double* stats, int stat_c, int sc, int r, bool ok, double& s, double& ss) {
@@ -354,10 +439,10 @@
     }
 }
 
-template <typename T, int CINT>
-__global__ __launch_bounds__(256) void stem_out_kernel(const float* x, const float* w, const float* coef, const float* pe_t,
+template <typename T, int CINT, bool GRAM = false>
+__global__ __launch_bounds__(GRAM ? PG_NT : 256, GRAM ? 4 : 1) void stem_out_kernel(const float* x, const float* w, const float* coef, const float* pe_t,
                                                        const float* pe_h, const float* pe_w, int Tn, int H, int W, int B,
-                                                       int Cin, i64 S, int C0, T* out) {
+                                                       int Cin, i64 S, int C0, T* out, double* gram) {
     SLICE_SETUP(C0)
     constexpr int STEM_MAXCIN = CINT;
     const int chs_ = chan_ok ? chan : 0;
@@ -366,51 +451,83 @@
     for (int c = 0; c < STEM_MAXCIN; ++c)
 #pragma unroll
         for (int i = 0; i < KC; ++i) wr[c][i] = (c < Cin && chan_ok) ? w[(chan + i) * Cin + c] : 0.f;
-    ld_coef<KC>(coef + chs_, sc);
-    ld_coef<KC>(coef + C0 + chs_, sh);
+    if constexpr (!GRAM) {
+        ld_coef<KC>(coef + chs_, sc);
+        ld_coef<KC>(coef + C0 + chs_, sh);
+    }
     const RasterIdx ro(H, W);
     const UDiv32 dT((unsigned)Tn), dS((unsigned)S);
     constexpr int RU = 2;
-    const unsigned nrows = (unsigned)((i64)B * S), stride = gridDim.x * 32u;
-    for (unsigned row0 = blockIdx.x * 32u + pl; row0 < nrows; row0 += RU * stride) {
-        float xm[RU], xv[RU][STEM_MAXCIN];
+    constexpr unsigned RPI = GRAM ? PG_RPI : 32;
+    const unsigned nrows = (unsigned)((i64)B * S), stride = gridDim.x * RPI;
+    using PG = PGram<RU * PG_RPI>;
+    __shared__ __attribute__((aligned(16))) unsigned char pg_tiles[GRAM ? 2 * PG::BYTES : 16];
+    [[maybe_unused]] PG pg;
+    [[maybe_unused]] unsigned pass = 0;
+    float xm[RU];
+    auto fetch_x = [&](unsigned base) {
 #pragma unroll
         for (int u = 0; u < RU; ++u) {
-            const unsigned row = row0 + u * stride < nrows ? row0 + u * stride : row0;
+            unsigned row = base + pl + u * stride;
+            if (row >= nrows) row = GRAM ? 0u : base + pl;
             const unsigned b = dS.div(row), sp = row - b * (unsigned)S;
             xm[u] = cv < Cin ? x[((i64)b * Cin + cv) * S + sp] : 0.f;
         }
+    };
+    if constexpr (GRAM) { if (blockIdx.x * RPI < nrows) fetch_x(blockIdx.x * RPI); }
+    for (unsigned base = blockIdx.x * RPI; base < nrows; base += RU * stride) {
+        const unsigned row0 = base + pl;
+        if constexpr (!GRAM) { if (row0 >= nrows) break; fetch_x(base); }
+        float xv[RU][STEM_MAXCIN];
 #pragma unroll
         for (int u = 0; u < RU; ++u)
 #pragma unroll
             for (int c = 0; c < STEM_MAXCIN; ++c) xv[u][c] = __shfl(xm[u], (tid & 56) | c);
+        if constexpr (GRAM) { if (base + RU * stride < nrows) fetch_x(base + RU * stride); }
+        [[maybe_unused]] unsigned char* tile = pg_tiles + (pass & 1u) * PG::BYTES;
 #pragma unroll
         for (int u = 0; u < RU; ++u) {
             const unsigned row = row0 + u * stride;
-            if (row >= nrows || !chan_ok) break;
-            float v[KC];
-#pragma unroll
-            for (int i = 0; i < KC; ++i) v[i] = 0.f;
-#pragma unroll
-            for (int c = 0; c < STEM_MAXCIN; ++c)
-#pragma unroll
-                for (int i = 0; i < KC; ++i) v[i] = fmaf(wr[c][i], xv[u][c], v[i]);
-#pragma unroll
-            for (int i = 0; i < KC; ++i) v[i] = fmaf(v[i], sc[i], sh[i]);
-            if (pe_t) {
-                unsigned f; int h, wq;
-                ro.decode(row, f, h, wq);
-                const unsigned t = f - dT.div(f) * (unsigned)Tn;
-                float pa[KC], pb[KC], pc[KC];
-                ld_coef<KC>(pe_t + (i64)t * C0 + chan, pa);
-                ld_coef<KC>(pe_h + (i64)h * C0 + chan, pb);
-                ld_coef<KC>(pe_w + (i64)wq * C0 + chan, pc);
-#pragma unroll
-                for (int i = 0; i < KC; ++i) v[i] = round_t<T>(v[i]) + ((pa[i] + pb[i]) + pc[i]);
-            }
-            st_vec<T>(out + (i64)row * C0 + chan, v);
-        }
-    }
+            uint4 pk = make_uint4(0, 0, 0, 0);
+            if (row < nrows && chan_ok) {
+                float v[KC];
+#pragma unroll
+                for (int i = 0; i < KC; ++i) v[i] = 0.f;
+#pragma unroll
+                for (int c = 0; c < STEM_MAXCIN; ++c)
+#pragma unroll
+                    for (int i = 0; i < KC; ++i) v[i] = fmaf(wr[c][i], xv[u][c], v[i]);
+                if constexpr (GRAM) {
+                    ld_coef<KC>(coef + chs_, sc);
+                    ld_coef<KC>(coef + C0 + chs_, sh);
+                }
+#pragma unroll
+                for (int i = 0; i < KC; ++i) v[i] = fmaf(v[i], sc[i], sh[i]);
+                if (pe_t) {
+                    unsigned f; int h, wq;
+                    ro.decode(row, f, h, wq);
+                    const unsigned t = f - dT.div(f) * (unsigned)Tn;
+                    float pa[KC], pb[KC], pc[KC];
+                    ld_coef<KC>(pe_t + (i64)t * C0 + chan, pa);
+                    ld_coef<KC>(pe_h + (i64)h * C0 + chan, pb);
+                    ld_coef<KC>(pe_w + (i64)wq * C0 + chan, pc);
+#pragma unroll
+                    for (int i = 0; i < KC; ++i) v[i] = round_t<T>(v[i]) + ((pa[i] + pb[i]) + pc[i]);
+                }
+                pk = pack16<T>(v);
+                *reinterpret_cast<uint4*>(out + (i64)row * C0 + chan) = pk;
+            } else if constexpr (!GRAM) {
+                break;
+            }
+            if constexpr (GRAM) PG::put(tile, u * (int)PG_RPI + pl, cv, pk);
+        }
+        if constexpr (GRAM) {
+            pg_lds_barrier();
+            pg.mma(tile);
+            ++pass;
+        }
+    }
+    if constexpr (GRAM) pg.flush(gram);
 }
 
 template <typename T, int CINT>
@@ -540,12 +657,21 @@
                             int Tn, int H, int W, int B, int Cin, i64 S, int C0, void* out, hipStream_t s) {
     auto kern = stem_out_kernel<T, CINT>;
     hipLaunchKernelGGL(kern, resident_slice_grid(kern, (i64)B * S, C0, TT<T>::KC), dim3(256), 0, s, x, w, coef, pe_t, pe_h, pe_w, Tn, H, W,
-                       B, Cin, S, C0, (T*)out);
+                       B, Cin, S, C0, (T*)out, (double*)nullptr);
 }
 int k_stem_out(const float* x, const float* w, const float* coef, const float* pe_t, const float* pe_h, const float* pe_w,
-               int Tn, int H, int W, int B, int Cin, i64 S, int C0, void* out, int dtype, hipStream_t s) {
+               int Tn, int H, int W, int B, int Cin, i64 S, int C0, void* out, int dtype, double* gram, hipStream_t s) {
     if (Cin > STEM_MAXCIN) return dwn_set_error(-4, "stem: in_channels > 8 not built");
     if ((i64)B * S >= (1ll << 31)) return dwn_set_error(-4, "stem: more than 2^31 rows");
+    if (gram) {
+        if (dtype != DWN_BF16 || C0 != PG_C) return dwn_set_error(-4, "stem: gram_out is built for bf16 and 64 stem channels");
+        if ((i64)B * S >= (1ll << 31) - 2 * (i64)PG_MAXWG * PG_RPI) return dwn_set_error(-4, "stem: more than 2^31 rows");
+        if (Cin > 5) return dwn_set_error(-4, "stem: gram_out is built for at most 5 input channels");
+        hipLaunchKernelGGL((stem_out_kernel<bf16_t, 5, true>), pgram_grid((i64)B * S), dim3(PG_NT), 0, s, x, w, coef, pe_t, pe_h, pe_w, Tn, H, W,
+                           B, Cin, S, C0, (bf16_t*)out, gram);
+        DWN_CHECK_LAUNCH();
+        return 0;
+    }
     if (Cin <= 5) {
         DISPATCH_T(dtype, (stem_out_launch<bf16_t, 5>(x, w, coef, pe_t, pe_h, pe_w, Tn, H, W, B, Cin, S, C0, out, s)),
                    (stem_out_launch<float, 5>(x, w, coef, pe_t, pe_h, pe_w, Tn, H, W, B, Cin, S, C0, out, s)));
@@ -878,14 +1004,14 @@
     DET_EXIT();
 }
 
-template <typename T>
-__global__ __launch_bounds__(256) void residual_fwd_kernel(LoadDesc xin, const T* y4, const float* coef4,
+template <typename T, bool GRAM = false>
+__global__ __launch_bounds__(GRAM ? PG_NT : 256, GRAM ? 4 : 1) void residual_fwd_kernel(LoadDesc xin, const T* y4, const float* coef4,
                                                            const float* coefsc, const float* dscale, ResGeom gm,
                                                            const float* ope_t, const float* ope_h, const float* ope_w,
-                                                           T* out) {
+                                                           T* out, double* gram) {
     SLICE_SETUP(gm.Cout)
     RES_STAGE_TABLES(gm.hsrc, gm.Hout, gm.wsrc, gm.Wout)
-    if (!chan_ok) return;
+    if constexpr (!GRAM) { if (!chan_ok) return; }
     float s4[KC], t4[KC], ss[KC], ts[KC];
     ld_coef<KC>(coef4 + chan, s4); ld_coef<KC>(coef4 + gm.Cout + chan, t4);
     ld_coef<KC>(coefsc + chan, ss); ld_coef<KC>(coefsc + gm.Cout + chan, ts);
@@ -894,40 +1020,65 @@
     const RasterIdx ro(gm.Hout, gm.Wout);
     const UDiv32 dT((unsigned)gm.T);
     const T* xp = reinterpret_cast<const T*>(xin.p);
-    const unsigned stride = gridDim.x * 32u;
-    for (unsigned row0 = blockIdx.x * 32u + pl; row0 < rows; row0 += RES_RU * stride) {
-        uint4 rs[RES_RU], ry[RES_RU];
-        unsigned btv[RES_RU]; int hov[RES_RU], wov[RES_RU];
+    constexpr unsigned RPI = GRAM ? PG_RPI : 32;
+    const unsigned stride = gridDim.x * RPI;
+    using PG = PGram<RES_RU * PG_RPI>;
+    __shared__ __attribute__((aligned(16))) unsigned char pg_tiles[GRAM ? 2 * PG::BYTES : 16];
+    [[maybe_unused]] PG pg;
+    [[maybe_unused]] unsigned pass = 0;
+    uint4 rs[RES_RU], ry[RES_RU];
+    unsigned btv[RES_RU]; int hov[RES_RU], wov[RES_RU];
+    auto issue_loads = [&](unsigned base) {
 #pragma unroll
         for (int u = 0; u < RES_RU; ++u) {
-            const unsigned row = row0 + u * stride < rows ? row0 + u * stride : row0;
+            unsigned row = base + pl + u * stride;
+            if (row >= rows) row = GRAM ? 0u : base + pl;
             ro.decode(row, btv[u], hov[u], wov[u]);
             const i64 rin = ((i64)btv[u] * gm.Hin + ht_[hov[u]]) * gm.Win + wt_[wov[u]];
             rs[u] = *reinterpret_cast<const uint4*>(xp + rin * xin.ld + csrc);
             ry[u] = *reinterpret_cast<const uint4*>(y4 + (i64)row * gm.Cout + chan);
         }
+    };
+    if constexpr (GRAM) { if (blockIdx.x * RPI < rows) issue_loads(blockIdx.x * RPI); }
+    for (unsigned base = blockIdx.x * RPI; base < rows; base += RES_RU * stride) {
+        const unsigned row0 = base + pl;
+        if constexpr (!GRAM) { if (row0 >= rows) break; issue_loads(base); }
+        [[maybe_unused]] unsigned char* tile = pg_tiles + (pass & 1u) * PG::BYTES;
 #pragma unroll
         for (int u = 0; u < RES_RU; ++u) {
             const unsigned row = row0 + u * stride;
-            if (row >= rows) break;
-            float sv[KC], yv[KC], o[KC];
-            unpack16<T>(rs[u], sv);
-            unpack16<T>(ry[u], yv);
-            const unsigned b = dT.div(btv[u]);
-            const float d = dscale ? dscale[b] : 1.0f;
-#pragma unroll
-            for (int i = 0; i < KC; ++i) o[i] = d * fmaf(yv[i], s4[i], t4[i]) + fmaf(sv[i], ss[i], ts[i]);
-            if (ope_t) {
-                float pa[KC], pb[KC], pc[KC];
-                ld_coef<KC>(ope_t + (i64)(btv[u] - b * (unsigned)gm.T) * gm.Cout + chan, pa);
-                ld_coef<KC>(ope_h + (i64)hov[u] * gm.Cout + chan, pb);
-                ld_coef<KC>(ope_w + (i64)wov[u] * gm.Cout + chan, pc);
-#pragma unroll
-                for (int i = 0; i < KC; ++i) o[i] = round_t<T>(o[i]) + ((pa[i] + pb[i]) + pc[i]);
-            }
-            st_vec<T>(out + (i64)row * gm.Cout + chan, o);
-        }
-    }
+            uint4 pk = make_uint4(0, 0, 0, 0);
+            if (row < rows) {
+                float sv[KC], yv[KC], o[KC];
+                unpack16<T>(rs[u], sv);
+                unpack16<T>(ry[u], yv);
+                const unsigned b = dT.div(btv[u]);
+                const float d = dscale ? dscale[b] : 1.0f;
+#pragma unroll
+                for (int i = 0; i < KC; ++i) o[i] = d * fmaf(yv[i], s4[i], t4[i]) + fmaf(sv[i], ss[i], ts[i]);
+                if (ope_t) {
+                    float pa[KC], pb[KC], pc[KC];
+                    ld_coef<KC>(ope_t + (i64)(btv[u] - b * (unsigned)gm.T) * gm.Cout + chan, pa);
+                    ld_coef<KC>(ope_h + (i64)hov[u] * gm.Cout + chan, pb);
+                    ld_coef<KC>(ope_w + (i64)wov[u] * gm.Cout + chan, pc);
+#pragma unroll
+                    for (int i = 0; i < KC; ++i) o[i] = round_t<T>(o[i]) + ((pa[i] + pb[i]) + pc[i]);
+                }
+                pk = pack16<T>(o);
+                *reinterpret_cast<uint4*>(out + (i64)row * gm.Cout + chan) = pk;
+            } else if constexpr (!GRAM) {
+                break;
+            }
+            if constexpr (GRAM) PG::put(tile, u * (int)PG_RPI + pl, cv, pk);
+        }
+        if constexpr (GRAM) {
+            if (base + RES_RU * stride < rows) issue_loads(base + RES_RU * stride);
+            pg_lds_barrier();
+            pg.mma(tile);
+            ++pass;
+        }
+    }
+    if constexpr (GRAM) pg.flush(gram);
 }
 
 #define RR_RU 2
@@ -1083,11 +1234,18 @@
 }
 int k_residual_fwd(const LoadDesc& xin, const void* y4, const float* coef4, const float* coefsc, const float* dscale,
                    const ResGeom& gm, const float* ope_t, const float* ope_h, const float* ope_w, void* out, int dtype,
-                   hipStream_t s) {
+                   double* gram, hipStream_t s) {
     i64 rows = (i64)gm.BT * gm.Hout * gm.Wout;
+    if (gram) {
+        if (dtype != DWN_BF16 || gm.Cout != PG_C) return dwn_set_error(-4, "residual_fwd: gram_out is built for bf16 and 64 output channels");
+        if (rows >= (1ll << 31) - 2 * (i64)PG_MAXWG * PG_RPI) return dwn_set_error(-4, "residual_fwd: more than 2^31 rows");
+        hipLaunchKernelGGL((residual_fwd_kernel<bf16_t, true>), pgram_grid(rows), dim3(PG_NT), 0, s, xin, (const bf16_t*)y4, coef4, coefsc, dscale, gm, ope_t, ope_h, ope_w, (bf16_t*)out, gram);
+        DWN_CHECK_LAUNCH();
+        return 0;
+    }
     DISPATCH_T(dtype,
-        hipLaunchKernelGGL((residual_fwd_kernel<bf16_t>), slice_grid(rows, gm.Cout, 8), dim3(256), 0, s, xin, (const bf16_t*)y4, coef4, coefsc, dscale, gm, ope_t, ope_h, ope_w, (bf16_t*)out),
-        hipLaunchKernelGGL((residual_fwd_kernel<float>), slice_grid(rows, gm.Cout, 4), dim3(256), 0, s, xin, (const float*)y4, coef4, coefsc, dscale, gm, ope_t, ope_h, ope_w, (float*)out));
+        hipLaunchKernelGGL((residual_fwd_kernel<bf16_t>), slice_grid(rows, gm.Cout, 8), dim3(256), 0, s, xin, (const bf16_t*)y4, coef4, coefsc, dscale, gm, ope_t, ope_h, ope_w, (bf16_t*)out, (double*)nullptr),
+        hipLaunchKernelGGL((residual_fwd_kernel<float>), slice_grid(rows, gm.Cout, 4), dim3(256), 0, s, xin, (const float*)y4, coef4, coefsc, dscale, gm, ope_t, ope_h, ope_w, (float*)out, (double*)nullptr));
     DWN_CHECK_LAUNCH();
     return 0;
 }
diff --git a/sensorium_amd/csrc/dwn_kernels.h b/sensorium_amd/csrc/dwn_kernels.h
--- a/sensorium_amd/csrc/dwn_kernels.h
+++ b/sensorium_amd/csrc/dwn_kernels.h
@@ -27,7 +27,7 @@
                        float* rv, long long* nbt, float momentum, float eps, float* coef, double* xmom, int C0, int Cin,
                        hipStream_t s);
 int k_stem_out(const float* x, const float* w, const float* coef, const float* pe_t, const float* pe_h, const float* pe_w,
-               int Tn, int H, int W, int B, int Cin, i64 S, int C0, void* out, int dtype, hipStream_t s);
+               int Tn, int H, int W, int B, int Cin, i64 S, int C0, void* out, int dtype, double* gram, hipStream_t s);
 int k_stem_bwd_acc(const void* dout, const float* x, const double* xmom, double count, int B, int Cin, i64 S, int C0,
                    double* acc, int dtype, hipStream_t s);
 int k_stem_bwd_finalize(const double* acc, const double* xmom, const float* w, const float* coef, double count, float* dgamma,
@@ -45,7 +45,7 @@
 int k_shortcut_stats(const LoadDesc& xin, const ResGeom& gm, double* stats, int dtype, hipStream_t s);
 int k_residual_fwd(const LoadDesc& xin, const void* y4, const float* coef4, const float* coefsc, const float* dscale,
                    const ResGeom& gm, const float* ope_t, const float* ope_h, const float* ope_w, void* out, int dtype,
-                   hipStream_t s);
+                   double* gram, hipStream_t s);
 int k_residual_bwd_reduce(const LoadDesc& xin, const void* y4, const void* dout, const float* coef4,
                           const float* coefsc, const float* dscale, const ResGeom& gm, double* stats4,
                           double* statssc, int dtype, hipStream_t s);
diff --git a/sensorium_amd/dwiseneuro.py b/sensorium_amd/dwiseneuro.py
--- a/sensorium_amd/dwiseneuro.py
+++ b/sensorium_amd/dwiseneuro.py
@@ -147,12 +147,12 @@
         return geom
 
     def forward(self, x: torch.Tensor, pe: PositionalEncoding3d, dtype: torch.dtype, x_has_pe: bool = False,
-                out_pe=None) -> torch.Tensor:
+                out_pe=None, gram=None) -> torch.Tensor:
         b, t, h, w, _ = x.shape
         geom = self.geometry(pe, t, h, w, x.device)
         drop = self.drop_path.sample(b, x.device)
         mode = ops.bn_mode(self.conv_pw[1].bn.training, x)
-        return ops.BlockFn.apply(x, drop, self, geom, dtype, x_has_pe, out_pe, mode, *self.parameters_in_kernel_order())
+        return ops.BlockFn.apply(x, drop, self, geom, dtype, x_has_pe, out_pe, mode, gram, *self.parameters_in_kernel_order())
 
 
 class ShuffleLayer(nn.Module):
@@ -281,9 +281,15 @@
             s = blk.spatial_stride
             h, w = (h - 1) // s + 1, (w - 1) // s + 1
         tables = [blk.geometry(pe, t, hw[0], hw[1], x.device)[:3] for pe, blk, hw in zip(pes, blks, sizes)]
-        x = ops.StemFn.apply(x, self.stem[0].weight, bn.weight, bn.bias, self, dtype, tables[0], ops.bn_mode(bn.training, x))
+        b = x.shape[0]
+        train = [bn.training] + [blk.conv_pw[1].bn.training for blk in blks]
+        grams = [ops.gram_buffer(blk.in_features, x.device)
+                 if train[i] and train[i + 1] and (i > 0 or x.shape[1] <= 5)
+                 and ops.block_takes_gram(blk, (b, t, hw[0], hw[1], blk.in_features), dtype) else None
+                 for i, (blk, hw) in enumerate(zip(blks, sizes))] + [None]
+        x = ops.StemFn.apply(x, self.stem[0].weight, bn.weight, bn.bias, self, dtype, tables[0], ops.bn_mode(bn.training, x), grams[0])
         for i, (pe, blk) in enumerate(zip(pes, blks)):
-            x = blk(x, pe, dtype, True, tables[i + 1] if i + 1 < len(blks) else None)
+            x = blk(x, pe, dtype, True, tables[i + 1] if i + 1 < len(blks) else None, (grams[i], grams[i + 1]))
         return x
 
 
diff --git a/sensorium_amd/ops.py b/sensorium_amd/ops.py
--- a/sensorium_amd/ops.py
+++ b/sensorium_amd/ops.py
@@ -109,6 +109,29 @@
 
 _PWL_BWD = _env_choice("DWN_PWL_BWD", {"": 0, "new": 1, "old": 2})
 _Y1_MODE = _env_choice("DWN_Y1", {"": 0, "free": 0, "materialise": 1, "all": 2})
+_GRAM_MODE = _env_choice("DWN_GRAM", {"": 0, "producer": 0, "pass": 1})
+GRAM_CHANNELS = 64
+
+
+def block_takes_gram(blk, x_shape, dtype) -> bool:
+    B, T, Hin, Win, Cin = x_shape
+    if _GRAM_MODE or dtype != torch.bfloat16 or Cin != GRAM_CHANNELS or not hasattr(L.lib, "dwn_block_takes_gram"):
+        return False
+    if torch.cuda.is_current_stream_capturing():
+        return False
+    a = L.BlockArgs()
+    a.dtype = _DT[dtype]; a.training = L.BN_TRAIN
+    a.B = B; a.T = T; a.Hin = Hin; a.Win = Win
+    a.Hout = (Hin - 1) // blk.spatial_stride + 1
+    a.Wout = (Win - 1) // blk.spatial_stride + 1
+    a.Cin = Cin; a.Cmid = blk.mid_features; a.Cout = blk.out_features
+    a.stride = blk.spatial_stride; a.ks = blk.spatial_kernel; a.kt = blk.temporal_kernel
+    a.y1_mode = getattr(blk, "_dwn_y1_mode", _Y1_MODE)
+    return bool(L.lib.dwn_block_takes_gram(C.byref(a)))
+
+
+def gram_buffer(channels: int, device) -> torch.Tensor:
+    return torch.empty((channels + 8) * channels, dtype=torch.float64, device=device)
 
 
 def grad_out(param: torch.Tensor, zero: bool = False) -> torch.Tensor:
@@ -158,7 +181,7 @@
 class StemFn(torch.autograd.Function):
 
     @staticmethod
-    def forward(ctx, x, weight, gamma, beta, mod, dtype, pe=None, mode=None):
+    def forward(ctx, x, weight, gamma, beta, mod, dtype, pe=None, mode=None, gram_out=None):
         _require_gpu(x, "StemFn")
         conv, bn = mod.stem[0], mod.stem[1].bn
         _check_bn(bn)
@@ -179,6 +202,7 @@
         if pe is not None:
             a.pe_t, a.pe_h, a.pe_w = (t.data_ptr() for t in pe)
         a.T, a.H, a.W = T, H, W
+        a.gram_out = _ptr(gram_out)
         ws = _ws(L.lib.dwn_stem_workspace_bytes(C.byref(a)), dev)
         a.ws = ws.data_ptr(); a.ws_bytes = ws.numel()
         L.check(L.lib.dwn_stem_forward(C.byref(a), dev.index, _stream(dev)), "dwn_stem_forward")
@@ -204,7 +228,7 @@
             g.w = weight.data_ptr(); g.coef = coef.data_ptr(); g.dout = dout.data_ptr(); g.dx = dx.data_ptr()
             L.check(L.lib.dwn_stem_input_grad(C.byref(g), dev.index, _stream(dev)), "dwn_stem_input_grad")
             if not any(ctx.needs_input_grad[1:4]):
-                return dx, None, None, None, None, None, None, None
+                return dx, None, None, None, None, None, None, None, None
         dw = grad_out(ctx.mod.stem[0].weight)
         dgamma = grad_out(bn.weight)
         dbeta = grad_out(bn.bias)
@@ -220,7 +244,7 @@
             L.check(L.lib.dwn_stem_backward_input(C.byref(a), dx.data_ptr(), dev.index, _stream(dev)), "dwn_stem_backward_input")
         else:
             L.check(L.lib.dwn_stem_backward(C.byref(a), dev.index, _stream(dev)), "dwn_stem_backward")
-        return dx, dw, dgamma, dbeta, None, None, None, None
+        return dx, dw, dgamma, dbeta, None, None, None, None, None
 
 
 _BLOCK_PARAMS = ("w_pw", "g1", "b1", "w_dws", "g2", "b2", "w_dwt", "g3", "b3", "se_wr", "se_br", "se_we", "se_be",
@@ -262,7 +286,7 @@
 class BlockFn(torch.autograd.Function):
 
     @staticmethod
-    def forward(ctx, x, drop_scale, blk, geom, dtype, x_has_pe, out_pe, mode, *params):
+    def forward(ctx, x, drop_scale, blk, geom, dtype, x_has_pe, out_pe, mode, gram, *params):
         _require_gpu(x, "BlockFn")
         x = x.contiguous()
         dev = x.device
@@ -294,6 +318,8 @@
         if out_pe is not None:
             a.out_pe_t, a.out_pe_h, a.out_pe_w = (t.data_ptr() for t in out_pe)
         a.bn1, a.bn2, a.bn3, a.bn4, a.bnsc = (_bn_struct(bn, cf) for bn, cf in zip(bns, coefs))
+        gram_in, gram_out = gram if gram is not None else (None, None)
+        a.gram_in = _ptr(gram_in); a.gram_out = _ptr(gram_out)
         ws = _ws(L.lib.dwn_block_workspace_bytes(C.byref(a), 0), dev)
         a.ws = ws.data_ptr(); a.ws_bytes = ws.numel()
         L.check(L.lib.dwn_block_forward(C.byref(a), dev.index, _stream(dev)), "dwn_block_forward")
@@ -359,7 +385,7 @@
         _ddp_flush()
         grads = (dw_pw, dg[0], db[0], dw_dws, dg[1], db[1], dw_dwt, dg[2], db[2], dse_wr, dse_br, dse_we, dse_be,
                  dw_pwl, dg[3], db[3], dg[4], db[4])
-        return (dx, None, None, None, None, None, None, None) + grads
+        return (dx, None, None, None, None, None, None, None, None) + grads
 
 
 class PoolFn(torch.autograd.Function):
```

Result: no change. 1476 (-0.0%).
